# chzchzchz/raftsql

Hardware: AMD Instinct MI355X
Metric: quorum decisions/sec (commit+vote) across G groups (higher is better)
Workload: dtype u64

## Files before the change

go/raftq/engine_more.go:

```go
package raftq

import "C"

import "unsafe"

func ABIVersion() int { return int(C.raftq_abi_version()) }

func Quorum(peers uint32) uint32 { return uint32(C.raftq_quorum(C.uint32_t(peers))) }

func (e *Engine) NGroups() uint64 { return uint64(C.raftq_groups(e.h)) }
func (e *Engine) NPeers() uint32  { return uint32(C.raftq_peers(e.h)) }

func (e *Engine) SelfMax() (int, error) {
	var slot C.int32_t
	if err := e.err(C.raftq_self_max(e.h, &slot)); err != nil {
		return -1, err
	}
	return int(slot), nil
}

func (e *Engine) Narrow() (bool, error) {
	var valid C.int32_t
	if err := e.err(C.raftq_narrow(e.h, &valid)); err != nil {
		return false, err
	}
	return valid != 0, nil
}

func (e *Engine) NarrowRebuild() error { return e.err(C.raftq_narrow_rebuild(e.h)) }

func (e *Engine) SetStream(stream unsafe.Pointer) error { return e.err(C.raftq_set_stream(e.h, stream)) }
func (e *Engine) Stream() unsafe.Pointer                { return C.raftq_get_stream(e.h) }

type TermDelta struct{ Group, CurTerm, FirstIdxCurTerm uint64 }

func (e *Engine) ApplyTermDeltas(d []TermDelta) error {
	if len(d) == 0 {
		return nil
	}
	return e.err(C.raftq_apply_term_deltas(e.h, (*C.raftq_term_delta_t)(unsafe.Pointer(&d[0])), C.uint64_t(len(d))))
}

func (e *Engine) CommitAdvance(gated bool, committedOut []uint64) (changed uint64, err error) {
	var p *C.uint64_t
	if committedOut != nil {
		p = (*C.uint64_t)(unsafe.Pointer(&committedOut[0]))
	}
	g := C.int(0)
	if gated {
		g = 1
	}
	var n C.uint64_t
	err = e.err(C.raftq_commit_advance(e.h, g, p, &n))
	return uint64(n), err
}

func (e *Engine) VoteTally(outcomeOut []uint8) (Counts, error) {
	var p *C.uint8_t
	if outcomeOut != nil {
		p = (*C.uint8_t)(unsafe.Pointer(&outcomeOut[0]))
	}
	var c C.raftq_counts_t
	if err := e.err(C.raftq_vote_tally(e.h, p, &c)); err != nil {
		return Counts{}, err
	}
	return Counts{uint64(c.n_changed), uint64(c.n_won), uint64(c.n_lost)}, nil
}

func (e *Engine) ReadVotes(out []uint8) error {
	return e.err(C.raftq_read_votes(e.h, (*C.uint8_t)(unsafe.Pointer(&out[0]))))
}

func (e *Engine) SetTimers(electionTick, heartbeatTick uint32, seed uint64) error {
	return e.err(C.raftq_set_timers(e.h, C.uint32_t(electionTick), C.uint32_t(heartbeatTick), C.uint64_t(seed)))
}

type TickCounts struct{ Hup, Beat uint64 }

func (e *Engine) Tick(wantCounts bool) (TickCounts, error) {
	var c C.raftq_tick_counts_t
	if !wantCounts {
		return TickCounts{}, e.err(C.raftq_tick(e.h, nil))
	}
	err := e.err(C.raftq_tick(e.h, &c))
	return TickCounts{uint64(c.n_hup), uint64(c.n_beat)}, err
}

func (e *Engine) CollectHups(out []uint64) (uint64, error) {
	var n C.uint64_t
	var p *C.uint64_t
	if len(out) > 0 {
		p = (*C.uint64_t)(unsafe.Pointer(&out[0]))
	}
	rc := C.raftq_collect_hups(e.h, p, C.uint64_t(len(out)), &n)
	return uint64(n), e.err(rc)
}

func (e *Engine) TickCollect(hups, beats []uint64) (nHup, nBeat uint64, err error) {
	var hp, bp *C.uint64_t
	if len(hups) > 0 {
		hp = (*C.uint64_t)(unsafe.Pointer(&hups[0]))
	}
	if len(beats) > 0 {
		bp = (*C.uint64_t)(unsafe.Pointer(&beats[0]))
	}
	var nh, nb C.uint64_t
	err = e.err(C.raftq_tick_collect(e.h, hp, C.uint64_t(len(hups)), &nh, bp, C.uint64_t(len(beats)), &nb))
	return uint64(nh), uint64(nb), err
}

const TickBeatBitmap = uint(C.RAFTQ_TICK_BEAT_BITMAP)

// ... 218 lines not shown
```

include/raftq.h:

```cpp
#ifndef RAFTQ_H
#define RAFTQ_H

#include <stddef.h>
#include <stdint.h>

#ifdef __cplusplus
extern "C" {
#endif

#define RAFTQ_ABI_VERSION 1
#define RAFTQ_MAX_PEERS 9

#define RAFTQ_OK 0
#define RAFTQ_EINVAL (-1)
#define RAFTQ_ENOMEM (-2)
#define RAFTQ_EHIP (-3)
#define RAFTQ_ESTATE (-4)
#define RAFTQ_ENODEV (-5)

#define RAFTQ_SWEEP_COMMIT 0x01u
#define RAFTQ_SWEEP_GATED 0x02u
#define RAFTQ_SWEEP_VOTES 0x04u
#define RAFTQ_SWEEP_NO_ADOPT 0x08u
#define RAFTQ_SWEEP_LDS 0x10u
// ... 16 lines not shown
  uint64_t match;
  uint32_t peer;
  uint32_t _pad;
} raftq_delta_t;

typedef struct raftq_vote_delta {
  uint64_t group;
  uint32_t peer;
  uint8_t vote;
  uint8_t _pad[3];
} raftq_vote_delta_t;

typedef struct raftq_term_delta {
  uint64_t group;
  uint64_t cur_term;
  uint64_t first_idx_cur_term;
} raftq_term_delta_t;

typedef struct raftq_advance {
  uint64_t group;
  uint64_t old_commit;
  uint64_t new_commit;
} raftq_advance_t;

typedef struct raftq_delta16 {
  uint64_t match;
  uint32_t group;
  uint32_t peer;
} raftq_delta16_t;
typedef struct raftq_advance16 {
  uint64_t new_commit;
  uint32_t group;
  uint32_t advanced_by;
} raftq_advance16_t;

int raftq_abi_version(void);
int raftq_device_count(int* n);
uint32_t raftq_quorum(uint32_t n_peers);

#define RAFTQ_MAX_GROUPS (1ull << 30)
int raftq_create(int device, uint64_t n_groups, uint32_t n_peers, raftq_t** out);
void raftq_destroy(raftq_t* h);
uint64_t raftq_groups(const raftq_t* h);
uint32_t raftq_peers(const raftq_t* h);
const char* raftq_last_error(const raftq_t* h);

int raftq_set_stream(raftq_t* h, void* stream);
void* raftq_get_stream(const raftq_t* h);

int raftq_load_match(raftq_t* h, const uint64_t* match ,
                     const uint64_t* committed );
int raftq_load_terms(raftq_t* h, const uint64_t* cur_term ,
                     const uint64_t* first_idx_cur_term );
int raftq_load_votes(raftq_t* h, const uint8_t* votes );

int raftq_apply_deltas(raftq_t* h, const raftq_delta_t* d, uint64_t n);
int raftq_apply_vote_deltas(raftq_t* h, const raftq_vote_delta_t* d, uint64_t n);
int raftq_apply_term_deltas(raftq_t* h, const raftq_term_delta_t* d, uint64_t n);

typedef struct raftq_voter_delta {
  uint64_t group;
  uint16_t voters;
  uint16_t reset;
  uint32_t _pad;
} raftq_voter_delta_t;
int raftq_load_voters(raftq_t* h, const uint16_t* voters);
int raftq_apply_voter_deltas(raftq_t* h, const raftq_voter_delta_t* d, uint64_t n);
int raftq_read_voters(raftq_t* h, uint16_t* voters_out);

int raftq_step_async(raftq_t* h, unsigned flags);
int raftq_wait(raftq_t* h, raftq_counts_t* counts);

int raftq_commit_advance(raftq_t* h, int gated, uint64_t* committed_out ,
                         uint64_t* n_changed );
int raftq_vote_tally(raftq_t* h, uint8_t* outcome_out ,
                     raftq_counts_t* counts );

int raftq_read_committed(raftq_t* h, uint64_t* committed_out );
int raftq_read_outcome(raftq_t* h, uint8_t* outcome_out );
int raftq_read_match(raftq_t* h, uint64_t* match_out );
int raftq_self_max(raftq_t* h, int32_t* slot_out);
int raftq_narrow(raftq_t* h, int32_t* valid_out);
int raftq_narrow_rebuild(raftq_t* h);
int raftq_read_votes(raftq_t* h, uint8_t* votes_out );
int raftq_collect_changed(raftq_t* h, raftq_advance_t* out, uint64_t cap, uint64_t* n);

#define RAFTQ_ROLE_FOLLOWER 0
#define RAFTQ_ROLE_CANDIDATE 1
#define RAFTQ_ROLE_LEADER 2
#define RAFTQ_ROLE_PRE_CANDIDATE 3
typedef struct raftq_tick_counts {
  uint64_t n_hup;
  uint64_t n_beat;
} raftq_tick_counts_t;
int raftq_set_timers(raftq_t* h, uint32_t election_tick, uint32_t heartbeat_tick, uint64_t seed);
int raftq_load_roles(raftq_t* h, const uint8_t* role , const uint32_t* elapsed );
int raftq_tick_set_voters(raftq_t* h, int on);
int raftq_tick(raftq_t* h, raftq_tick_counts_t* counts);
int raftq_read_tick(raftq_t* h, uint8_t* action , uint32_t* elapsed , uint8_t* role );
int raftq_collect_hups(raftq_t* h, uint64_t* groups, uint64_t cap, uint64_t* n);
int raftq_collect_beats(raftq_t* h, uint64_t* groups, uint64_t cap, uint64_t* n);
int raftq_tick_collect(raftq_t* h, uint64_t* hups, uint64_t hup_cap, uint64_t* n_hup, uint64_t* beats, uint64_t beat_cap,
                       uint64_t* n_beat);

#define RAFTQ_TICK_BEAT_BITMAP 1u
int raftq_tick_collect_lists(raftq_t* h, unsigned flags, uint64_t hup_cap, uint64_t beat_cap, uint64_t* n_hup, uint64_t* n_beat);
int raftq_last_tick_lists(raftq_t* h, const uint32_t** hups, uint64_t* n_hups, const uint32_t** beats, uint64_t* n_beats,
                          const uint64_t** beat_bitmap, uint64_t* bitmap_words);
int raftq_set_check_quorum(raftq_t* h, int on);
int raftq_tick_set_checks(raftq_t* h, uint64_t chk_cap);
int raftq_last_tick_checks(raftq_t* h, const uint32_t** checks, uint64_t* n_listed, uint64_t* n_total);
int raftq_load_activity(raftq_t* h, const uint16_t* active , const uint32_t* lead_elapsed );
int raftq_read_activity(raftq_t* h, uint16_t* active , uint32_t* lead_elapsed );
int raftq_collect_checks(raftq_t* h, uint64_t* groups, uint64_t cap, uint64_t* n);

int raftq_set_pre_vote(raftq_t* h, int on);

int raftq_set_lead_transfer(raftq_t* h, int on);
int raftq_load_transfer(raftq_t* h, const uint8_t* transferee );
int raftq_read_transfer(raftq_t* h, uint8_t* transferee );

#define RAFTQ_READ_SAFE 1
#define RAFTQ_READ_LEASE 2
int raftq_set_read_index(raftq_t* h, int mode);
int raftq_load_reads(raftq_t* h, const uint32_t* seq , const uint32_t* acked );
int raftq_read_reads(raftq_t* h, uint32_t* seq, uint32_t* acked, uint32_t* confirmed );

int raftq_campaign(raftq_t* h, const uint64_t* groups, uint64_t n, uint32_t self_peer);

int raftq_cycle(raftq_t* h, const raftq_delta_t* deltas, uint64_t n_deltas,
                const raftq_vote_delta_t* vote_deltas, uint64_t n_vote_deltas, unsigned flags,
                raftq_advance_t* advances_out, uint64_t cap, uint64_t* n_advanced,
                raftq_counts_t* counts);

int raftq_stage(raftq_t* h, uint64_t n_deltas, uint64_t n_vote_deltas, raftq_delta_t** deltas,
                raftq_vote_delta_t** vote_deltas);
int raftq_last_advances(raftq_t* h, const raftq_advance_t** list, uint64_t* n_listed);

int raftq_cycle_packed(raftq_t* h, const raftq_delta16_t* deltas, uint64_t n_deltas,
                       const raftq_vote_delta_t* vote_deltas, uint64_t n_vote_deltas, unsigned flags,
                       raftq_advance16_t* advances_out, uint64_t cap, uint64_t* n_advanced,
                       raftq_counts_t* counts);
int raftq_stage_packed(raftq_t* h, uint64_t n_deltas, uint64_t n_vote_deltas, raftq_delta16_t** deltas,
                       raftq_vote_delta_t** vote_deltas);
int raftq_last_advances_packed(raftq_t* h, const raftq_advance16_t** list, uint64_t* n_listed);

#define RAFTQ_CYCLE_SEGMENTED 0x200u
int raftq_last_advance_segments(raftq_t* h, const raftq_advance16_t** recs, const uint32_t** counts, uint32_t* n_segments,
                                uint64_t* stride);

typedef struct raftq_set raftq_set_t;
#define RAFTQ_SET_GRID 0
#define RAFTQ_SET_PERSISTENT 1
int raftq_set_create(raftq_t* const* handles, uint32_t n, raftq_set_t** out);
int raftq_set_create_voters(raftq_t* const* handles, uint32_t n, raftq_set_t** out);
void raftq_set_destroy(raftq_set_t* s);
uint32_t raftq_set_size(const raftq_set_t* s);
const char* raftq_set_last_error(const raftq_set_t* s);
void* raftq_set_get_stream(const raftq_set_t* s);
int raftq_set_mode(raftq_set_t* s, int mode, uint32_t persist_workgroups);
int raftq_set_sweep_async(raftq_set_t* s, unsigned flags);
int raftq_set_tick(raftq_set_t* s);
int raftq_set_wait(raftq_set_t* s, raftq_counts_t* per_member, raftq_counts_t* total);
int raftq_set_timer_begin(raftq_set_t* s);
int raftq_set_timer_end(raftq_set_t* s, float* elapsed_ms);
int raftq_sweep_many_async(raftq_t* const* handles, uint32_t n, unsigned flags);
// ... 13 lines not shown
```

raftsql_amd/_lib.py:

```python
from __future__ import annotations

import ctypes as C
import os

_HERE = os.path.dirname(os.path.abspath(__file__))
LIB_PATH = os.environ.get("RAFTQ_LIB") or os.path.join(_HERE, "libraftq.so")

RAFTQ_OK = 0
RAFTQ_EINVAL, RAFTQ_ENOMEM, RAFTQ_EHIP, RAFTQ_ESTATE, RAFTQ_ENODEV = -1, -2, -3, -4, -5

SWEEP_COMMIT = 0x01
SWEEP_GATED = 0x02
SWEEP_VOTES = 0x04
SWEEP_NO_ADOPT = 0x08
SWEEP_LDS = 0x10
SWEEP_CHANGED = 0x20
SWEEP_STREAM = 0x40
SWEEP_CACHED = 0x80
CYCLE_TRUSTED = 0x100
TICK_BEAT_BITMAP = 1
CYCLE_SEGMENTED = 0x200
SET_GRID, SET_PERSISTENT = 0, 1

MAX_PEERS = 9
READ_SAFE, READ_LEASE = 1, 2


class Counts(C.Structure):
    _fields_ = [("n_changed", C.c_uint64), ("n_won", C.c_uint64), ("n_lost", C.c_uint64)]


class TickCounts(C.Structure):
    _fields_ = [("n_hup", C.c_uint64), ("n_beat", C.c_uint64)]


class Delta(C.Structure):
    _fields_ = [("group", C.c_uint64), ("match", C.c_uint64), ("peer", C.c_uint32), ("_pad", C.c_uint32)]


class VoteDelta(C.Structure):
    _fields_ = [("group", C.c_uint64), ("peer", C.c_uint32), ("vote", C.c_uint8), ("_pad", C.c_uint8 * 3)]


class VoterDelta(C.Structure):
    _fields_ = [("group", C.c_uint64), ("voters", C.c_uint16), ("reset", C.c_uint16), ("_pad", C.c_uint32)]


class Advance(C.Structure):
    _fields_ = [("group", C.c_uint64), ("old_commit", C.c_uint64), ("new_commit", C.c_uint64)]


_H = C.c_void_p
_SIGS = [
    ("raftq_abi_version", C.c_int, []),
    ("raftq_device_count", C.c_int, [C.POINTER(C.c_int)]),
    ("raftq_quorum", C.c_uint32, [C.c_uint32]),
    ("raftq_create", C.c_int, [C.c_int, C.c_uint64, C.c_uint32, C.POINTER(_H)]),
    ("raftq_destroy", None, [_H]),
    ("raftq_groups", C.c_uint64, [_H]),
    ("raftq_peers", C.c_uint32, [_H]),
    ("raftq_last_error", C.c_char_p, [_H]),
    ("raftq_set_stream", C.c_int, [_H, C.c_void_p]),
    ("raftq_get_stream", C.c_void_p, [_H]),
    ("raftq_load_match", C.c_int, [_H, C.c_void_p, C.c_void_p]),
    ("raftq_load_terms", C.c_int, [_H, C.c_void_p, C.c_void_p]),
    ("raftq_load_votes", C.c_int, [_H, C.c_void_p]),
    ("raftq_apply_deltas", C.c_int, [_H, C.c_void_p, C.c_uint64]),
    ("raftq_apply_vote_deltas", C.c_int, [_H, C.c_void_p, C.c_uint64]),
    ("raftq_apply_term_deltas", C.c_int, [_H, C.c_void_p, C.c_uint64]),
    ("raftq_load_voters", C.c_int, [_H, C.c_void_p]),
    ("raftq_apply_voter_deltas", C.c_int, [_H, C.c_void_p, C.c_uint64]),
    ("raftq_read_voters", C.c_int, [_H, C.c_void_p]),
    ("raftq_step_async", C.c_int, [_H, C.c_uint]),
    ("raftq_wait", C.c_int, [_H, C.POINTER(Counts)]),
    ("raftq_commit_advance", C.c_int, [_H, C.c_int, C.c_void_p, C.POINTER(C.c_uint64)]),
    ("raftq_vote_tally", C.c_int, [_H, C.c_void_p, C.POINTER(Counts)]),
    ("raftq_read_committed", C.c_int, [_H, C.c_void_p]),
    ("raftq_read_outcome", C.c_int, [_H, C.c_void_p]),
    ("raftq_read_match", C.c_int, [_H, C.c_void_p]),
    ("raftq_self_max", C.c_int, [_H, C.POINTER(C.c_int32)]),
    ("raftq_narrow", C.c_int, [_H, C.POINTER(C.c_int32)]),
    ("raftq_narrow_rebuild", C.c_int, [_H]),
    ("raftq_read_votes", C.c_int, [_H, C.c_void_p]),
    ("raftq_collect_changed", C.c_int, [_H, C.c_void_p, C.c_uint64, C.POINTER(C.c_uint64)]),
    ("raftq_set_timers", C.c_int, [_H, C.c_uint32, C.c_uint32, C.c_uint64]),
    ("raftq_load_roles", C.c_int, [_H, C.c_void_p, C.c_void_p]),
    ("raftq_tick_set_voters", C.c_int, [_H, C.c_int]),
    ("raftq_tick_set_checks", C.c_int, [_H, C.c_uint64]),
    ("raftq_last_tick_checks", C.c_int, [_H, C.POINTER(C.c_void_p), C.POINTER(C.c_uint64), C.POINTER(C.c_uint64)]),
    ("raftq_tick", C.c_int, [_H, C.POINTER(TickCounts)]),
    ("raftq_read_tick", C.c_int, [_H, C.c_void_p, C.c_void_p, C.c_void_p]),
    ("raftq_collect_hups", C.c_int, [_H, C.c_void_p, C.c_uint64, C.POINTER(C.c_uint64)]),
    ("raftq_collect_beats", C.c_int, [_H, C.c_void_p, C.c_uint64, C.POINTER(C.c_uint64)]),
    ("raftq_tick_collect", C.c_int, [_H, C.c_void_p, C.c_uint64, C.POINTER(C.c_uint64), C.c_void_p, C.c_uint64, C.POINTER(C.c_uint64)]),
    ("raftq_tick_collect_lists", C.c_int, [_H, C.c_uint, C.c_uint64, C.c_uint64, C.POINTER(C.c_uint64), C.POINTER(C.c_uint64)]),
    ("raftq_last_tick_lists", C.c_int, [_H, C.POINTER(C.c_void_p), C.POINTER(C.c_uint64), C.POINTER(C.c_void_p), C.POINTER(C.c_uint64),
                                        C.POINTER(C.c_void_p), C.POINTER(C.c_uint64)]),
    ("raftq_set_check_quorum", C.c_int, [_H, C.c_int]),
    ("raftq_set_pre_vote", C.c_int, [_H, C.c_int]),
    ("raftq_set_lead_transfer", C.c_int, [_H, C.c_int]),
    ("raftq_load_transfer", C.c_int, [_H, C.c_void_p]),
    ("raftq_read_transfer", C.c_int, [_H, C.c_void_p]),
    ("raftq_set_read_index", C.c_int, [_H, C.c_int]),
    ("raftq_load_reads", C.c_int, [_H, C.c_void_p, C.c_void_p]),
    ("raftq_read_reads", C.c_int, [_H, C.c_void_p, C.c_void_p, C.c_void_p]),
    ("raftq_load_activity", C.c_int, [_H, C.c_void_p, C.c_void_p]),
    ("raftq_read_activity", C.c_int, [_H, C.c_void_p, C.c_void_p]),
    ("raftq_collect_checks", C.c_int, [_H, C.c_void_p, C.c_uint64, C.POINTER(C.c_uint64)]),
    ("raftq_campaign", C.c_int, [_H, C.c_void_p, C.c_uint64, C.c_uint32]),
    ("raftq_cycle", C.c_int, [_H, C.c_void_p, C.c_uint64, C.c_void_p, C.c_uint64, C.c_uint, C.c_void_p, C.c_uint64,
                              C.POINTER(C.c_uint64), C.POINTER(Counts)]),
    ("raftq_stage", C.c_int, [_H, C.c_uint64, C.c_uint64, C.POINTER(C.c_void_p), C.POINTER(C.c_void_p)]),
    ("raftq_last_advances", C.c_int, [_H, C.POINTER(C.c_void_p), C.POINTER(C.c_uint64)]),
    ("raftq_cycle_packed", C.c_int, [_H, C.c_void_p, C.c_uint64, C.c_void_p, C.c_uint64, C.c_uint, C.c_void_p, C.c_uint64,
                                     C.POINTER(C.c_uint64), C.POINTER(Counts)]),
    ("raftq_stage_packed", C.c_int, [_H, C.c_uint64, C.c_uint64, C.POINTER(C.c_void_p), C.POINTER(C.c_void_p)]),
    ("raftq_last_advances_packed", C.c_int, [_H, C.POINTER(C.c_void_p), C.POINTER(C.c_uint64)]),
    ("raftq_last_advance_segments", C.c_int, [_H, C.POINTER(C.c_void_p), C.POINTER(C.c_void_p), C.POINTER(C.c_uint32), C.POINTER(C.c_uint64)]),
    ("raftq_set_create", C.c_int, [C.POINTER(_H), C.c_uint32, C.POINTER(_H)]),
    ("raftq_set_create_voters", C.c_int, [C.POINTER(_H), C.c_uint32, C.POINTER(_H)]),
    ("raftq_set_destroy", None, [_H]),
    ("raftq_set_size", C.c_uint32, [_H]),
    ("raftq_set_last_error", C.c_char_p, [_H]),
    ("raftq_set_get_stream", C.c_void_p, [_H]),
    ("raftq_set_mode", C.c_int, [_H, C.c_int, C.c_uint32]),
    ("raftq_set_sweep_async", C.c_int, [_H, C.c_uint]),
    ("raftq_set_wait", C.c_int, [_H, C.c_void_p, C.POINTER(Counts)]),
    ("raftq_set_tick", C.c_int, [_H]),
    ("raftq_set_timer_begin", C.c_int, [_H]),
    ("raftq_set_timer_end", C.c_int, [_H, C.POINTER(C.c_float)]),
    ("raftq_sweep_many_async", C.c_int, [C.POINTER(_H), C.c_uint32, C.c_uint]),
    ("raftq_clone_state", C.c_int, [_H, _H]),
    ("raftq_timer_begin", C.c_int, [_H]),
    ("raftq_timer_end", C.c_int, [_H, C.POINTER(C.c_float)]),
    ("raftq_host_alloc", C.c_int, [C.POINTER(C.c_void_p), C.c_uint64]),
    ("raftq_host_free", None, [C.c_void_p]),
]
EXPORTS = [s[0] for s in _SIGS]


class StepCounts(C.Structure):
    _fields_ = [("n_msgs", C.c_uint64), ("n_groups_touched", C.c_uint64)]


_STEP_SIGS = [
    ("raftq_set_self", C.c_int, [_H, C.c_uint32]),
    ("raftq_load_node", C.c_int, [_H, C.c_void_p, C.c_void_p, C.c_void_p, C.c_void_p, C.c_void_p]),
    ("raftq_read_node", C.c_int, [_H, C.c_void_p, C.c_void_p, C.c_void_p, C.c_void_p, C.c_void_p, C.c_void_p]),
    ("raftq_step_batch", C.c_int, [_H, C.c_void_p, C.c_uint64, C.c_void_p, C.POINTER(StepCounts)]),
    ("raftq_apply_log_deltas", C.c_int, [_H, C.c_void_p, C.c_uint64, C.c_void_p]),
    ("raftq_apply_log_deltas_nowait", C.c_int, [_H, C.c_void_p, C.c_uint64]),
    ("raftq_step_submit", C.c_int, [_H, C.c_void_p, C.c_uint64]),
    ("raftq_step_collect", C.c_int, [_H, C.c_void_p, C.POINTER(StepCounts)]),
    ("raftq_step_stage", C.c_int, [_H, C.c_uint64, C.POINTER(C.c_void_p)]),
    ("raftq_step_stage_packed", C.c_int, [_H, C.c_uint64, C.POINTER(C.c_void_p)]),
    ("raftq_step_submit_packed", C.c_int, [_H, C.c_void_p, C.c_uint64]),
    ("raftq_step_results", C.c_int, [_H, C.POINTER(C.c_void_p), C.POINTER(C.c_uint64)]),
    ("raftq_step_set_compact", C.c_int, [_H, C.c_int]),
    ("raftq_step_set_msg_flags", C.c_int, [_H, C.c_int]),
    ("raftq_step_set_voters", C.c_int, [_H, C.c_int]),
    ("raftq_step_set_props", C.c_int, [_H, C.c_int]),
    ("raftq_step_results_c", C.c_int, [_H, C.POINTER(C.c_void_p), C.POINTER(C.c_uint64)]),
    ("raftq_step_results_s", C.c_int, [_H, C.POINTER(C.c_void_p), C.POINTER(C.c_uint64)]),
]
STEP_EXPORTS = [s[0] for s in _STEP_SIGS]
# ... 86 lines not shown
```

raftsql_amd/csrc/raftq_capi.hip:

```cpp
#include "raftq.h"

#include <hip/hip_runtime.h>

#include <algorithm>
#include <atomic>
#include <mutex>
#include <chrono>
#include <cstdlib>
#include <cstdio>
#include <cstring>
#include <new>
#include <string>
#include <type_traits>
#include <unordered_set>
#include <vector>

#include "raftq_internal.hpp"

#ifndef RAFTQ_GPL
#define RAFTQ_GPL 4
#endif
#ifndef RAFTQ_AUTO_STREAM_BYTES
#define RAFTQ_AUTO_STREAM_BYTES (128ull << 20)
#endif
// ... 147 lines not shown
        const dim3 grid((unsigned)(gpad / ((uint64_t)kBlock * G))), block(kBlock);
        hipLaunchKernelGGL((sweep_voters_kernel<NP, G, Form::commit, Form::gated, Form::votes, decltype(pol)::value>), grid, block, 0, s, a);
        return hipGetLastError();
      });
    });
  });
}

struct VoterSetLaunch {
  const VoterSweepArgs* tab;
  uint32_t members, want_bits;
  uint64_t gpad;
};

hipError_t launch_set_voters(uint32_t N, const VoterSetLaunch& L, unsigned flags, int nt, hipStream_t s) {
  return with_peers(N, [&](auto n) {
    return with_flag_form(flags, [&](auto form) {
      return with_policy(nt, [&](auto pol) {
        using Form = decltype(form);
        constexpr int NP = decltype(n)::value, G = voters_gpl(NP);
        const dim3 grid((unsigned)(L.gpad / ((uint64_t)kBlock * G)), L.members), block(kBlock);
        hipLaunchKernelGGL((sweep_set_voters_kernel<NP, G, Form::commit, Form::gated, Form::votes, decltype(pol)::value>), grid, block, 0, s,
                           L.tab, L.want_bits);
        return hipGetLastError();
      });
    });
  });
}

}
int raftq_detail::ensure_staging(raftq_t* h, size_t bytes) {
  HIPCHK(h, h->stage.grow(bytes, std::max({bytes, h->stage.cap * 2, (size_t)1 << 20}), &h->stream));
  return RAFTQ_OK;
}

int raftq_detail::ensure_ingest(raftq_t* h, size_t bytes) {
  HIPCHK(h, h->ingest.grow(bytes, std::max({bytes, h->ingest.cap * 2, (size_t)1 << 20}), &h->stream, h->bar));
  return RAFTQ_OK;
}

namespace {
int ensure_adv(raftq_t* h, uint64_t entries) {
  const uint64_t have = h->adv.cap / sizeof(Advance);
  const uint64_t want = std::min<uint64_t>(std::max<uint64_t>({entries, have * 2, 4096}), h->gpad);
  HIPCHK(h, h->adv.grow(entries * sizeof(Advance), want * sizeof(Advance), &h->stream));
  return RAFTQ_OK;
}

}
int raftq_detail::self_max_check(raftq_t* h) {
  if (int rc = use_device(h)) return rc;
  if (h->step_collected != h->step_submitted) {
    HIPCHK(h, hipMemsetAsync(h->self_max, 0, sizeof(uint32_t), h->stream));
    return RAFTQ_OK;
  }
  HIPCHK(h, hipMemsetD32Async((hipDeviceptr_t)h->self_max, (int)(kSelfMaxValid | h->self_peer), 1, h->stream));
  const uint64_t blocks = std::min<uint64_t>((h->G + kBlock - 1) / kBlock, 4096);
  hipLaunchKernelGGL(self_max_check_kernel, dim3((unsigned)std::max<uint64_t>(blocks, 1)), dim3(kBlock), 0, h->stream,
                     (const uint64_t*)h->match, h->ld, h->G, h->N, h->self_peer, h->self_max);
  HIPCHK(h, hipGetLastError());
  return RAFTQ_OK;
}
int raftq_detail::narrow_build(raftq_t* h) {
  if (int rc = use_device(h)) return rc;
  if (h->narrow_off) return RAFTQ_OK;
  if (h->step_collected != h->step_submitted) {
    HIPCHK(h, hipMemsetAsync(h->narrow_word(), 0, sizeof(uint32_t), h->stream));
    return RAFTQ_OK;
  }
  if (!h->anchor) {
    const hipError_t e = raftq_buf::alloc_group({{(void**)&h->anchor, h->ld * sizeof(uint64_t)},
                                                 {(void**)&h->moff, (size_t)h->N * h->ld * sizeof(uint32_t)}},
                                                h->stream);
    if (e != hipSuccess) {
      (void)hipGetLastError();
      return RAFTQ_OK;
    }
    if (h->in_set) h->in_set->tab_stale = true;
  }
  HIPCHK(h, hipMemsetD32Async((hipDeviceptr_t)h->narrow_word(), (int)kNarrowValid, 1, h->stream));
  const uint64_t blocks = std::min<uint64_t>((h->G + kBlock - 1) / kBlock, 4096);
  hipLaunchKernelGGL(narrow_build_kernel, dim3((unsigned)std::max<uint64_t>(blocks, 1)), dim3(kBlock), 0, h->stream,
                     (const uint64_t*)h->match, h->ld, h->G, h->N, h->anchor, h->moff, h->narrow_word());
  HIPCHK(h, hipGetLastError());
  return RAFTQ_OK;
}
int raftq_detail::use_device(raftq_t* h) {
  if (!h) return fail(nullptr, RAFTQ_EINVAL, "null handle");
  HIPCHK(h, hipSetDevice(h->device));
  return RAFTQ_OK;
}
int raftq_detail::use_device_idle(raftq_t* h, const char* who) {
  if (int rc = use_device(h)) return rc;
  if (h->step_collected != h->step_submitted)
    return fail(h, RAFTQ_ESTATE, std::string(who) + ": Step batches are in flight; collect them first");
  return RAFTQ_OK;
}
using raftq_detail::ensure_staging;
using raftq_detail::ensure_ingest;
using raftq_detail::use_device;
using raftq_detail::use_device_idle;
using raftq_detail::ensure_tick_state;
using raftq_detail::dense_changed;

template <typename W>
static void pack_votes(const uint8_t* votes, uint64_t G, uint32_t N, W* out) {
  for (uint64_t g = 0; g < G; ++g) out[g] = 0;
  for (uint32_t p = 0; p < N; ++p) {
    const uint8_t* row = votes + (size_t)p * G;
    for (uint64_t g = 0; g < G; ++g) {
      const uint8_t v = row[g];
      out[g] = (W)(out[g] | (W)((v == 1 ? 1u : v == 2 ? 2u : 0u) << (2 * p)));
    }
  }
}
template <typename W>
static void unpack_votes(const W* in, uint64_t G, uint32_t N, uint8_t* votes) {
  for (uint32_t p = 0; p < N; ++p) {
    uint8_t* row = votes + (size_t)p * G;
    for (uint64_t g = 0; g < G; ++g) {
      const uint32_t f = ((uint32_t)in[g] >> (2 * p)) & 3u;
      row[g] = f == 3u ? 0 : (uint8_t)f;
    }
  }
}

extern "C" {

int raftq_abi_version(void) { return RAFTQ_ABI_VERSION; }

uint32_t raftq_quorum(uint32_t n_peers) { return n_peers / 2 + 1; }

int raftq_device_count(int* n) {
  if (!n) return fail(nullptr, RAFTQ_EINVAL, "raftq_device_count: null out");
  int c = 0;
  hipError_t e = hipGetDeviceCount(&c);
  if (e != hipSuccess) {
    *n = 0;
    return fail(nullptr, RAFTQ_ENODEV, std::string("hipGetDeviceCount: ") + hipGetErrorString(e));
  }
  *n = c;
  return RAFTQ_OK;
}

const char* raftq_last_error(const raftq_t* h) { return h ? h->err.c_str() : g_err.c_str(); }

uint64_t raftq_groups(const raftq_t* h) { return h ? h->G : 0; }
uint32_t raftq_peers(const raftq_t* h) { return h ? h->N : 0; }

int raftq_create(int device, uint64_t n_groups, uint32_t n_peers, raftq_t** out) {
  if (!out) return fail(nullptr, RAFTQ_EINVAL, "raftq_create: null out");
  *out = nullptr;
  if (n_groups == 0 || n_groups > RAFTQ_MAX_GROUPS)
    return fail(nullptr, RAFTQ_EINVAL, "raftq_create: n_groups out of range (1 .. RAFTQ_MAX_GROUPS = 2^30 per handle)");
  if (n_peers < 1 || n_peers > RAFTQ_MAX_PEERS) return fail(nullptr, RAFTQ_EINVAL, "raftq_create: n_peers must be 1..9");
  int ndev = 0;
  if (hipGetDeviceCount(&ndev) != hipSuccess || ndev <= 0)
    return fail(nullptr, RAFTQ_ENODEV, "raftq_create: no HIP device (this library has no CPU path)");
  if (device < 0 || device >= ndev) return fail(nullptr, RAFTQ_ENODEV, "raftq_create: device index out of range");
  raftq_t* h = new (std::nothrow) raftq();
  if (!h) return fail(nullptr, RAFTQ_ENOMEM, "raftq_create: host allocation failed");
  h->device = device;
  h->G = n_groups;
  h->N = n_peers;
  h->last_gpl = kGPL;
  h->gpad = (n_groups + kTileMax - 1) / kTileMax * kTileMax;
  h->ld = h->gpad + kRowStagger;
  const uint64_t ld = h->ld;
  h->max_partials = h->gpad / (kBlock * 2) * kWaves;
  int rc = RAFTQ_OK;
  do {
    if ((rc = use_device(h))) break;
    hipError_t e = hipStreamCreateWithFlags(&h->stream, hipStreamNonBlocking);
    if (e != hipSuccess) { rc = fail(h, RAFTQ_EHIP, std::string("hipStreamCreate: ") + hipGetErrorString(e)); break; }
    h->own_stream = true;
    {
      int large_bar = 0;
      (void)hipDeviceGetAttribute(&large_bar, hipDeviceAttributeIsLargeBar, device);
      const char* st = std::getenv("RAFTQ_STAGE");
      h->bar.staging = large_bar == 1 && !(st && std::strcmp(st, "host") == 0);
    }
    e = raftq_buf::alloc_group({{(void**)&h->match, (size_t)n_peers * ld * 8},
                                {(void**)&h->committed[0], ld * 8},
                                {(void**)&h->committed[1], ld * 8},
                                {(void**)&h->first_idx, ld * 8},
                                {(void**)&h->votes, (size_t)vote_word_bytes((int)n_peers) * ld},
                                {(void**)&h->outcome, ld / 4 + 64},
                                {(void**)&h->changed_bits, h->gpad / 8},
                                {(void**)&h->partials, h->max_partials * sizeof(uint4)},
                                {(void**)&h->offsets, (h->max_partials + 1) * 8},
                                {(void**)&h->self_max, 64}},
                               h->stream);
    if (e != hipSuccess) {
      rc = fail(h, e == hipErrorOutOfMemory ? RAFTQ_ENOMEM : RAFTQ_EHIP, std::string("device arrays: ") + hipGetErrorString(e));
      break;
    }
    {
      const char* nr = std::getenv("RAFTQ_NARROW");
      h->narrow_off = nr && std::strcmp(nr, "0") == 0;
    }
    e = hipMemsetD32Async((hipDeviceptr_t)h->self_max, (int)(kSelfMaxValid | 0u), 1, h->stream);
    if (e != hipSuccess) { rc = fail(h, RAFTQ_EHIP, std::string("hipMemsetD32Async: ") + hipGetErrorString(e)); break; }
    e = raftq_buf::alloc_group({{(void**)&h->h_partials, h->max_partials * sizeof(uint4), raftq_buf::Kind::pinned},
                                {(void**)&h->h_total, 64, raftq_buf::Kind::mapped_coherent, (void**)&h->d_total}},
                               h->stream);
    if (e != hipSuccess) { rc = fail(h, RAFTQ_ENOMEM, std::string("page-locked memory: ") + hipGetErrorString(e)); break; }
    e = hipEventCreate(&h->ev0);
    if (e == hipSuccess) e = hipEventCreate(&h->ev1);
    if (e != hipSuccess) { rc = fail(h, RAFTQ_EHIP, std::string("hipEventCreate: ") + hipGetErrorString(e)); break; }
    e = hipStreamSynchronize(h->stream);
    if (e != hipSuccess) { rc = fail(h, RAFTQ_EHIP, std::string("hipStreamSynchronize: ") + hipGetErrorString(e)); break; }
  } while (0);
  if (rc != RAFTQ_OK) {
    std::string keep = h->err;
    raftq_destroy(h);
    g_err = keep;
    return rc;
  }
  *out = h;
  return RAFTQ_OK;
}

void raftq_destroy(raftq_t* h) {
  if (!h) return;
  if (h->in_set) {
    raftq_set_t* s = h->in_set;
    s->broken = true;
    s->members.erase(std::remove(s->members.begin(), s->members.end(), h), s->members.end());
    (void)hipSetDevice(h->device);
    (void)hipStreamSynchronize(s->stream);
    h->stream = nullptr;
    h->own_stream = false;
  }
  if (h->prof_n && std::getenv("RAFTQ_PROFILE"))
    std::fprintf(stderr,
                 "[raftq] cycle phases, avg us over %llu calls: stage/validate %.1f | enqueue scatter %.1f | enqueue sweep "
                 "%.1f | enqueue collect %.1f | sync %.1f | copy-out %.1f | turns that ended in the blocking wait instead of the "
                 "polled flag: %llu\n",
                 (unsigned long long)h->prof_n, h->prof[0] / h->prof_n, h->prof[1] / h->prof_n, h->prof[2] / h->prof_n,
                 h->prof[3] / h->prof_n, h->prof[4] / h->prof_n, h->prof[5] / h->prof_n, (unsigned long long)h->flag_fallbacks);
  (void)hipSetDevice(h->device);
  if (h->stream) (void)hipStreamSynchronize(h->stream);
  if (h->many_aux) (void)hipStreamSynchronize(h->many_aux);
  raftq_detail::free_node_state(h);
  raftq_detail::free_wire_state(h);
  raftq_buf::free_device(h->match, h->committed[0], h->committed[1], h->first_idx, h->votes, h->voters, h->outcome, h->changed_bits,
                         h->partials, h->offsets, h->self_max, h->anchor, h->moff, h->claim, h->delta_bad, h->role, h->elapsed, h->action, h->hup_bits,
                         h->beat_bits, h->tick_partials, h->tick_offsets2, h->tick_offsets3, h->cq, h->chk_bits, h->reads);
  raftq_buf::free_host(h->h_partials, h->h_total);
  if (h->ev0) (void)hipEventDestroy(h->ev0);
  if (h->ev1) (void)hipEventDestroy(h->ev1);
  if (h->many_aux) {
    (void)hipEventDestroy(h->many_fork);
    (void)hipEventDestroy(h->many_join);
  }
  const hipStream_t streams[4] = {h->many_aux, h->step_s_in, h->step_s_out, h->own_stream ? h->stream : nullptr};
  delete h;
  for (hipStream_t st : streams)
    if (st) (void)hipStreamDestroy(st);
}

int raftq_set_stream(raftq_t* h, void* stream) {
  if (int rc = use_device_idle(h, "raftq_set_stream")) return rc;
  if (h->in_set) return fail(h, RAFTQ_ESTATE, "raftq_set_stream: the handle is a member of a sweep set, which owns its stream");
  HIPCHK(h, hipStreamSynchronize(h->stream));
  if (h->own_stream) HIPCHK(h, hipStreamDestroy(h->stream));
  h->stream = (hipStream_t)stream;
  h->own_stream = false;
  return RAFTQ_OK;
}

void* raftq_get_stream(const raftq_t* h) { return h ? (void*)h->stream : nullptr; }

int raftq_load_match(raftq_t* h, const uint64_t* match, const uint64_t* committed) {
  if (int rc = use_device_idle(h, "raftq_load_match")) return rc;
  if (!match && !committed) return fail(h, RAFTQ_EINVAL, "raftq_load_match: nothing to load");
  if (match) {
    for (uint32_t p = 0; p < h->N; ++p)
      HIPCHK(h, hipMemcpyAsync(h->match + (size_t)p * h->ld, match + (size_t)p * h->G, h->G * 8, hipMemcpyHostToDevice, h->stream));
    if (int rc = raftq_detail::self_max_check(h)) return rc;
    if (int rc = raftq_detail::narrow_build(h)) return rc;
  }
  dense_changed(h);
  if (committed)
    HIPCHK(h, hipMemcpyAsync(h->committed[h->cur], committed, h->G * 8, hipMemcpyHostToDevice, h->stream));
  HIPCHK(h, hipStreamSynchronize(h->stream));
  return RAFTQ_OK;
}

int raftq_load_terms(raftq_t* h, const uint64_t* cur_term, const uint64_t* first_idx_cur_term) {
  if (int rc = use_device_idle(h, "raftq_load_terms")) return rc;
  if (!cur_term || !first_idx_cur_term) return fail(h, RAFTQ_EINVAL, "raftq_load_terms: null argument");
  std::vector<uint64_t> f;
  try {
    f.assign(first_idx_cur_term, first_idx_cur_term + h->G);
  } catch (...) {
    return fail(h, RAFTQ_ENOMEM, "raftq_load_terms: host allocation failed");
  }
  for (uint64_t g = 0; g < h->G; ++g)
    if (cur_term[g] == 0) f[g] = 0;
  HIPCHK(h, hipMemcpyAsync(h->first_idx, f.data(), h->G * 8, hipMemcpyHostToDevice, h->stream));
  dense_changed(h);
  HIPCHK(h, hipStreamSynchronize(h->stream));
  h->have_terms = true;
  return RAFTQ_OK;
}

int raftq_load_votes(raftq_t* h, const uint8_t* votes) {
  if (int rc = use_device_idle(h, "raftq_load_votes")) return rc;
  if (!votes) return fail(h, RAFTQ_EINVAL, "raftq_load_votes: null argument");
  const size_t wb = (size_t)vote_word_bytes((int)h->N);
  std::vector<uint8_t> packed;
  try {
    packed.resize(h->G * wb);
  } catch (...) {
    return fail(h, RAFTQ_ENOMEM, "raftq_load_votes: host allocation failed");
  }
  if (wb == 2) pack_votes(votes, h->G, h->N, reinterpret_cast<uint16_t*>(packed.data()));
  else pack_votes(votes, h->G, h->N, reinterpret_cast<uint32_t*>(packed.data()));
  HIPCHK(h, hipMemcpyAsync(h->votes, packed.data(), packed.size(), hipMemcpyHostToDevice, h->stream));
  HIPCHK(h, hipStreamSynchronize(h->stream));
  return RAFTQ_OK;
}

static int ensure_delta_dev(raftq_t* h, size_t bytes) {
  if (!h->delta_bad) HIPCHK(h, raftq_buf::alloc_zeroed((void**)&h->delta_bad, 64, h->stream));
  HIPCHK(h, h->delta_dev.grow(bytes, std::max(bytes * 2, (size_t)1 << 20), &h->stream));
  return RAFTQ_OK;
}

static int check_deltas(raftq_t* h, bool trusted = false) {
  int rc = RAFTQ_OK;
  const char* what = trusted ? "; that record was dropped, every other record of the turn was applied (RAFTQ_CYCLE_TRUSTED)"
                             : "; nothing applied";
  if (h->delta_check[0] && h->h_total[1] == h->delta_check[0])
    rc = fail(h, RAFTQ_EINVAL, std::string("a match delta is out of range (group >= G or peer >= N)") + what);
  if (h->delta_check[1] && h->h_total[2] == h->delta_check[1])
    rc = fail(h, RAFTQ_EINVAL, std::string("a vote delta is invalid (group/peer out of range or vote not 1/2)") + what);
  h->delta_check[0] = h->delta_check[1] = 0;
  return rc;
}

}

template <typename Rec, typename AbiRec>
static int enqueue_ingest(raftq_t* h, const AbiRec* d, uint64_t n, const raftq_vote_delta_t* vd, uint64_t nv, size_t off_votes,
                          bool trusted = false) {
  static_assert(sizeof(Rec) == sizeof(AbiRec), "ABI struct mismatch");
  static_assert(sizeof(VoteDeltaRec) == sizeof(raftq_vote_delta_t), "ABI struct mismatch");
  if (nv > 0xfffffffeull) return fail(h, RAFTQ_EINVAL, "vote delta batch too large");
  auto inside = [&](const void* q) {
    return (const uint8_t*)q >= (const uint8_t*)h->ingest.h && (const uint8_t*)q < (const uint8_t*)h->ingest.h + h->ingest.cap;
  };
  if (n) {
    AbiRec* dst = (AbiRec*)h->ingest.h;
    if ((const void*)d != (const void*)dst) {
      if (inside(d)) return fail(h, RAFTQ_EINVAL, "match deltas staged with other counts / another record layout than this call's");
      std::memcpy(dst, d, (size_t)n * sizeof(AbiRec));
    }
  }
  if (nv) {
    raftq_vote_delta_t* dst = (raftq_vote_delta_t*)((uint8_t*)h->ingest.h + off_votes);
    if ((const void*)vd != (const void*)dst) {
      if (inside(vd)) return fail(h, RAFTQ_EINVAL, "vote deltas staged with other counts / another record layout than this call's");
      std::memcpy(dst, vd, (size_t)nv * sizeof(raftq_vote_delta_t));
    }
    if (!h->claim) {
      HIPCHK(h, raftq_buf::alloc_filled((void**)&h->claim, (size_t)h->N * h->ld * sizeof(uint32_t), 0xff, h->stream));
    }
  }
  h->ingest.publish();
  if (int rc = ensure_delta_dev(h, h->ingest.cap)) return rc;
  const unsigned long long em = n ? ++h->delta_epoch : kNoEpoch, ev = nv ? ++h->delta_epoch : kNoEpoch;
  h->delta_check[0] = n ? em : 0;
  h->delta_check[1] = nv ? ev : 0;
  Rec* dev_m = (Rec*)h->delta_dev.d;
  VoteDeltaRec* dev_v = (VoteDeltaRec*)((uint8_t*)h->delta_dev.d + off_votes);
  const unsigned long long* bad = h->delta_bad;
  const dim3 gm((unsigned)((n + kBlock - 1) / kBlock)), gv((unsigned)((nv + kBlock - 1) / kBlock));
  if (n) dense_changed(h);
  if (n && trusted)
    hipLaunchKernelGGL((deltas_in_apply_kernel<Rec>), gm, dim3(kBlock), 0, h->stream, (const Rec*)h->ingest.d, n, h->match, h->ld,
                       h->G, h->N, h->delta_bad, h->d_total + 1, em, h->self_max, h->narrow_mirror());
  else if (n)
    hipLaunchKernelGGL((deltas_in_kernel<Rec>), gm, dim3(kBlock), 0, h->stream, (const Rec*)h->ingest.d, dev_m, n, h->G, h->N,
                       h->delta_bad, h->d_total + 1, em);
  if (nv)
    hipLaunchKernelGGL(vote_deltas_in_kernel, gv, dim3(kBlock), 0, h->stream,
                       (const VoteDeltaRec*)((uint8_t*)h->ingest.d + off_votes), dev_v, nv, h->G, h->N, h->delta_bad + 1,
                       h->d_total + 2, ev);
  if (n && !trusted)
    hipLaunchKernelGGL((apply_deltas_kernel<Rec>), gm, dim3(kBlock), 0, h->stream, h->match, h->ld, (const Rec*)dev_m, n, bad, em,
                       ev, h->self_max, h->narrow_mirror());
  if (nv) {
    const unsigned long long em_gate = trusted ? kNoEpoch : em;
    hipLaunchKernelGGL(vote_claim_kernel, gv, dim3(kBlock), 0, h->stream, h->claim, h->ld, (const VoteDeltaRec*)dev_v, nv, bad,
                       em_gate, ev, h->G, h->N, trusted ? 1 : 0);
    hipLaunchKernelGGL(vote_apply_kernel, gv, dim3(kBlock), 0, h->stream, h->votes, h->N > 8 ? 1 : 0, h->claim, h->ld,
                       (const VoteDeltaRec*)dev_v, nv, bad, em_gate, ev, h->G, h->N, trusted ? 1 : 0);
  }
  HIPCHK(h, hipGetLastError());
  return RAFTQ_OK;
}

extern "C" {

int raftq_apply_deltas(raftq_t* h, const raftq_delta_t* d, uint64_t n) {
  if (int rc = use_device_idle(h, "raftq_apply_deltas")) return rc;
  if (n == 0) return RAFTQ_OK;
  if (!d) return fail(h, RAFTQ_EINVAL, "raftq_apply_deltas: null argument");
  if (int rc = ensure_ingest(h, (size_t)n * sizeof(raftq_delta_t))) return rc;
  if (int rc = enqueue_ingest<DeltaRec>(h, d, n, nullptr, 0, 0)) return rc;
  HIPCHK(h, hipStreamSynchronize(h->stream));
  return check_deltas(h);
}

int raftq_apply_term_deltas(raftq_t* h, const raftq_term_delta_t* d, uint64_t n) {
  static_assert(sizeof(TermDeltaRec) == sizeof(raftq_term_delta_t), "ABI struct mismatch");
  if (int rc = use_device_idle(h, "raftq_apply_term_deltas")) return rc;
  if (n == 0) return RAFTQ_OK;
  if (!d) return fail(h, RAFTQ_EINVAL, "raftq_apply_term_deltas: null argument");
  for (uint64_t i = 0; i < n; ++i)
    if (d[i].group >= h->G) return fail(h, RAFTQ_EINVAL, "a term delta is out of range; nothing applied");
  if (int rc = ensure_staging(h, (size_t)n * sizeof(raftq_term_delta_t))) return rc;
  raftq_term_delta_t* dst = (raftq_term_delta_t*)h->stage.h;
  uint64_t m = 0;
  {
    std::unordered_set<uint64_t> seen;
    seen.reserve((size_t)n * 2);
    std::vector<uint64_t> keep;
    keep.reserve(n);
    for (uint64_t i = n; i-- > 0;)
      if (seen.insert(d[i].group).second) keep.push_back(i);
    for (auto it = keep.rbegin(); it != keep.rend(); ++it) dst[m++] = d[*it];
  }
  const dim3 grid((unsigned)((m + kBlock - 1) / kBlock));
  dense_changed(h);
  hipLaunchKernelGGL(apply_term_deltas_kernel, grid, dim3(kBlock), 0, h->stream, h->first_idx,
                     (const TermDeltaRec*)h->stage.d, m);
  HIPCHK(h, hipGetLastError());
  HIPCHK(h, hipStreamSynchronize(h->stream));
  h->have_terms = true;
  return RAFTQ_OK;
}

int raftq_apply_vote_deltas(raftq_t* h, const raftq_vote_delta_t* d, uint64_t n) {
  if (int rc = use_device_idle(h, "raftq_apply_vote_deltas")) return rc;
  if (n == 0) return RAFTQ_OK;
  if (!d) return fail(h, RAFTQ_EINVAL, "raftq_apply_vote_deltas: null argument");
  if (int rc = ensure_ingest(h, (size_t)n * sizeof(raftq_vote_delta_t))) return rc;
  if (int rc = enqueue_ingest<DeltaRec>(h, (const raftq_delta_t*)nullptr, 0, d, n, 0)) return rc;
  HIPCHK(h, hipStreamSynchronize(h->stream));
  return check_deltas(h);
}

}

static int ensure_voters(raftq_t* h) {
  if (h->voters) return RAFTQ_OK;
  HIPCHK(h, raftq_buf::alloc_zeroed((void**)&h->voters, h->ld * sizeof(uint16_t), h->stream));
  if (h->in_set) h->in_set->tab_stale = true;
  return RAFTQ_OK;
}
static int drop_voters(raftq_t* h) {
  if (!h->voters) return RAFTQ_OK;
  HIPCHK(h, hipStreamSynchronize(h->stream));
  raftq_buf::free_device(h->voters);
  if (h->in_set) h->in_set->tab_stale = true;
  return RAFTQ_OK;
}
static int voters_not_in_set(raftq_t* h, const char* who) {
  if (!h->in_set || h->in_set->allow_voters) return RAFTQ_OK;
  return fail(h, RAFTQ_ESTATE, std::string(who) + ": the handle is a member of a sweep set, whose dispatches count every slot "
                                                  "(voter masks on set members are out of scope)");
}
int raftq_detail::refuse_voters(raftq_t* h, const char* who, bool step_family, bool tick_rounds, bool bcast) {
  if (!h || !h->voters) return RAFTQ_OK;
  if (tick_rounds && h->tick_voters) return RAFTQ_OK;
  if (bcast) {
    if (h->bcast_voters) return RAFTQ_OK;
    return fail(h, RAFTQ_ESTATE, std::string(who) + ": the handle has voter masks loaded and did not opt in with raftq_bcast_set_voters; its broadcast "
                                                    "would go to N - 1 slots, not to a group's membership (whatever raftq_step_set_voters and "
                                                    "raftq_tick_set_voters say)");
  }
  if (h->step_voters) {
    if (step_family) return RAFTQ_OK;
    return fail(h, RAFTQ_ESTATE, std::string(who) + ": the handle has voter masks loaded; the broadcasts built on the device go to N - 1 slots, "
                                                    "not to a group's membership (out of scope, whatever raftq_step_set_voters says)");
  }
  return fail(h, RAFTQ_ESTATE, std::string(who) + ": the handle has voter masks loaded; Step's maybeCommit / poll on the device "
                                                  "count every slot (out of scope: raftq_load_voters(h, NULL) first)");
}

extern "C" {

int raftq_load_voters(raftq_t* h, const uint16_t* voters) {
  if (int rc = use_device_idle(h, "raftq_load_voters")) return rc;
  if (int rc = voters_not_in_set(h, "raftq_load_voters")) return rc;
  if (!voters) return drop_voters(h);
  const uint32_t beyond = 0xffffu & ~((1u << h->N) - 1u);
  for (uint64_t g = 0; g < h->G; ++g)
    if (voters[g] & beyond) return fail(h, RAFTQ_EINVAL, "raftq_load_voters: a mask names a peer slot >= N; nothing loaded");
  if (int rc = ensure_voters(h)) return rc;
  HIPCHK(h, hipMemcpyAsync(h->voters, voters, h->G * sizeof(uint16_t), hipMemcpyHostToDevice, h->stream));
  HIPCHK(h, hipStreamSynchronize(h->stream));
  return RAFTQ_OK;
}

int raftq_read_voters(raftq_t* h, uint16_t* voters_out) {
  if (int rc = use_device_idle(h, "raftq_read_voters")) return rc;
  if (!voters_out) return fail(h, RAFTQ_EINVAL, "raftq_read_voters: null argument");
  if (!h->voters) {
    std::fill(voters_out, voters_out + h->G, (uint16_t)((1u << h->N) - 1u));
    return RAFTQ_OK;
  }
  HIPCHK(h, hipMemcpyAsync(voters_out, h->voters, h->G * sizeof(uint16_t), hipMemcpyDeviceToHost, h->stream));
  HIPCHK(h, hipStreamSynchronize(h->stream));
  return RAFTQ_OK;
}

int raftq_apply_voter_deltas(raftq_t* h, const raftq_voter_delta_t* d, uint64_t n) {
  static_assert(sizeof(VoterDeltaRec) == sizeof(raftq_voter_delta_t), "ABI struct mismatch");
  if (int rc = use_device_idle(h, "raftq_apply_voter_deltas")) return rc;
  if (int rc = voters_not_in_set(h, "raftq_apply_voter_deltas")) return rc;
  if (n == 0) return RAFTQ_OK;
  if (!d) return fail(h, RAFTQ_EINVAL, "raftq_apply_voter_deltas: null argument");
  const uint32_t beyond = 0xffffu & ~((1u << h->N) - 1u);
  for (uint64_t i = 0; i < n; ++i)
    if (d[i].group >= h->G || ((d[i].voters | d[i].reset) & beyond))
      return fail(h, RAFTQ_EINVAL, "a voter delta is out of range (group >= G or a bit >= N); nothing applied");
  if (int rc = ensure_staging(h, (size_t)n * sizeof(raftq_voter_delta_t))) return rc;
  raftq_voter_delta_t* dst = (raftq_voter_delta_t*)h->stage.h;
  uint64_t m = 0;
  try {
    std::unordered_set<uint64_t> seen;
    seen.reserve((size_t)n * 2);
    std::vector<uint64_t> keep;
    keep.reserve(n);
    for (uint64_t i = n; i-- > 0;)
      if (seen.insert(d[i].group).second) keep.push_back(i);
    for (auto it = keep.rbegin(); it != keep.rend(); ++it) dst[m++] = d[*it];
  } catch (...) {
    return fail(h, RAFTQ_ENOMEM, "raftq_apply_voter_deltas: host allocation failed");
  }
  if (!h->voters) {
    if (int rc = ensure_voters(h)) return rc;
    hipLaunchKernelGGL(fill_voters_kernel, dim3((unsigned)((h->G + kBlock - 1) / kBlock)), dim3(kBlock), 0, h->stream, h->voters, h->G,
                       (uint16_t)((1u << h->N) - 1u));
    HIPCHK(h, hipGetLastError());
  }
  dense_changed(h);
  hipLaunchKernelGGL(apply_voter_deltas_kernel, dim3((unsigned)((m + kBlock - 1) / kBlock)), dim3(kBlock), 0, h->stream, h->voters, h->match,
                     h->ld, h->votes, h->N > 8 ? 1 : 0, h->N, (const VoterDeltaRec*)h->stage.d, m, h->self_max, h->narrow_word());
  HIPCHK(h, hipGetLastError());
  HIPCHK(h, hipStreamSynchronize(h->stream));
  return RAFTQ_OK;
}

static int sweep_check(raftq_t* h, unsigned flags, const char* who) {
  const unsigned known = RAFTQ_SWEEP_COMMIT | RAFTQ_SWEEP_GATED | RAFTQ_SWEEP_VOTES | RAFTQ_SWEEP_NO_ADOPT |
                         RAFTQ_SWEEP_LDS | RAFTQ_SWEEP_CHANGED | RAFTQ_SWEEP_STREAM | RAFTQ_SWEEP_CACHED;
  const std::string w(who);
  if (flags & ~known) return fail(h, RAFTQ_EINVAL, w + ": unknown flag");
  const bool commit = flags & (RAFTQ_SWEEP_COMMIT | RAFTQ_SWEEP_GATED);
  const bool votes = flags & RAFTQ_SWEEP_VOTES;
  if (!commit && !votes) return fail(h, RAFTQ_EINVAL, w + ": nothing to sweep");
  if ((flags & RAFTQ_SWEEP_GATED) && !h->have_terms)
    return fail(h, RAFTQ_ESTATE, w + ": gated sweep before raftq_load_terms");
  if ((flags & RAFTQ_SWEEP_STREAM) && (flags & RAFTQ_SWEEP_CACHED))
    return fail(h, RAFTQ_EINVAL, w + ": RAFTQ_SWEEP_STREAM and RAFTQ_SWEEP_CACHED are exclusive");
  if ((flags & RAFTQ_SWEEP_CHANGED) && !commit)
    return fail(h, RAFTQ_EINVAL, w + ": RAFTQ_SWEEP_CHANGED needs a commit sweep");
  if ((flags & RAFTQ_SWEEP_LDS) && h->voters)
    return fail(h, RAFTQ_EINVAL, w + ": RAFTQ_SWEEP_LDS has no form for a handle with voter masks loaded (the A/B variant counts every slot)");
  return RAFTQ_OK;
}

static SweepArgs sweep_args(const raftq_t* h, int cur, bool want_bits) {
  SweepArgs a;
  a.match = h->match;
  a.committed = h->committed[cur];
  a.committed_out = h->committed[cur ^ 1];
  a.first_idx = h->first_idx;
  a.votes = h->votes;
  a.outcome = h->outcome;
  a.changed_bits = want_bits ? h->changed_bits : nullptr;
  a.partials = h->partials;
  a.ld = h->ld;
  a.self_max = h->self_max;
  a.narrow = h->anchor ? h->narrow_word() : nullptr;
  a.anchor = h->anchor;
  a.moff = h->moff;
  return a;
}

static uint64_t sweep_footprint(const raftq_t* h) { return h->ld * (8ull * h->N + 24 + vote_word_bytes((int)h->N) + 1 + (h->voters ? 2 : 0)); }

static int sweep_policy(unsigned flags, uint64_t footprint) {
  const bool stream = (flags & RAFTQ_SWEEP_STREAM) ? true
                      : (flags & RAFTQ_SWEEP_CACHED) ? false
                                                     : footprint >= RAFTQ_AUTO_STREAM_BYTES;
  return !stream ? 0 : footprint >= RAFTQ_AUTO_STREAM_BYTES ? 3 : 1;
}

static void sweep_done(raftq_t* h, unsigned flags, int gpl) {
  const bool commit = flags & (RAFTQ_SWEEP_COMMIT | RAFTQ_SWEEP_GATED);
  h->n_partials = h->gpad / ((uint64_t)kBlock * gpl) * kWaves;
  h->last_flags = flags;
  h->last_gpl = gpl;
  if (commit) {
    h->last_old = h->committed[h->cur];
    h->last_new = h->committed[h->cur ^ 1];
    if (!(flags & RAFTQ_SWEEP_NO_ADOPT)) {
      h->cur ^= 1;
      dense_changed(h);
    }
  }
}

static int sweep_on(raftq_t* h, unsigned flags, hipStream_t s, const char* who) {
  if (int rc = use_device_idle(h, who)) return rc;
  if (int rc = sweep_check(h, flags, who)) return rc;
  const bool commit = flags & (RAFTQ_SWEEP_COMMIT | RAFTQ_SWEEP_GATED);
  const SweepArgs a = sweep_args(h, h->cur, flags & RAFTQ_SWEEP_CHANGED);
  if (h->voters) {
    VoterSweepArgs va;
    va.s = a;
    va.voters = h->voters;
    HIPCHK(h, launch_voters(h->N, va, h->gpad, flags, sweep_policy(flags, sweep_footprint(h)), s));
    sweep_done(h, flags, voters_gpl((int)h->N));
    return RAFTQ_OK;
  }
  const bool lds = (flags & RAFTQ_SWEEP_LDS) && commit;
  SweepLaunch L;
  L.one = &a;
  L.gpad = h->gpad;
  HIPCHK(h, launch_sweep(h->N, L, flags, sweep_policy(flags, sweep_footprint(h)), s));
  sweep_done(h, flags, lds ? kLdsGPL : kGPL);
  return RAFTQ_OK;
}

int raftq_step_async(raftq_t* h, unsigned flags) {
  if (!h) return fail(nullptr, RAFTQ_EINVAL, "null handle");
  return sweep_on(h, flags, h->stream, "raftq_step_async");
}


int raftq_sweep_many_async(raftq_t* const* handles, uint32_t n, unsigned flags) {
  if (!handles && n) return fail(nullptr, RAFTQ_EINVAL, "raftq_sweep_many_async: null handle array");
  bool alternate = n >= 2;
  for (uint32_t i = 0; alternate && i < n; ++i) {
    if (!handles[i] || handles[i]->stream != handles[0]->stream || handles[i]->device != handles[0]->device) alternate = false;
    for (uint32_t j = 0; alternate && j < i; ++j)
      if (handles[j] == handles[i]) alternate = false;
  }
  if (!alternate) {
    for (uint32_t i = 0; i < n; ++i)
      if (int rc = raftq_step_async(handles[i], flags)) return rc;
    return RAFTQ_OK;
  }
  raftq_t* h0 = handles[0];
  if (int rc = use_device(h0)) return rc;
  if (!h0->many_aux) {
    HIPCHK(h0, hipStreamCreateWithFlags(&h0->many_aux, hipStreamNonBlocking));
    HIPCHK(h0, hipEventCreateWithFlags(&h0->many_fork, hipEventDisableTiming));
    HIPCHK(h0, hipEventCreateWithFlags(&h0->many_join, hipEventDisableTiming));
  }
  HIPCHK(h0, hipEventRecord(h0->many_fork, h0->stream));
  HIPCHK(h0, hipStreamWaitEvent(h0->many_aux, h0->many_fork, 0));
  int rc = RAFTQ_OK;
  for (uint32_t i = 0; i < n && rc == RAFTQ_OK; ++i)
    rc = sweep_on(handles[i], flags, (i & 1) ? h0->many_aux : h0->stream, "raftq_sweep_many_async");
  HIPCHK(h0, hipEventRecord(h0->many_join, h0->many_aux));
  HIPCHK(h0, hipStreamWaitEvent(h0->stream, h0->many_join, 0));
  return rc;
}

int raftq_wait(raftq_t* h, raftq_counts_t* counts) {
  if (int rc = use_device_idle(h, "raftq_wait")) return rc;
  if (counts) {
    if (h->n_partials == 0) return fail(h, RAFTQ_ESTATE, "raftq_wait: no sweep to report on");
    HIPCHK(h, hipMemcpyAsync(h->h_partials, h->partials, h->n_partials * sizeof(uint4), hipMemcpyDeviceToHost, h->stream));
  }
  HIPCHK(h, hipStreamSynchronize(h->stream));
  if (counts) {
    uint64_t c = 0, w = 0, l = 0;
    for (uint64_t i = 0; i < h->n_partials; ++i) {
      c += h->h_partials[i].x;
      w += h->h_partials[i].y;
      l += h->h_partials[i].z;
    }
    const bool commit = h->last_flags & (RAFTQ_SWEEP_COMMIT | RAFTQ_SWEEP_GATED);
    const bool votes = h->last_flags & RAFTQ_SWEEP_VOTES;
    counts->n_changed = commit ? c : 0;
    counts->n_won = votes ? w : 0;
    counts->n_lost = votes ? l : 0;
  }
  return RAFTQ_OK;
}

int raftq_read_committed(raftq_t* h, uint64_t* out) {
  if (int rc = use_device_idle(h, "raftq_read_committed")) return rc;
  if (!out) return fail(h, RAFTQ_EINVAL, "raftq_read_committed: null argument");
  const uint64_t* src = (h->last_flags & RAFTQ_SWEEP_NO_ADOPT) && h->last_new ? h->last_new : h->committed[h->cur];
  HIPCHK(h, hipMemcpyAsync(out, src, h->G * 8, hipMemcpyDeviceToHost, h->stream));
  HIPCHK(h, hipStreamSynchronize(h->stream));
  return RAFTQ_OK;
}

int raftq_read_outcome(raftq_t* h, uint8_t* out) {
  if (int rc = use_device_idle(h, "raftq_read_outcome")) return rc;
  if (!out) return fail(h, RAFTQ_EINVAL, "raftq_read_outcome: null argument");
  std::vector<uint8_t> packed;
  try {
    packed.resize((h->G + 3) / 4);
  } catch (...) {
    return fail(h, RAFTQ_ENOMEM, "raftq_read_outcome: host allocation failed");
  }
  HIPCHK(h, hipMemcpyAsync(packed.data(), h->outcome, packed.size(), hipMemcpyDeviceToHost, h->stream));
  HIPCHK(h, hipStreamSynchronize(h->stream));
  for (uint64_t g = 0; g < h->G; ++g) out[g] = (uint8_t)((packed[g >> 2] >> (2 * (g & 3))) & 3u);
  return RAFTQ_OK;
}

int raftq_self_max(raftq_t* h, int32_t* slot) {
  if (int rc = use_device_idle(h, "raftq_self_max")) return rc;
  if (!slot) return fail(h, RAFTQ_EINVAL, "raftq_self_max: null argument");
  uint32_t w = 0;
  HIPCHK(h, hipMemcpyAsync(&w, h->self_max, sizeof w, hipMemcpyDeviceToHost, h->stream));
  HIPCHK(h, hipStreamSynchronize(h->stream));
  *slot = (w & kSelfMaxValid) ? (int32_t)(w & 0xffu) : -1;
  return RAFTQ_OK;
}

int raftq_narrow(raftq_t* h, int32_t* valid) {
  if (int rc = use_device_idle(h, "raftq_narrow")) return rc;
  if (!valid) return fail(h, RAFTQ_EINVAL, "raftq_narrow: null argument");
  uint32_t w = 0;
  HIPCHK(h, hipMemcpyAsync(&w, h->narrow_word(), sizeof w, hipMemcpyDeviceToHost, h->stream));
  HIPCHK(h, hipStreamSynchronize(h->stream));
  *valid = w == kNarrowValid ? 1 : 0;
  return RAFTQ_OK;
}

int raftq_narrow_rebuild(raftq_t* h) {
  if (int rc = use_device_idle(h, "raftq_narrow_rebuild")) return rc;
  if (int rc = raftq_detail::narrow_build(h)) return rc;
  HIPCHK(h, hipStreamSynchronize(h->stream));
  return RAFTQ_OK;
}

int raftq_read_match(raftq_t* h, uint64_t* out) {
  if (int rc = use_device_idle(h, "raftq_read_match")) return rc;
  if (!out) return fail(h, RAFTQ_EINVAL, "raftq_read_match: null argument");
  for (uint32_t p = 0; p < h->N; ++p)
    HIPCHK(h, hipMemcpyAsync(out + (size_t)p * h->G, h->match + (size_t)p * h->ld, h->G * 8, hipMemcpyDeviceToHost, h->stream));
  HIPCHK(h, hipStreamSynchronize(h->stream));
  return RAFTQ_OK;
}

int raftq_read_votes(raftq_t* h, uint8_t* out) {
  if (int rc = use_device_idle(h, "raftq_read_votes")) return rc;
  if (!out) return fail(h, RAFTQ_EINVAL, "raftq_read_votes: null argument");
  const size_t wb = (size_t)vote_word_bytes((int)h->N);
  std::vector<uint8_t> packed;
  try {
    packed.resize(h->G * wb);
  } catch (...) {
    return fail(h, RAFTQ_ENOMEM, "raftq_read_votes: host allocation failed");
  }
  HIPCHK(h, hipMemcpyAsync(packed.data(), h->votes, packed.size(), hipMemcpyDeviceToHost, h->stream));
  HIPCHK(h, hipStreamSynchronize(h->stream));
  if (wb == 2) unpack_votes(reinterpret_cast<const uint16_t*>(packed.data()), h->G, h->N, out);
  else unpack_votes(reinterpret_cast<const uint32_t*>(packed.data()), h->G, h->N, out);
  return RAFTQ_OK;
}

int raftq_commit_advance(raftq_t* h, int gated, uint64_t* committed_out, uint64_t* n_changed) {
  if (int rc = raftq_step_async(h, gated ? (RAFTQ_SWEEP_COMMIT | RAFTQ_SWEEP_GATED) : RAFTQ_SWEEP_COMMIT)) return rc;
  raftq_counts_t c;
  if (int rc = raftq_wait(h, &c)) return rc;
  if (n_changed) *n_changed = c.n_changed;
  if (committed_out) return raftq_read_committed(h, committed_out);
  return RAFTQ_OK;
}

int raftq_vote_tally(raftq_t* h, uint8_t* outcome_out, raftq_counts_t* counts) {
  if (int rc = raftq_step_async(h, RAFTQ_SWEEP_VOTES)) return rc;
  raftq_counts_t c;
  if (int rc = raftq_wait(h, &c)) return rc;
  if (counts) *counts = c;
  if (outcome_out) return raftq_read_outcome(h, outcome_out);
  return RAFTQ_OK;
}

}

static hipError_t wait_turn(raftq_t* h, uint64_t flag_epoch, int kind = 0) {
  constexpr uint32_t kMisses = 8, kRetry = 1024;
  const bool try_flag = flag_epoch && (h->flag_misses[kind] < kMisses || (++h->flag_rested[kind] % kRetry) == 0);
  if (try_flag) {
    volatile uint64_t* flag = h->h_total + 3;
    const auto t0 = std::chrono::steady_clock::now();
    for (int i = 0;; ++i) {
      if ((*flag & h->flag_mask) == flag_epoch) {
        std::atomic_thread_fence(std::memory_order_acquire);
        h->flag_misses[kind] = 0;
        if (hipPeekAtLastError() == hipSuccess) return hipSuccess;
        (void)hipGetLastError();
        return hipStreamSynchronize(h->stream);
      }
      if ((i & 255) == 255 && std::chrono::steady_clock::now() - t0 > std::chrono::microseconds(2000)) break;
    }
    ++h->flag_misses[kind];
  }
  if (flag_epoch) ++h->flag_fallbacks;
  return hipStreamSynchronize(h->stream);
}

hipError_t raftq_detail::wait_call(raftq_t* h) {
  hipError_t e;
  if (!h->d_total) {
    e = hipStreamSynchronize(h->stream);
  } else {
    const uint64_t epoch = ++h->compact_epoch;
    h->flag_mask = ~0ull;
    hipLaunchKernelGGL(raise_flag_kernel, dim3(1), dim3(64), 0, h->stream, h->d_total + 3, epoch);
    e = hipGetLastError() != hipSuccess ? hipStreamSynchronize(h->stream) : wait_turn(h, epoch, 1);
  }
  if (e == hipSuccess && h->wal_pending && !h->wal_pending_done) h->wal_pending_waited = true;
// ... 564 lines not shown
  if (beats) *beats = bitmap ? nullptr : h->tl.h + h->tl_beat_at;
  if (n_beats) *n_beats = bitmap ? 0 : std::min(h->tl_n_beat, h->tl_beat_cap);
  if (beat_bitmap) *beat_bitmap = bitmap ? (const uint64_t*)((const uint8_t*)h->tl.h + h->tl_map_off) : nullptr;
  if (bitmap_words) *bitmap_words = bitmap ? (h->G + 63) / 64 : 0;
  return RAFTQ_OK;
}

int raftq_last_tick_checks(raftq_t* h, const uint32_t** checks, uint64_t* n_listed, uint64_t* n_total) {
  if (!h) return fail(nullptr, RAFTQ_EINVAL, "null handle");
  if (!h->tl_valid || !h->tl_chk_valid)
    return fail(h, RAFTQ_ESTATE, "raftq_last_tick_checks: no raftq_tick_collect_lists / raftq_tick_frames / raftq_tick_elect_frames under "
                                 "raftq_tick_set_checks (with raftq_set_check_quorum on) before it");
  if (checks) *checks = (const uint32_t*)((const uint8_t*)h->tl.h + h->tl_chk_off);
  if (n_listed) *n_listed = std::min(h->tl_n_chk, h->tl_chk_cap);
  if (n_total) *n_total = h->tl_n_chk;
  return RAFTQ_OK;
}

int raftq_read_tick(raftq_t* h, uint8_t* action, uint32_t* elapsed, uint8_t* role) {
  if (int rc = use_device_idle(h, "raftq_read_tick")) return rc;
  if (!h->role) return fail(h, RAFTQ_ESTATE, "raftq_read_tick: no tick state (raftq_load_roles / raftq_tick first)");
  if (action) HIPCHK(h, hipMemcpyAsync(action, h->action, h->G, hipMemcpyDeviceToHost, h->stream));
  if (elapsed) HIPCHK(h, hipMemcpyAsync(elapsed, h->elapsed, h->G * 4, hipMemcpyDeviceToHost, h->stream));
  if (role) HIPCHK(h, hipMemcpyAsync(role, h->role, h->G, hipMemcpyDeviceToHost, h->stream));
  HIPCHK(h, hipStreamSynchronize(h->stream));
  return RAFTQ_OK;
}

static int collect_tick_list(raftq_t* h, const char* who, int field, uint64_t* groups, uint64_t cap, uint64_t* n) {
  if (int rc = use_device_idle(h, who)) return rc;
  if (!n) return fail(h, RAFTQ_EINVAL, std::string(who) + ": null count");
  if (!h->ticked) return fail(h, RAFTQ_ESTATE, std::string(who) + ": no raftq_tick yet");
  if (cap && !groups) return fail(h, RAFTQ_EINVAL, std::string(who) + ": null out with cap > 0");
  const uint64_t take_cap = std::min<uint64_t>(cap, h->G);
  if (take_cap)
    if (int rc = ensure_adv(h, (take_cap + 2) / 3 + 1)) return rc;
  const uint64_t nw = h->gpad / 256;
  hipLaunchKernelGGL(scan_partials_kernel, dim3(1), dim3(1024), 0, h->stream, h->tick_partials, nw, h->offsets,
                     h->d_total, field);
  if (take_cap)
    hipLaunchKernelGGL(compact_hups_kernel, dim3((unsigned)(h->gpad / 1024)), dim3(kBlock), 0, h->stream,
                       field == 2 ? h->chk_bits : field ? h->beat_bits : h->hup_bits, h->offsets, (uint64_t*)h->adv.d, take_cap);
  HIPCHK(h, hipGetLastError());
  HIPCHK(h, hipStreamSynchronize(h->stream));
  const uint64_t total = *h->h_total;
  *n = total;
  const uint64_t take = std::min(total, take_cap);
  if (take) std::memcpy(groups, h->adv.h, take * 8);
  h->adv_listed = 0;
  return RAFTQ_OK;
}

int raftq_collect_hups(raftq_t* h, uint64_t* groups, uint64_t cap, uint64_t* n) {
  return collect_tick_list(h, "raftq_collect_hups", 0, groups, cap, n);
}

int raftq_collect_beats(raftq_t* h, uint64_t* groups, uint64_t cap, uint64_t* n) {
  return collect_tick_list(h, "raftq_collect_beats", 1, groups, cap, n);
}

int raftq_collect_checks(raftq_t* h, uint64_t* groups, uint64_t cap, uint64_t* n) {
  if (h && !h->cq) {
    if (int rc = use_device_idle(h, "raftq_collect_checks")) return rc;
    if (!n) return fail(h, RAFTQ_EINVAL, "raftq_collect_checks: null count");
    if (cap && !groups) return fail(h, RAFTQ_EINVAL, "raftq_collect_checks: null out with cap > 0");
    *n = 0;
    return RAFTQ_OK;
  }
  return collect_tick_list(h, "raftq_collect_checks", 2, groups, cap, n);
}

int raftq_campaign(raftq_t* h, const uint64_t* groups, uint64_t n, uint32_t self_peer) {
  if (int rc = use_device_idle(h, "raftq_campaign")) return rc;
  if (n == 0) return RAFTQ_OK;
  if (!groups) return fail(h, RAFTQ_EINVAL, "raftq_campaign: null argument");
  if (self_peer >= h->N) return fail(h, RAFTQ_EINVAL, "raftq_campaign: self_peer out of range");
  uint64_t bad = 0;
  for (uint64_t i = 0; i < n; ++i) bad |= (uint64_t)(groups[i] >= h->G);
  if (bad) return fail(h, RAFTQ_EINVAL, "raftq_campaign: a group is out of range; nothing applied");
  if (int rc = ensure_tick_state(h)) return rc;
  if (int rc = ensure_staging(h, (size_t)n * 8)) return rc;
  std::memcpy(h->stage.h, groups, n * 8);
  hipLaunchKernelGGL(campaign_kernel, dim3((unsigned)((n + kBlock - 1) / kBlock)), dim3(kBlock), 0, h->stream,
                     h->role, h->elapsed, h->votes, h->N, self_peer, (const uint64_t*)h->stage.d, n);
  dense_changed(h);
  HIPCHK(h, hipGetLastError());
  HIPCHK(h, hipStreamSynchronize(h->stream));
  return RAFTQ_OK;
}

}


template <typename Adv>
static int enqueue_collect(raftq_t* h, uint64_t take_cap, bool want_flag) {
  static_assert(sizeof(Advance) == sizeof(raftq_advance_t) && sizeof(Advance16) == sizeof(raftq_advance16_t), "ABI struct mismatch");
  const int gpl = h->last_gpl;
  const dim3 grid((unsigned)(h->gpad / ((uint64_t)kBlock * gpl)));
  Adv* out = (Adv*)h->adv.d;
  const uint64_t* wave_offsets = nullptr;
  if (h->n_partials > (1u << 14)) {
    hipLaunchKernelGGL(scan_partials_kernel, dim3(1), dim3(1024), 0, h->stream, h->partials, h->n_partials, h->offsets,
                       h->d_total, 0);
    wave_offsets = h->offsets;
  }
  switch (gpl) {
    case 2:
      hipLaunchKernelGGL((compact_changed_kernel<2, Adv>), grid, dim3(kBlock), 0, h->stream, h->changed_bits, h->partials,
                         h->last_old, h->last_new, out, take_cap, h->d_total, wave_offsets);
      break;
    case 8:
      hipLaunchKernelGGL((compact_changed_kernel<8, Adv>), grid, dim3(kBlock), 0, h->stream, h->changed_bits, h->partials,
                         h->last_old, h->last_new, out, take_cap, h->d_total, wave_offsets);
      break;
    default:
      static_assert((kGPL == 4 || kGPL == 8) && kLdsGPL == 4, "compaction instantiations cover GPL 2, 4, 8");
      hipLaunchKernelGGL((compact_changed_kernel<4, Adv>), grid, dim3(kBlock), 0, h->stream, h->changed_bits, h->partials,
                         h->last_old, h->last_new, out, take_cap, h->d_total, wave_offsets);
  }
  HIPCHK(h, hipGetLastError());
  h->compact_epoch_armed = 0;
  if (want_flag) {
    const uint64_t epoch = ++h->compact_epoch;
    hipLaunchKernelGGL(raise_flag_kernel, dim3(1), dim3(64), 0, h->stream, h->d_total + 3, epoch);
    HIPCHK(h, hipGetLastError());
    h->compact_epoch_armed = epoch;
  }
  return RAFTQ_OK;
}

constexpr uint64_t kSegmentsMaxGroups = 1ull << 22;
static bool segments_ok(const raftq_t* h, unsigned flags) {
  if (const char* e = std::getenv("RAFTQ_CYCLE_SEGMENTS"))
    if (e[0] == '0') return false;
  const unsigned allowed = RAFTQ_SWEEP_COMMIT | RAFTQ_SWEEP_GATED | RAFTQ_SWEEP_CHANGED | RAFTQ_SWEEP_NO_ADOPT | RAFTQ_SWEEP_STREAM | RAFTQ_SWEEP_CACHED;
  if (h->voters) return false;
  return (flags & (RAFTQ_SWEEP_COMMIT | RAFTQ_SWEEP_GATED)) && !(flags & ~allowed) && h->gpad <= kSegmentsMaxGroups;
}
static int enqueue_sweep_segments(raftq_t* h, unsigned flags) {
  const uint32_t n_tiles = (uint32_t)(h->gpad / kTile);
  if (int rc = ensure_adv(h, (h->gpad * sizeof(Advance16) + sizeof(Advance) - 1) / sizeof(Advance))) return rc;
  HIPCHK(h, h->seg_h.grow((size_t)n_tiles * 4, (size_t)n_tiles * 4, &h->stream));
  HIPCHK(h, h->seg_d.grow((size_t)n_tiles * 4, (size_t)n_tiles * 4, &h->stream));
  const SweepArgs a = sweep_args(h, h->cur, true);
  uint64_t epoch = ++h->compact_epoch;
  if ((uint32_t)epoch == 0) epoch = ++h->compact_epoch;
  HIPCHK(h, launch_segments(h->N, a, n_tiles, (flags & RAFTQ_SWEEP_GATED) != 0, sweep_policy(flags, sweep_footprint(h)), (Advance16*)h->adv.d, h->seg_h.d,
                            h->seg_d.d, h->stream));
  sweep_done(h, flags, kGPL);
  hipLaunchKernelGGL(raise_flag_segments_kernel, dim3(1), dim3(kBlock), 0, h->stream, h->d_total + 3, (uint32_t)epoch, h->seg_d.d, n_tiles);
  HIPCHK(h, hipGetLastError());
  h->compact_epoch_armed = (uint64_t)(uint32_t)epoch << 32;
  h->flag_mask = 0xffffffff00000000ull;
  h->seg_tiles = n_tiles;
  h->seg_stride = kTile;
  return RAFTQ_OK;
}

extern "C" {

int raftq_collect_changed(raftq_t* h, raftq_advance_t* out, uint64_t cap, uint64_t* n) {
  if (int rc = use_device_idle(h, "raftq_collect_changed")) return rc;
  if (!n) return fail(h, RAFTQ_EINVAL, "raftq_collect_changed: null count");
  if (!(h->last_flags & RAFTQ_SWEEP_CHANGED) || !h->last_old)
    return fail(h, RAFTQ_ESTATE, "raftq_collect_changed: last sweep did not set RAFTQ_SWEEP_CHANGED");
  if (cap && !out) return fail(h, RAFTQ_EINVAL, "raftq_collect_changed: null out with cap > 0");
  const uint64_t take_cap = std::min<uint64_t>(cap, h->G);
// ... 559 lines not shown
  if (want) {
    if (!s->swept) return sfail(s, RAFTQ_ESTATE, "raftq_set_wait: no set sweep to report on");
    set_fill_table(s, -1, s->tab_host);
    SETCHK(s, hipMemcpyAsync(s->tab[2].d, s->tab_host.data(), n * sizeof(SweepArgs), hipMemcpyHostToDevice, s->stream));
    s->np_host.resize(n);
    for (size_t i = 0; i < n; ++i) s->np_host[i] = s->members[i]->n_partials;
    SETCHK(s, hipMemcpyAsync(s->np.d, s->np_host.data(), n * 8, hipMemcpyHostToDevice, s->stream));
    hipLaunchKernelGGL(set_counts_kernel, dim3((unsigned)n), dim3(kBlock), 0, s->stream, (const SweepArgs*)s->tab[2].d,
                       (const uint64_t*)s->np.d, s->counts.d);
    SETCHK(s, hipGetLastError());
    SETCHK(s, hipMemcpyAsync(s->counts_h.h, s->counts.d, n * 32, hipMemcpyDeviceToHost, s->stream));
  }
  SETCHK(s, hipStreamSynchronize(s->stream));
  if (want) {
    raftq_counts_t t{0, 0, 0};
    for (size_t i = 0; i < n; ++i) {
      const unsigned f = s->members[i]->last_flags;
      const bool commit = f & (RAFTQ_SWEEP_COMMIT | RAFTQ_SWEEP_GATED);
      const bool votes = f & RAFTQ_SWEEP_VOTES;
      raftq_counts_t c{commit ? s->counts_h.h[4 * i] : 0, votes ? s->counts_h.h[4 * i + 1] : 0, votes ? s->counts_h.h[4 * i + 2] : 0};
      if (per_member) per_member[i] = c;
      t.n_changed += c.n_changed;
      t.n_won += c.n_won;
      t.n_lost += c.n_lost;
    }
    if (total) *total = t;
  }
  return RAFTQ_OK;
}

int raftq_set_timer_begin(raftq_set_t* s) {
  if (int rc = set_ready(s, "raftq_set_timer_begin")) return rc;
  SETCHK(s, hipEventRecord(s->ev0, s->stream));
  return RAFTQ_OK;
}

int raftq_set_timer_end(raftq_set_t* s, float* elapsed_ms) {
  if (int rc = set_ready(s, "raftq_set_timer_end")) return rc;
  if (!elapsed_ms) return sfail(s, RAFTQ_EINVAL, "raftq_set_timer_end: null argument");
  SETCHK(s, hipEventRecord(s->ev1, s->stream));
  SETCHK(s, hipEventSynchronize(s->ev1));
  SETCHK(s, hipEventElapsedTime(elapsed_ms, s->ev0, s->ev1));
  return RAFTQ_OK;
}

int raftq_clone_state(raftq_t* dst, raftq_t* src) {
  if (int rc = use_device_idle(dst, "raftq_clone_state")) return rc;
  if (!src) return fail(dst, RAFTQ_EINVAL, "raftq_clone_state: null source");
  if (src == dst) return RAFTQ_OK;
  if (src->device != dst->device || src->N != dst->N || src->G != dst->G)
    return fail(dst, RAFTQ_EINVAL, "raftq_clone_state: source and destination must have the same device, groups and peers");
  if (src->step_collected != src->step_submitted)
    return fail(dst, RAFTQ_ESTATE, "raftq_clone_state: the source has Step batches in flight");
  if (src->voters && dst->in_set && !dst->in_set->allow_voters)
    return fail(dst, RAFTQ_ESTATE, "raftq_clone_state: the source has voter masks loaded and the destination is a member of a sweep "
                                   "set, whose dispatches count every slot (out of scope)");
  if (src->voters) {
    if (int rc = ensure_voters(dst)) return rc;
  } else if (int rc = drop_voters(dst)) {
    return rc;
  }
  HIPCHK(dst, hipStreamSynchronize(src->stream));
  const uint64_t ld = dst->ld;
  HIPCHK(dst, hipMemcpyAsync(dst->match, src->match, (size_t)dst->N * ld * 8, hipMemcpyDeviceToDevice, dst->stream));
  HIPCHK(dst, hipMemcpyAsync(dst->committed[dst->cur], src->committed[src->cur], ld * 8, hipMemcpyDeviceToDevice, dst->stream));
  HIPCHK(dst, hipMemcpyAsync(dst->first_idx, src->first_idx, ld * 8, hipMemcpyDeviceToDevice, dst->stream));
  HIPCHK(dst, hipMemcpyAsync(dst->votes, src->votes, (size_t)vote_word_bytes((int)dst->N) * ld, hipMemcpyDeviceToDevice,
                             dst->stream));
  HIPCHK(dst, hipMemcpyAsync(dst->self_max, src->self_max, sizeof(uint32_t), hipMemcpyDeviceToDevice, dst->stream));
  if (src->anchor && !dst->narrow_off && !dst->anchor) {
    if (raftq_buf::alloc_group({{(void**)&dst->anchor, ld * sizeof(uint64_t), raftq_buf::Kind::device, nullptr, false},
                                {(void**)&dst->moff, (size_t)dst->N * ld * sizeof(uint32_t), raftq_buf::Kind::device, nullptr, false}},
                               dst->stream) != hipSuccess)
      (void)hipGetLastError();
    else if (dst->in_set) dst->in_set->tab_stale = true;
  }
  if (src->anchor && dst->anchor && !dst->narrow_off) {
    HIPCHK(dst, hipMemcpyAsync(dst->anchor, src->anchor, ld * sizeof(uint64_t), hipMemcpyDeviceToDevice, dst->stream));
    HIPCHK(dst, hipMemcpyAsync(dst->moff, src->moff, (size_t)dst->N * ld * sizeof(uint32_t), hipMemcpyDeviceToDevice, dst->stream));
    HIPCHK(dst, hipMemcpyAsync(dst->narrow_word(), src->narrow_word(), sizeof(uint32_t), hipMemcpyDeviceToDevice, dst->stream));
  } else {
    HIPCHK(dst, hipMemsetAsync(dst->narrow_word(), 0, sizeof(uint32_t), dst->stream));
  }
  if (src->voters) HIPCHK(dst, hipMemcpyAsync(dst->voters, src->voters, ld * sizeof(uint16_t), hipMemcpyDeviceToDevice, dst->stream));
  if (src->cq && dst->cq) HIPCHK(dst, hipMemcpyAsync(dst->cq, src->cq, ld * sizeof(uint32_t), hipMemcpyDeviceToDevice, dst->stream));
  if (src->reads && dst->reads) HIPCHK(dst, hipMemcpyAsync(dst->reads, src->reads, ld * sizeof(raftqk::ReadRec), hipMemcpyDeviceToDevice, dst->stream));
  HIPCHK(dst, hipStreamSynchronize(dst->stream));
  dst->have_terms = src->have_terms;
  dense_changed(dst);
  return RAFTQ_OK;
}

}
```

raftsql_amd/csrc/raftq_internal.hpp:

```cpp
#pragma once
#include <hip/hip_runtime.h>

#include <string>
#include <vector>

#include "raftq.h"
#include "raftq_wire.h"
#include "raftq_kernels.hpp"
#include "raftq_buffers.hpp"

struct raftq {
  int device = 0;
  uint64_t G = 0, gpad = 0, ld = 0;
  uint32_t N = 0;
  hipStream_t stream = nullptr;
  bool own_stream = false;
  struct raftq_set* in_set = nullptr;
  uint64_t* match = nullptr;
  uint64_t* committed[2] = {nullptr, nullptr};
  int cur = 0;
  uint64_t* first_idx = nullptr;
  uint8_t* votes = nullptr;
  uint16_t* voters = nullptr;
  uint8_t* outcome = nullptr;
  uint64_t* changed_bits = nullptr;
  uint4* partials = nullptr;
  uint4* h_partials = nullptr;
  uint64_t n_partials = 0;
  uint64_t max_partials = 0;
  uint64_t* offsets = nullptr;
  uint64_t* h_total = nullptr;
  raftq_buf::Buffer<> stage{raftq_buf::Kind::mapped};
  raftq_buf::HostWritable ingest;
  raftq_buf::BarRule bar;
  std::vector<uint64_t> ld_mark, ld_start;
  struct LdNowait {
    raftq_buf::Buffer<> buf{raftq_buf::Kind::mapped};
    hipEvent_t ev = nullptr;
  };
  LdNowait ld_nowait[2];
  uint32_t ld_nowait_next = 0;
  std::vector<uint32_t> ld_round, ld_pos;
  uint32_t ld_epoch = 0;
  raftq_buf::Buffer<raftqk::Advance> adv{raftq_buf::Kind::mapped_coherent};
  uint64_t adv_listed = 0;
  bool adv_packed = false;
  bool adv_segmented = false;
  raftq_buf::Buffer<uint32_t> seg_h{raftq_buf::Kind::mapped_coherent};
  raftq_buf::Buffer<unsigned int> seg_d{raftq_buf::Kind::device};
  uint32_t seg_tiles = 0, seg_stride = 0, seg_one = 0;
  uint64_t flag_mask = ~0ull;
  uint32_t* self_max = nullptr;
  uint64_t* anchor = nullptr;
  uint32_t* moff = nullptr;
  bool narrow_off = false;
  uint32_t* narrow_word() const { return self_max + 1; }
  raftqk::NarrowMirror narrow_mirror() const { return raftqk::NarrowMirror{self_max + 1, anchor, moff}; }
  uint64_t compact_epoch = 0;
  uint64_t compact_epoch_armed = 0;
  uint32_t flag_misses[2] = {0, 0}, flag_rested[2] = {0, 0};
  uint64_t flag_fallbacks = 0;
  uint32_t* claim = nullptr;
  raftq_buf::Buffer<> delta_dev{raftq_buf::Kind::device};
  unsigned long long* delta_bad = nullptr;
  unsigned long long delta_epoch = 0;
  unsigned long long delta_check[2] = {0, 0};
  uint8_t* role = nullptr;
  uint32_t* elapsed = nullptr;
  uint8_t* action = nullptr;
  uint64_t* hup_bits = nullptr;
  uint64_t* beat_bits = nullptr;
  uint4* tick_partials = nullptr;
  raftq_buf::Buffer<uint32_t> tl{raftq_buf::Kind::mapped_coherent};
  uint64_t tl_hup_cap = 0, tl_beat_cap = 0, tl_beat_at = 0, tl_map_off = 0;
  uint64_t tl_n_hup = 0, tl_n_beat = 0;
  unsigned tl_flags = 0;
  bool tl_valid = false;
  uint64_t* tick_offsets2 = nullptr;
  uint32_t election_tick = 10, heartbeat_tick = 1;
  uint64_t tick_seed = 0x1000, tick_no = 0;
  bool ticked = false;
  uint32_t* cq = nullptr;
  uint64_t* chk_bits = nullptr;
  bool pre_vote = false;
  bool lead_transfer = false;
  uint8_t read_index = 0;
  void* reads = nullptr;
  uint64_t tick_chk_cap = 0;
  uint64_t tl_chk_cap = 0, tl_chk_off = 0, tl_n_chk = 0;
  bool tl_chk_valid = false;
  uint64_t* tick_offsets3 = nullptr;
  uint64_t* d_total = nullptr;
  bool have_terms = false;
  unsigned last_flags = 0;
  int last_gpl = 0;
  const uint64_t* last_old = nullptr;
  const uint64_t* last_new = nullptr;
  uint32_t self_peer = 0;
  bool self_set = false;
  bool node_mirror_fresh = false;
  uint64_t node_mirror_refreshes = 0;
  void* node_rec = nullptr;
  unsigned int* step_stall = nullptr;
  uint8_t step_compact = 0;
  bool step_msg_flags = false;
  bool step_voters = false;
  bool step_props = false;
  bool tick_voters = false;
  bool bcast_voters = false;
  bool resp_lead = false;
  bool resp_props = false;
  bool prop_forward = false;
  int step_walk_mode = 1;
  uint32_t step_stalls_in_a_row = 0, step_sorted_left = 0;
  uint64_t step_replays = 0;
  static constexpr int kStepSlots = 3;
  struct StepSlot {
    raftq_buf::Buffer<> in_h{raftq_buf::Kind::pinned};
    raftq_buf::HostWritable in_bar;
    raftq_buf::Buffer<> dev{raftq_buf::Kind::device};
    raftq_buf::Buffer<> out{raftq_buf::Kind::mapped};
    uint64_t n = 0;
    hipEvent_t ev_in = nullptr, ev_out = nullptr;
    bool busy = false;
    bool lists = false;
    bool replayed = false;
    bool copy_pending = false;
    const void* w_off_in_place = nullptr;
    const void* w_stream_in_place = nullptr;
    size_t w_stage_stream_off = 0;
    const void* msgs_in_place = nullptr;
    const void* outs_d = nullptr;
    uint64_t out_quads = 0;
    int end_bit = 0;
    uint32_t rec = 64;
    bool tail_zeroed = false;
    uint64_t tail_n = 0;
    uint32_t tail_rec = 0;
    const void* tail_dev = nullptr;
    uint64_t w_nbytes = 0;
// ... 24 lines not shown
  unsigned long long* wire_flags = nullptr;
  raftq_buf::Buffer<unsigned long long> wire_lb{raftq_buf::Kind::device};
  uint64_t wire_lb_tiles = 0;
  uint32_t wire_ticket_base = 0, wire_epoch = 0;
  uint32_t wire_chunk_base = 0, wire_chunk_pending = 0;
  bool wire_chunk_unknown = false;
  unsigned int prop_stamp = 0;
  raftq_buf::Buffer<uint8_t> prop_what{raftq_buf::Kind::mapped};
  uint64_t prop_what_n = 0;
  raftq_buf::Buffer<> resp_dev{raftq_buf::Kind::device};
  bool resp_on = false;
  uint32_t resp_stamp = 0;
  const uint64_t* resp_at_tail_d = nullptr;
  uint32_t resp_ent_base = 0;
  bool wal_pending = false, wal_pending_done = false;
  bool wal_pending_waited = false;
  uint64_t wal_pending_n = 0, wal_pending_cap = 0;
  uint32_t wal_pending_prev = 0;
  int wal_pending_rc = 0;
  raftq_wal_counts_t wal_pending_counts{};
  std::string wal_pending_err;
  std::string err;
  double prof[6] = {0, 0, 0, 0, 0, 0};
  uint64_t prof_n = 0;
};


struct raftq_set {
  template <class T>
  struct Dev : raftq_buf::Buffer<T> {
    Dev() : raftq_buf::Buffer<T>(raftq_buf::Kind::device) {}
  };
  int device = 0;
  uint32_t N = 0;
  uint64_t gpad = 0;
  std::vector<raftq_t*> members;
  hipStream_t stream = nullptr;
  Dev<raftqk::SweepArgs> tab[3];
  std::vector<raftqk::SweepArgs> tab_host;
  Dev<uint64_t> counts;
  Dev<uint64_t> np;
  std::vector<uint64_t> np_host;
  raftq_buf::Buffer<uint64_t> counts_h{raftq_buf::Kind::pinned};
  bool swept = false;
  bool broken = false;
  bool tab_stale = false;
  bool allow_voters = false;
  Dev<raftqk::VoterSweepArgs> vtab[3];
  std::vector<raftqk::VoterSweepArgs> vtab_host;
  unsigned last_flags = 0;
  int mode = 0;
  uint32_t persist_wgs = 0;
  hipEvent_t ev0 = nullptr, ev1 = nullptr;
  Dev<raftqk::TickArgs> tick_tab;
  std::vector<raftqk::TickArgs> tick_host;
  uint64_t tick_since = 0;
  Dev<raftqk::TickVotersArgs> tick_vtab;
  std::vector<raftqk::TickVotersArgs> tick_vhost;
  uint64_t tick_vsince = 0;
  std::string err;
};


struct raftq_wire_counts;
namespace raftqk {
struct NodeArrays;
}
namespace raftq_detail {
int node_arrays_of(raftq_t* h, raftqk::NodeArrays* out);
int fail(raftq_t* h, int code, const std::string& msg);
int use_device(raftq_t* h);
int use_device_idle(raftq_t* h, const char* who);
int refuse_voters(raftq_t* h, const char* who, bool step_family = false, bool tick_rounds = false, bool bcast = false);
inline void dense_changed(raftq_t* h) { h->node_mirror_fresh = false; }
inline bool masked_tick(const raftq_t* h) { return h->voters != nullptr && h->tick_voters; }
inline bool masked_bcast(const raftq_t* h) { return h->voters != nullptr && h->bcast_voters; }
int refuse_check_quorum(raftq_t* h, const char* who, bool fused = false);
int refuse_pre_vote(raftq_t* h, const char* who, bool fused = false);
int refuse_lead_transfer(raftq_t* h, const char* who);
int refuse_read_index(raftq_t* h, const char* who);
inline bool tick_checks(const raftq_t* h) { return h->cq != nullptr && h->tick_chk_cap != 0; }
int self_max_check(raftq_t* h);
int narrow_build(raftq_t* h);
int ensure_staging(raftq_t* h, size_t bytes);
int ensure_ingest(raftq_t* h, size_t bytes);
int ensure_tick_state(raftq_t* h);
void free_node_state(raftq_t* h);
void free_wire_state(raftq_t* h);
struct PackedDst {
  int form;
  uint32_t head_types;
  void* wide;
  uint64_t wide_cap;
};
int wire_frames_enqueue(raftq_t* h, const void* stream, uint64_t nbytes, const uint64_t* frame_off, uint64_t n, void* msgs, void* ents,
                        uint64_t ents_cap, void* msgs_d, int tail_appends, void* zero2 ,
                        const PackedDst* packed = nullptr);
uint64_t wire_frames_n_wide(raftq_t* h);
int wire_frames_finish(raftq_t* h, const uint64_t* frame_off, uint64_t n, bool have_ents, uint64_t ents_cap, ::raftq_wire_counts* counts);
struct RespPlan {
  uint64_t n = 0, n_max = 0, cap = 0;
  void* v_out = nullptr;
  uint64_t* v_resp_off = nullptr;
  uint64_t* peer_off = nullptr;
  bool lead = false;
  bool props = false;
  uint64_t ent_base = 0, nbytes = 0;
  const void* v_ents = nullptr;
  const void* v_stream = nullptr;
  size_t keep = 0, pool_off = 0;
};
int respond_prepare(raftq_t* h, const void* stream, uint64_t nbytes, const uint64_t* frame_off, const void* msgs, const void* ents,
                    uint64_t ents_cap, const uint64_t* at_tail, void* out, uint64_t cap, uint64_t* resp_off, uint64_t* peer_off, uint64_t n,
                    RespPlan* p);
int respond_enqueue(raftq_t* h, const RespPlan& p);
int respond_finish(raftq_t* h, const RespPlan& p, ::raftq_wire_counts* resp_counts);
struct TickLists {
  unsigned flags;
  uint64_t cap_h, cap_b, beat_at, map_off;
  const uint64_t* off_beat;
  const uint64_t* off_h = nullptr;
  uint64_t cap_c = 0, chk_off = 0;
};
int tick_lists_prepare(raftq_t* h, const char* who, unsigned flags, uint64_t hup_cap, uint64_t beat_cap, TickLists* tl);
int tick_lists_enqueue(raftq_t* h, TickLists* tl);
int tick_lists_finish(raftq_t* h, const char* who, const TickLists& tl, uint64_t* n_hup, uint64_t* n_beat);
int node_records_of(raftq_t* h, const char* who, raftqk::NodeArrays* out, bool tick_rounds = false, bool bcast = false);
int respond_pass_ok(raftq_t* h);
hipError_t wait_call(raftq_t* h);
}

#define HIPCHK(h, expr)                                                                        \
  do {                                                                                         \
    hipError_t _e = (expr);                                                                    \
    if (_e != hipSuccess) {                                                                    \
      return raftq_detail::fail((h), _e == hipErrorOutOfMemory ? RAFTQ_ENOMEM : RAFTQ_EHIP,    \
                                std::string(#expr) + ": " + hipGetErrorString(_e));            \
    }                                                                                          \
  } while (0)
```

raftsql_amd/csrc/raftq_kernels.hpp:

```cpp
#pragma once
#include <hip/hip_runtime.h>
#include <stdint.h>

#include <utility>

namespace raftqk {

typedef unsigned long long u64x2 __attribute__((ext_vector_type(2)));

constexpr int kBlock = 256;
constexpr int kWaves = kBlock / 64;
constexpr int kMaxPeers = 9;
constexpr int kTileMax = 2048;

struct __attribute__((aligned(64))) ReadRec {
  uint32_t seq;
  uint32_t acked[kMaxPeers];
  uint32_t pad[15 - kMaxPeers];
};
static_assert(sizeof(ReadRec) == 64, "one record per group, half a line");

struct SweepArgs {
  const uint64_t* match;
  const uint64_t* committed;
  uint64_t* committed_out;
  const uint64_t* first_idx;
  const uint8_t* votes;
  uint8_t* outcome;
  uint64_t* changed_bits;
  uint4* partials;
  uint64_t ld;
  const uint32_t* self_max = nullptr;
  const uint32_t* narrow = nullptr;
  const uint64_t* anchor = nullptr;
  const uint32_t* moff = nullptr;
};

constexpr uint32_t kSelfMaxValid = 0x80000000u;

constexpr uint32_t kNarrowValid = 1u;

template <typename T>
__device__ __forceinline__ void ce_desc(T& a, T& b) {
  const bool gt = a > b;
  const T hi = gt ? a : b;
  const T lo = gt ? b : a;
  a = hi;
  b = lo;
}

template <int N, typename T = uint64_t>
__device__ __forceinline__ T select_quorum_network(T (&v)[N]) {
#define CE(i, j) ce_desc(v[i], v[j])
  if constexpr (N == 2) { CE(0, 1); }
  if constexpr (N == 3) { CE(0, 2); CE(0, 1); CE(1, 2); }
  if constexpr (N == 4) { CE(0, 2); CE(1, 3); CE(0, 1); CE(2, 3); CE(1, 2); }
  if constexpr (N == 5) {
    CE(0, 3); CE(1, 4); CE(0, 2); CE(1, 3); CE(0, 1); CE(2, 4); CE(1, 2); CE(3, 4); CE(2, 3);
  }
  if constexpr (N == 6) {
    CE(0, 5); CE(1, 3); CE(2, 4); CE(1, 2); CE(3, 4); CE(0, 3);
    CE(2, 5); CE(0, 1); CE(2, 3); CE(4, 5); CE(1, 2); CE(3, 4);
  }
  if constexpr (N == 7) {
    CE(0, 6); CE(2, 3); CE(4, 5); CE(0, 2); CE(1, 4); CE(3, 6); CE(0, 1); CE(2, 5);
    CE(3, 4); CE(1, 2); CE(4, 6); CE(2, 3); CE(4, 5); CE(1, 2); CE(3, 4); CE(5, 6);
  }
  if constexpr (N == 8) {
    CE(0, 2); CE(1, 3); CE(4, 6); CE(5, 7); CE(0, 4); CE(1, 5); CE(2, 6); CE(3, 7); CE(0, 1); CE(2, 3);
    CE(4, 5); CE(6, 7); CE(2, 4); CE(3, 5); CE(1, 4); CE(3, 6); CE(1, 2); CE(3, 4); CE(5, 6);
  }
  if constexpr (N == 9) {
    CE(0, 3); CE(1, 7); CE(2, 5); CE(4, 8); CE(0, 7); CE(2, 4); CE(3, 8); CE(5, 6); CE(0, 2);
    CE(1, 3); CE(4, 5); CE(7, 8); CE(1, 4); CE(3, 6); CE(5, 7); CE(0, 1); CE(2, 4); CE(3, 5);
    CE(6, 8); CE(2, 3); CE(4, 5); CE(6, 7); CE(1, 2); CE(3, 4); CE(5, 6);
  }
#undef CE
  return v[N / 2];
}

template <int N>
__device__ __forceinline__ uint64_t select_other_network(uint64_t (&v)[N]) {
#define CE(i, j) ce_desc(v[i], v[j])
  if constexpr (N == 3) { CE(0, 1); }
  if constexpr (N == 4) { CE(0, 2); CE(0, 1); CE(1, 2); }
  if constexpr (N == 5) { CE(0, 2); CE(1, 3); CE(0, 1); CE(2, 3); CE(1, 2); }
  if constexpr (N == 6) {
    CE(0, 3); CE(1, 4); CE(0, 2); CE(1, 3); CE(0, 1); CE(2, 4); CE(1, 2); CE(3, 4); CE(2, 3);
  }
  if constexpr (N == 7) {
    CE(0, 5); CE(1, 3); CE(2, 4); CE(1, 2); CE(3, 4); CE(0, 3); CE(2, 5); CE(0, 1); CE(2, 3); CE(1, 2);
  }
  if constexpr (N == 8) {
    CE(0, 6); CE(2, 3); CE(4, 5); CE(0, 2); CE(1, 4); CE(3, 6); CE(0, 1);
    CE(2, 5); CE(3, 4); CE(1, 2); CE(4, 6); CE(2, 3); CE(4, 5); CE(3, 4);
  }
  if constexpr (N == 9) {
    CE(0, 2); CE(1, 3); CE(4, 6); CE(5, 7); CE(0, 4); CE(1, 5); CE(2, 6); CE(3, 7); CE(0, 1);
    CE(2, 3); CE(4, 5); CE(6, 7); CE(2, 4); CE(3, 5); CE(1, 4); CE(3, 6); CE(3, 4);
  }
#undef CE
  return v[N / 2 - 1];
}

template <int N>
__device__ __forceinline__ uint64_t select_quorum_oddeven(uint64_t (&v)[N]) {
#pragma unroll
  for (int r = 0; r < N; ++r) {
#pragma unroll
    for (int i = (r & 1); i + 1 < N; i += 2) ce_desc(v[i], v[i + 1]);
  }
  return v[N / 2];
}

template <bool GATED>
__device__ __forceinline__ uint64_t maybe_commit(uint64_t mci, uint64_t committed, uint64_t first_idx) {
  bool adv = mci > committed;
  if constexpr (GATED) adv = adv && (first_idx != 0) && (mci >= first_idx);
  return adv ? mci : committed;
}

__device__ __forceinline__ uint64_t bytes_equal(uint64_t v, uint64_t pattern) {
  const uint64_t k7f = 0x7f7f7f7f7f7f7f7full;
  const uint64_t x = v ^ pattern;
  uint64_t y = (x & k7f) + k7f;
  y = ~(y | x | k7f);
  return y >> 7;
}

__host__ __device__ constexpr int vote_word_bytes(int n_peers) { return n_peers <= 8 ? 2 : 4; }
typedef unsigned int u32x4p __attribute__((ext_vector_type(4)));

template <int N>
__device__ __forceinline__ uint32_t poll_word(uint32_t w) {
  constexpr uint32_t kLow = 0x55555555u & ((N >= 16) ? 0xffffffffu : ((1u << (2 * N)) - 1u));
  constexpr uint32_t q = N / 2 + 1;
  const uint32_t granted = __popc(w & ~(w >> 1) & kLow);
  const uint32_t rejected = __popc((w >> 1) & ~w & kLow);
  const uint32_t won = granted >= q ? 1u : 0u;
  const uint32_t lost = (won == 0u && rejected >= q) ? 2u : 0u;
  return won | lost;
}

template <typename T>
__device__ __forceinline__ T ld_stream(const T* p) {
  return __builtin_nontemporal_load(p);
}
template <typename T>
__device__ __forceinline__ void st_stream(T* p, T v) {
  __builtin_nontemporal_store(v, p);
}

#define RAFTQ_GLOBAL __attribute__((address_space(1)))
template <bool NT, typename T>
__device__ __forceinline__ T ldg(const T* p) {
  const RAFTQ_GLOBAL T* g = (const RAFTQ_GLOBAL T*)p;
  if constexpr (NT) return __builtin_nontemporal_load(g);
  else return *g;
}
template <bool NT, typename T>
__device__ __forceinline__ void stg(T* p, T v) {
  RAFTQ_GLOBAL T* g = (RAFTQ_GLOBAL T*)p;
  if constexpr (NT) __builtin_nontemporal_store(v, g);
  else *g = v;
}
typedef unsigned int u32x4 __attribute__((ext_vector_type(4)));
__device__ __forceinline__ void stg_u4(uint4* p, uint4 v) {
  u32x4 t;
  t.x = v.x; t.y = v.y; t.z = v.z; t.w = v.w;
  *(RAFTQ_GLOBAL u32x4*)p = t;
}

__device__ __forceinline__ uint32_t wave_sum_u32(uint32_t x) {
#pragma unroll
  for (int o = 32; o > 0; o >>= 1) x += __shfl_xor(x, o, 64);
  return x;
}

constexpr int kLdNT = 1, kStNT = 2, kNoStore = 4;
constexpr int kNoCompute = 8;

template <int N, int GPL, bool COMMIT, bool GATED, bool VOTES>
struct TileRegs {
  static constexpr int kRounds = GPL / 2;
  u64x2 m[COMMIT ? kRounds : 1][N];
  u64x2 c[COMMIT ? kRounds : 1];
  u64x2 f[COMMIT && GATED ? kRounds : 1];
  u32x4p vw[VOTES ? (N <= 8 ? 1 : 2) : 1];
  uint32_t skip = 0;
};

constexpr int kBodyAll = 0, kBodySkip = 1, kBodyNarrow = 2;
constexpr uint32_t kSkipNarrow = 0x100u;

template <int N, bool COMMIT>
__device__ __forceinline__ uint32_t self_max_skip(const SweepArgs& a) {
  if constexpr (!COMMIT || N < 2) {
    return 0;
  } else {
    if (a.self_max == nullptr) return 0;
    const uint32_t w = __builtin_amdgcn_readfirstlane(ldg<false>(a.self_max));
    return (w & kSelfMaxValid) != 0 ? (w & 0xffu) + 1 : 0;
  }
}

template <int N, bool COMMIT>
__device__ __forceinline__ uint32_t tile_body(const SweepArgs& a) {
  const uint32_t skip = self_max_skip<N, COMMIT>(a);
  if constexpr (!COMMIT || N < 3) {
    return skip;
  } else {
    if (N < 5 && skip != 0) return skip;
    if (a.narrow == nullptr) return skip;
    const uint32_t w = __builtin_amdgcn_readfirstlane(ldg<false>(a.narrow));
    return w == kNarrowValid ? kSkipNarrow : skip;
  }
}

template <int N, int GPL, bool COMMIT, bool GATED, bool VOTES, int POLICY, int BLOCK = kBlock, int BODY = kBodyAll>
__device__ __forceinline__ void tile_load(TileRegs<N, GPL, COMMIT, GATED, VOTES>& r, const SweepArgs& a,
                                          const uint32_t tile) {
  constexpr bool NT = (POLICY & kLdNT) != 0;
  constexpr int kTile = BLOCK * GPL;
  constexpr int kRounds = GPL / 2;
  constexpr bool SKIP = BODY == kBodySkip;
  constexpr int kRows = SKIP && N >= 2 ? N - 1 : N;
  static_assert(BODY != kBodyNarrow || N >= 3, "the narrow body is chosen from N = 3 (tile_body)");
  const uint32_t tid = threadIdx.x;
  const uint64_t tile0 = (uint64_t)tile * kTile;
  constexpr int kVoteLanes = kTile / 8;
  if constexpr (VOTES) {
    if (tid < kVoteLanes) {
      const uint8_t* src = a.votes + (tile0 + 8ull * tid) * vote_word_bytes(N);
      r.vw[0] = ldg<NT>(reinterpret_cast<const u32x4p*>(src));
      if constexpr (N > 8) r.vw[1] = ldg<NT>(reinterpret_cast<const u32x4p*>(src + 16));
    }
  }
  if constexpr (COMMIT) {
    const uint64_t* row[kRows];
#pragma unroll
    for (int p = 0; p < kRows; ++p) {
      const uint32_t slot = SKIP ? (uint32_t)p + ((uint32_t)p + 1 >= r.skip ? 1u : 0u) : (uint32_t)p;
      row[p] = a.match + (uint64_t)slot * a.ld;
    }
#pragma unroll
    for (int j = 0; j < kRounds; ++j) {
      const uint64_t g = tile0 + (uint64_t)(tid >> 6) * (64 * GPL) + (uint64_t)j * 128 + 2 * (tid & 63);
      if constexpr (BODY == kBodyNarrow) {
#pragma unroll
        for (int p = 0; p < N; ++p) {
          const uint64_t w = ldg<NT>(reinterpret_cast<const uint64_t*>(a.moff + (uint64_t)p * a.ld + g));
          if (p & 1) r.m[j][p >> 1].y = w;
          else r.m[j][p >> 1].x = w;
        }
        r.m[j][N - 1] = ldg<NT>(reinterpret_cast<const u64x2*>(a.anchor + g));
      } else {
#pragma unroll
        for (int p = 0; p < kRows; ++p) {
          r.m[j][p] = ldg<NT>(reinterpret_cast<const u64x2*>(row[p] + g));
        }
      }
      r.c[j] = ldg<NT>(reinterpret_cast<const u64x2*>(a.committed + g));
      if constexpr (GATED) r.f[j] = ldg<NT>(reinterpret_cast<const u64x2*>(a.first_idx + g));
    }
  }
}

template <int N, bool SKIP>
__device__ __forceinline__ uint64_t quorum_select(uint64_t (&v)[N]) {
  if constexpr (N == 1) return v[0];
  else if constexpr (SKIP) return select_other_network<N>(v);
  else return select_quorum_network<N>(v);
}

template <int N, int BODY, bool XOR, typename Regs>
__device__ __forceinline__ void tile_mci(const Regs& r, const int j, uint64_t& mci0, uint64_t& mci1) {
  if constexpr (BODY == kBodyNarrow) {
    uint32_t v0[N], v1[N];
#pragma unroll
    for (int p = 0; p < N; ++p) {
      const uint64_t w = (p & 1) ? r.m[j][p >> 1].y : r.m[j][p >> 1].x;
      v0[p] = (uint32_t)w;
      v1[p] = (uint32_t)(w >> 32);
    }
    uint32_t s0, s1;
    if constexpr (XOR) {
      s0 = v0[0];
      s1 = v1[0];
#pragma unroll
      for (int p = 1; p < N; ++p) {
        s0 ^= v0[p];
        s1 ^= v1[p];
      }
    } else {
      s0 = select_quorum_network<N, uint32_t>(v0);
      s1 = select_quorum_network<N, uint32_t>(v1);
    }
    mci0 = r.m[j][N - 1].x + s0;
    mci1 = r.m[j][N - 1].y + s1;
  } else {
    constexpr bool SKIP = BODY == kBodySkip;
    constexpr int kRows = SKIP && N >= 2 ? N - 1 : N;
    uint64_t v0[N], v1[N];
#pragma unroll
    for (int p = 0; p < kRows; ++p) {
      v0[p] = r.m[j][p].x;
      v1[p] = r.m[j][p].y;
    }
    if constexpr (XOR) {
      mci0 = v0[0];
      mci1 = v1[0];
#pragma unroll
      for (int p = 1; p < kRows; ++p) {
        mci0 ^= v0[p];
        mci1 ^= v1[p];
      }
    } else {
      mci0 = quorum_select<N, SKIP>(v0);
      mci1 = quorum_select<N, SKIP>(v1);
    }
  }
}

template <int N, int GPL, bool COMMIT, bool GATED, bool VOTES, int POLICY, bool BITS, int BLOCK = kBlock, int BODY = kBodyAll>
__device__ __forceinline__ void tile_finish(const TileRegs<N, GPL, COMMIT, GATED, VOTES>& r, const SweepArgs& a,
                                            const uint32_t tile) {
  constexpr bool STNT = (POLICY & kStNT) != 0;
  constexpr bool NOSTORE = (POLICY & kNoStore) != 0;
  constexpr int kTile = BLOCK * GPL;
  constexpr int kWavesB = BLOCK / 64;
  constexpr int kRounds = GPL / 2;
  const uint32_t tid = threadIdx.x;
  const uint64_t tile0 = (uint64_t)tile * kTile;
  uint32_t n_changed = 0;
  uint32_t won_lost = 0;
  constexpr int kVoteLanes = kTile / 8;
  const bool vote_lane = VOTES && tid < kVoteLanes;

  if constexpr (COMMIT) {
#pragma unroll
    for (int j = 0; j < kRounds; ++j) {
      const uint64_t g = tile0 + (uint64_t)(tid >> 6) * (64 * GPL) + (uint64_t)j * 128 + 2 * (tid & 63);
      uint64_t mci0, mci1;
      tile_mci<N, BODY, (POLICY & kNoCompute) != 0>(r, j, mci0, mci1);
      u64x2 o;
      if constexpr ((POLICY & kNoCompute) != 0) {
        o.x = mci0 ^ r.c[j].x;
        o.y = mci1 ^ r.c[j].y;
      } else {
        o.x = maybe_commit<GATED>(mci0, r.c[j].x, GATED ? r.f[j].x : 0);
        o.y = maybe_commit<GATED>(mci1, r.c[j].y, GATED ? r.f[j].y : 0);
      }
      const bool ch0 = o.x != r.c[j].x;
      const bool ch1 = o.y != r.c[j].y;
      const uint64_t b0 = __ballot(ch0);
      const uint64_t b1 = __ballot(ch1);
      n_changed += __popcll(b0) + __popcll(b1);
      if constexpr (BITS) {
        if (a.changed_bits != nullptr && (tid & 63) == 0) {
          u64x2 w;
          w.x = b0;
          w.y = b1;
          stg<false>(reinterpret_cast<u64x2*>(a.changed_bits + (g >> 6)), w);
        }
      }
      if constexpr (NOSTORE) {
        asm volatile("" ::"v"(o.x), "v"(o.y));
      } else {
        stg<STNT>(reinterpret_cast<u64x2*>(a.committed_out + g), o);
      }
    }
  }

  if constexpr (VOTES) {
    if (vote_lane) {
      const uint64_t g = tile0 + 8ull * tid;
      uint32_t out = 0, n_won = 0, n_lost = 0;
#pragma unroll
      for (int k = 0; k < 8; ++k) {
        uint32_t w;
        if constexpr (N <= 8) {
          const uint32_t pair = k < 2 ? r.vw[0].x : k < 4 ? r.vw[0].y : k < 6 ? r.vw[0].z : r.vw[0].w;
          w = (k & 1) ? pair >> 16 : pair & 0xffffu;
        } else {
          w = k == 0 ? r.vw[0].x : k == 1 ? r.vw[0].y : k == 2 ? r.vw[0].z : k == 3 ? r.vw[0].w
            : k == 4 ? r.vw[1].x : k == 5 ? r.vw[1].y : k == 6 ? r.vw[1].z : r.vw[1].w;
        }
        const uint32_t oc = poll_word<N>(w);
        out |= oc << (2 * k);
        n_won += oc & 1u;
        n_lost += oc >> 1;
      }
      uint16_t* dst = reinterpret_cast<uint16_t*>(a.outcome + (g >> 2));
      if constexpr (NOSTORE) {
        asm volatile("" ::"v"(out));
      } else {
        stg<STNT>(dst, (uint16_t)out);
      }
      won_lost = n_won | (n_lost << 16);
    }
  }

  const uint32_t wl = VOTES ? wave_sum_u32(won_lost) : 0u;
  if ((tid & 63) == 0) {
    uint4 t;
    t.x = n_changed;
    t.y = wl & 0xffffu;
    t.z = wl >> 16;
    t.w = 0;
    stg_u4(a.partials + ((uint64_t)tile * kWavesB + (tid >> 6)), t);
  }
}

template <int N, int GPL, bool COMMIT, bool GATED, bool VOTES, int POLICY, bool BITS, int BLOCK = kBlock>
__device__ __forceinline__ void sweep_tile(const SweepArgs& a, const uint32_t tile) {
  TileRegs<N, GPL, COMMIT, GATED, VOTES> r;
  r.skip = tile_body<N, COMMIT>(a);
  if constexpr (COMMIT && N >= 3) {
    if (r.skip == kSkipNarrow) {
      tile_load<N, GPL, COMMIT, GATED, VOTES, POLICY, BLOCK, kBodyNarrow>(r, a, tile);
      tile_finish<N, GPL, COMMIT, GATED, VOTES, POLICY, BITS, BLOCK, kBodyNarrow>(r, a, tile);
      return;
    }
  }
  if (r.skip != 0) {
    tile_load<N, GPL, COMMIT, GATED, VOTES, POLICY, BLOCK, kBodySkip>(r, a, tile);
    tile_finish<N, GPL, COMMIT, GATED, VOTES, POLICY, BITS, BLOCK, kBodySkip>(r, a, tile);
  } else {
    tile_load<N, GPL, COMMIT, GATED, VOTES, POLICY, BLOCK>(r, a, tile);
    tile_finish<N, GPL, COMMIT, GATED, VOTES, POLICY, BITS, BLOCK>(r, a, tile);
  }
}

template <int N, int GPL, bool COMMIT, bool GATED, bool VOTES, int POLICY, bool BITS, int BLOCK = kBlock>
static __global__ __launch_bounds__(BLOCK) void sweep_kernel(SweepArgs a) {
  sweep_tile<N, GPL, COMMIT, GATED, VOTES, POLICY, BITS, BLOCK>(a, blockIdx.x);
}

template <int N, int GPL, bool COMMIT, bool GATED, bool VOTES, int POLICY, bool BITS, int BLOCK = kBlock>
static __global__ __launch_bounds__(BLOCK) void sweep_set_kernel(const SweepArgs* __restrict__ tab, uint32_t want_bits) {
  SweepArgs a = tab[blockIdx.y];
  if (!want_bits) a.changed_bits = nullptr;
  sweep_tile<N, GPL, COMMIT, GATED, VOTES, POLICY, BITS, BLOCK>(a, blockIdx.x);
}

template <int N, int GPL, bool COMMIT, bool GATED, bool VOTES, int POLICY, bool BITS, int MINW = 1>
static __global__ __launch_bounds__(kBlock, MINW) void sweep_persist_kernel(const SweepArgs* __restrict__ tab,
                                                                      uint32_t tiles_per_member, uint32_t total_tiles,
                                                                      uint32_t want_bits) {
  using Regs = TileRegs<N, GPL, COMMIT, GATED, VOTES>;
  const uint32_t stride = gridDim.x;
  uint32_t t = blockIdx.x;
  if (t >= total_tiles) return;
  auto locate = [&](uint32_t lin, SweepArgs& a, uint32_t& tile) {
    const uint32_t m = lin / tiles_per_member;
    tile = lin - m * tiles_per_member;
    a = tab[m];
    if (!want_bits) a.changed_bits = nullptr;
  };
  auto load = [&](Regs& r, const SweepArgs& a, uint32_t tile) {
    r.skip = tile_body<N, COMMIT>(a);
    if constexpr (COMMIT && N >= 3) {
      if (r.skip == kSkipNarrow) {
        tile_load<N, GPL, COMMIT, GATED, VOTES, POLICY, kBlock, kBodyNarrow>(r, a, tile);
        return;
      }
    }
    if (r.skip != 0) tile_load<N, GPL, COMMIT, GATED, VOTES, POLICY, kBlock, kBodySkip>(r, a, tile);
    else tile_load<N, GPL, COMMIT, GATED, VOTES, POLICY>(r, a, tile);
  };
  auto finish = [&](const Regs& r, const SweepArgs& a, uint32_t tile) {
    if constexpr (COMMIT && N >= 3) {
      if (r.skip == kSkipNarrow) {
        tile_finish<N, GPL, COMMIT, GATED, VOTES, POLICY, BITS, kBlock, kBodyNarrow>(r, a, tile);
        return;
      }
    }
    if (r.skip != 0) tile_finish<N, GPL, COMMIT, GATED, VOTES, POLICY, BITS, kBlock, kBodySkip>(r, a, tile);
    else tile_finish<N, GPL, COMMIT, GATED, VOTES, POLICY, BITS>(r, a, tile);
  };
  Regs A, B;
  SweepArgs aA, aB;
  uint32_t tileA, tileB;
  locate(t, aA, tileA);
  load(A, aA, tileA);
  while (true) {
    t += stride;
    if (t >= total_tiles) {
      finish(A, aA, tileA);
      break;
    }
    locate(t, aB, tileB);
    load(B, aB, tileB);
    finish(A, aA, tileA);
    t += stride;
    if (t >= total_tiles) {
      finish(B, aB, tileB);
      break;
    }
    locate(t, aA, tileA);
    load(A, aA, tileA);
    finish(B, aB, tileB);
  }
}

static __global__ __launch_bounds__(kBlock) void set_counts_kernel(const SweepArgs* __restrict__ tab,
                                                                    const uint64_t* __restrict__ n_partials_of,
                                                                    uint64_t* __restrict__ out) {
  __shared__ uint64_t red[3][kWaves];
  const uint4* p = tab[blockIdx.x].partials;
  const uint64_t n_partials = n_partials_of[blockIdx.x];
  uint64_t c = 0, w = 0, l = 0;
  for (uint64_t i = threadIdx.x; i < n_partials; i += kBlock) {
    const uint4 v = p[i];
    c += v.x;
    w += v.y;
    l += v.z;
  }
#pragma unroll
  for (int o = 32; o > 0; o >>= 1) {
    c += __shfl_xor(c, o, 64);
    w += __shfl_xor(w, o, 64);
    l += __shfl_xor(l, o, 64);
  }
  if ((threadIdx.x & 63) == 0) {
    red[0][threadIdx.x >> 6] = c;
    red[1][threadIdx.x >> 6] = w;
    red[2][threadIdx.x >> 6] = l;
  }
  __syncthreads();
  if (threadIdx.x < 3) {
    uint64_t t = 0;
    for (int k = 0; k < kWaves; ++k) t += red[threadIdx.x][k];
    out[(uint64_t)blockIdx.x * 4 + threadIdx.x] = t;
  }
  if (threadIdx.x == 3) out[(uint64_t)blockIdx.x * 4 + 3] = 0;
}

typedef __attribute__((address_space(3))) void lds_void_t;
typedef const __attribute__((address_space(1))) void global_cvoid_t;

template <int N, int GPL, bool GATED, bool VOTES, bool BITS>
static __global__ __launch_bounds__(kBlock) void sweep_lds_kernel(SweepArgs a) {
  constexpr int kTile = kBlock * GPL;
// ... 99 lines not shown
  }
}

struct DeltaRec {
  uint64_t group, match;
  uint32_t peer, pad;
};
struct Delta16Rec {
  uint64_t match;
  uint32_t group, peer;
};
struct VoteDeltaRec {
  uint64_t group;
  uint32_t peer;
  uint8_t vote, pad[3];
};

constexpr unsigned long long kNoEpoch = ~0ull;
__device__ __forceinline__ bool batch_is_bad(const unsigned long long* bad, unsigned long long epoch_match,
                                             unsigned long long epoch_votes) {
  return bad[0] == epoch_match || bad[1] == epoch_votes;
}

static __global__ __launch_bounds__(kBlock) void self_max_check_kernel(const uint64_t* __restrict__ match, uint64_t ld,
                                                                       uint64_t n_groups, uint32_t n_peers, uint32_t slot,
                                                                       uint32_t* word) {
  bool broken = false;
  for (uint64_t g = (uint64_t)blockIdx.x * kBlock + threadIdx.x; g < n_groups; g += (uint64_t)gridDim.x * kBlock) {
    const uint64_t own = match[(uint64_t)slot * ld + g];
    for (uint32_t p = 0; p < n_peers; ++p) broken |= match[(uint64_t)p * ld + g] > own;
  }
  if (__ballot(broken) != 0 && (threadIdx.x & 63) == 0) *word = 0u;
}

__device__ __forceinline__ bool breaks_self_max(uint32_t w, const uint64_t* match, uint64_t ld, uint64_t group, uint32_t peer,
                                                uint64_t value) {
  if ((w & kSelfMaxValid) == 0) return false;
  const uint32_t slot = w & 0xffu;
  return peer != slot && value > match[(uint64_t)slot * ld + group];
}
__device__ __forceinline__ void clear_self_max_if(bool broken, uint32_t* word) {
  const uint64_t b = __ballot(broken);
  if (b != 0 && (threadIdx.x & 63) == (uint32_t)(__ffsll((unsigned long long)b) - 1)) *word = 0u;
}

static __global__ __launch_bounds__(kBlock) void narrow_build_kernel(const uint64_t* __restrict__ match, uint64_t ld,
                                                                     uint64_t n_groups, uint32_t n_peers,
                                                                     uint64_t* __restrict__ anchor, uint32_t* __restrict__ moff,
                                                                     uint32_t* word) {
  bool broken = false;
  for (uint64_t g = (uint64_t)blockIdx.x * kBlock + threadIdx.x; g < n_groups; g += (uint64_t)gridDim.x * kBlock) {
    uint64_t lo = match[g], hi = lo;
    for (uint32_t p = 1; p < n_peers; ++p) {
      const uint64_t v = match[(uint64_t)p * ld + g];
      lo = v < lo ? v : lo;
      hi = v > hi ? v : hi;
    }
    anchor[g] = lo;
    if (hi - lo > 0xffffffffull) {
      broken = true;
    } else {
      for (uint32_t p = 0; p < n_peers; ++p) moff[(uint64_t)p * ld + g] = (uint32_t)(match[(uint64_t)p * ld + g] - lo);
    }
  }
  if (__ballot(broken) != 0 && (threadIdx.x & 63) == 0) *word = 0u;
}

struct NarrowMirror {
  uint32_t* word;
  const uint64_t* anchor;
  uint32_t* moff;
};
__device__ __forceinline__ bool narrow_follow(uint32_t w, const NarrowMirror& m, uint64_t ld, uint64_t group, uint32_t peer,
                                              uint64_t value) {
  if (w != kNarrowValid) return false;
  const uint64_t base = m.anchor[group];
  if (value < base) return false;
  if (value - base > 0xffffffffull) return true;
  atomicMax(m.moff + (uint64_t)peer * ld + group, (uint32_t)(value - base));
  return false;
}
__device__ __forceinline__ void clear_narrow_if(bool broken, uint32_t* word) { clear_self_max_if(broken, word); }

template <typename Rec>
static __global__ __launch_bounds__(kBlock) void deltas_in_kernel(const Rec* __restrict__ src, Rec* __restrict__ dst,
                                                                  uint64_t n, uint64_t n_groups, uint32_t n_peers,
                                                                  unsigned long long* bad_epoch, uint64_t* bad_host,
                                                                  unsigned long long epoch) {
  const uint64_t i = (uint64_t)blockIdx.x * kBlock + threadIdx.x;
  bool bad = false;
  if (i < n) {
    const Rec r = src[i];
    dst[i] = r;
    bad = r.group >= n_groups || r.peer >= n_peers;
  }
  if (__ballot(bad) != 0 && (threadIdx.x & 63) == 0) {
    atomicMax(bad_epoch, epoch);
    *bad_host = epoch;
  }
}

template <typename Rec>
static __global__ __launch_bounds__(kBlock) void deltas_in_apply_kernel(const Rec* __restrict__ src, uint64_t n, uint64_t* match,
                                                                        uint64_t ld, uint64_t n_groups, uint32_t n_peers,
                                                                        unsigned long long* bad_epoch, uint64_t* bad_host,
                                                                        unsigned long long epoch, uint32_t* self_max,
                                                                        NarrowMirror mirror) {
  const uint64_t i = (uint64_t)blockIdx.x * kBlock + threadIdx.x;
  const uint32_t w = *self_max;
  const uint32_t nw = *mirror.word;
  bool bad = false, broken = false, wide = false;
  if (i < n) {
    const Rec r = src[i];
    bad = r.group >= n_groups || r.peer >= n_peers;
    if (!bad) {
      broken = breaks_self_max(w, match, ld, r.group, r.peer, r.match);
      wide = narrow_follow(nw, mirror, ld, r.group, r.peer, r.match);
      atomicMax(reinterpret_cast<unsigned long long*>(match + (uint64_t)r.peer * ld + r.group), (unsigned long long)r.match);
    }
  }
  clear_self_max_if(broken, self_max);
  clear_narrow_if(wide, mirror.word);
  if (__ballot(bad) != 0 && (threadIdx.x & 63) == 0) {
    atomicMax(bad_epoch, epoch);
    *bad_host = epoch;
  }
}

template <typename Rec>
static __global__ __launch_bounds__(kBlock) void apply_deltas_kernel(uint64_t* match, uint64_t ld,
                                                              const Rec* __restrict__ d, uint64_t n,
                                                              const unsigned long long* bad,
                                                              unsigned long long epoch_match, unsigned long long epoch_votes,
                                                              uint32_t* self_max, NarrowMirror mirror) {
  if (batch_is_bad(bad, epoch_match, epoch_votes)) return;
  const uint64_t i = (uint64_t)blockIdx.x * kBlock + threadIdx.x;
  const uint32_t w = *self_max;
  const uint32_t nw = *mirror.word;
  bool broken = false, wide = false;
  if (i < n) {
    const Rec r = d[i];
    broken = breaks_self_max(w, match, ld, r.group, r.peer, r.match);
    wide = narrow_follow(nw, mirror, ld, r.group, r.peer, r.match);
    atomicMax(reinterpret_cast<unsigned long long*>(match + (uint64_t)r.peer * ld + r.group),
              (unsigned long long)r.match);
  }
  clear_self_max_if(broken, self_max);
  clear_narrow_if(wide, mirror.word);
}

struct TermDeltaRec {
  uint64_t group, cur_term, first_idx_cur_term;
};
static __global__ __launch_bounds__(kBlock) void apply_term_deltas_kernel(uint64_t* first_idx,
                                                                   const TermDeltaRec* __restrict__ d, uint64_t n) {
  const uint64_t i = (uint64_t)blockIdx.x * kBlock + threadIdx.x;
  if (i >= n) return;
  const TermDeltaRec r = d[i];
  first_idx[r.group] = r.cur_term == 0 ? 0ull : r.first_idx_cur_term;
}

static __global__ __launch_bounds__(kBlock) void vote_deltas_in_kernel(const VoteDeltaRec* __restrict__ src,
                                                                       VoteDeltaRec* __restrict__ dst, uint64_t n,
                                                                       uint64_t n_groups, uint32_t n_peers,
                                                                       unsigned long long* bad_epoch, uint64_t* bad_host,
                                                                       unsigned long long epoch) {
  const uint64_t i = (uint64_t)blockIdx.x * kBlock + threadIdx.x;
  bool bad = false;
  if (i < n) {
    const VoteDeltaRec r = src[i];
    dst[i] = r;
    bad = r.group >= n_groups || r.peer >= n_peers || (unsigned)(r.vote - 1) > 1u;
  }
  if (__ballot(bad) != 0 && (threadIdx.x & 63) == 0) {
    atomicMax(bad_epoch, epoch);
    *bad_host = epoch;
  }
}

__device__ __forceinline__ bool vote_rec_ok(const VoteDeltaRec& r, uint64_t n_groups, uint32_t n_peers) {
  return r.group < n_groups && r.peer < n_peers && (unsigned)(r.vote - 1) <= 1u;
}

static __global__ __launch_bounds__(kBlock) void vote_claim_kernel(uint32_t* claim, uint64_t ld,
                                                            const VoteDeltaRec* __restrict__ d, uint64_t n,
                                                            const unsigned long long* bad, unsigned long long epoch_match,
                                                            unsigned long long epoch_votes, uint64_t n_groups,
                                                            uint32_t n_peers, int each) {
  if (!each && batch_is_bad(bad, epoch_match, epoch_votes)) return;
  const uint64_t i = (uint64_t)blockIdx.x * kBlock + threadIdx.x;
  if (i >= n) return;
  const VoteDeltaRec r = d[i];
  if (each && !vote_rec_ok(r, n_groups, n_peers)) return;
  atomicMin(claim + (uint64_t)r.peer * ld + r.group, (uint32_t)i);
}

static __global__ __launch_bounds__(kBlock) void vote_apply_kernel(uint8_t* votes, int wide, uint32_t* claim, uint64_t ld,
                                                            const VoteDeltaRec* __restrict__ d, uint64_t n,
                                                            const unsigned long long* bad, unsigned long long epoch_match,
                                                            unsigned long long epoch_votes, uint64_t n_groups,
                                                            uint32_t n_peers, int each) {
  if (!each && batch_is_bad(bad, epoch_match, epoch_votes)) return;
  const uint64_t i = (uint64_t)blockIdx.x * kBlock + threadIdx.x;
  if (i >= n) return;
  const VoteDeltaRec r = d[i];
  if (each && !vote_rec_ok(r, n_groups, n_peers)) return;
  const uint64_t slot = (uint64_t)r.peer * ld + r.group;
  if (claim[slot] != (uint32_t)i) return;
  unsigned int* word = reinterpret_cast<unsigned int*>(votes) + (wide ? r.group : r.group >> 1);
  const unsigned sh = (wide ? 0u : (unsigned)(r.group & 1ull) * 16u) + 2u * r.peer;
  const unsigned nv = (unsigned)r.vote << sh;
  unsigned old = *word;
  while (true) {
    const unsigned cur = (old >> sh) & 3u;
    if (cur == 1u || cur == 2u) break;
    const unsigned seen = atomicCAS(word, old, (old & ~(3u << sh)) | nv);
    if (seen == old) break;
    old = seen;
  }
  claim[slot] = 0xffffffffu;
}

struct Advance {
  uint64_t group, old_commit, new_commit;
};
struct Advance16 {
  uint64_t new_commit;
  uint32_t group, advanced_by;
};
__device__ __forceinline__ Advance make_advance(Advance*, uint64_t g, uint64_t o, uint64_t n) { return Advance{g, o, n}; }
__device__ __forceinline__ Advance16 make_advance(Advance16*, uint64_t g, uint64_t o, uint64_t n) {
  const uint64_t by = n - o;
  return Advance16{n, (uint32_t)g, by > 0xfffffffeull ? 0xffffffffu : (uint32_t)by};
}

static __global__ __launch_bounds__(1024) void scan_partials_kernel(const uint4* __restrict__ partials, uint64_t n_waves,
                                                             uint64_t* __restrict__ offsets, uint64_t* total, int field) {
  __shared__ uint64_t wave_tot[16];
  const uint32_t tid = threadIdx.x, lane = tid & 63, w = tid >> 6;
  const uint64_t per = (n_waves + 1023) / 1024;
  const uint64_t lo = (uint64_t)tid * per, hi = lo + per < n_waves ? lo + per : n_waves;
  const uint32_t* p32 = reinterpret_cast<const uint32_t*>(partials) + field;
  constexpr int kKeep = 8;
  uint32_t keep[kKeep];
  uint64_t sum = 0;
  if (per <= kKeep) {
#pragma unroll
    for (int k = 0; k < kKeep; ++k) keep[k] = (uint64_t)k < per && lo + k < hi ? p32[(lo + k) * 4] : 0u;
#pragma unroll
    for (int k = 0; k < kKeep; ++k) sum += keep[k];
  } else {
    for (uint64_t i = lo; i < hi; ++i) sum += p32[i * 4];
  }
  uint64_t incl = sum;
#pragma unroll
  for (int o = 1; o < 64; o <<= 1) {
    const uint64_t y = __shfl_up(incl, o, 64);
    if (lane >= (uint32_t)o) incl += y;
  }
  if (lane == 63) wave_tot[w] = incl;
  __syncthreads();
  uint64_t pre = 0;
  for (uint32_t k = 0; k < w; ++k) pre += wave_tot[k];
  uint64_t run = pre + incl - sum;
  if (per <= kKeep) {
#pragma unroll
    for (int k = 0; k < kKeep; ++k)
      if ((uint64_t)k < per && lo + k < hi) {
        offsets[lo + k] = run;
        run += keep[k];
      }
  } else {
    for (uint64_t i = lo; i < hi; ++i) {
      offsets[i] = run;
      run += p32[i * 4];
    }
  }
  if (tid == 1023) *total = pre + incl;
}

template <int GPL, typename Adv>
static __global__ __launch_bounds__(kBlock) void compact_changed_kernel(const uint64_t* changed_bits,
                                                                 const uint4* __restrict__ partials,
                                                                 const uint64_t* old_commit,
                                                                 const uint64_t* new_commit,
                                                                 Adv* out, uint64_t cap, uint64_t* total,
                                                                 const uint64_t* __restrict__ wave_offsets) {
  constexpr int kTile = kBlock * GPL;
  constexpr int kRounds = GPL / 2;
  __shared__ uint64_t red[kWaves];
  __shared__ uint32_t mine[kWaves];
  const uint32_t tid = threadIdx.x, lane = tid & 63, wave = tid >> 6;
  const uint64_t first_wave = (uint64_t)blockIdx.x * kWaves;
  const uint32_t* cnt = reinterpret_cast<const uint32_t*>(partials);
  uint64_t acc = 0;
  if (wave_offsets == nullptr) {
    uint32_t a0 = 0, a1 = 0, a2 = 0, a3 = 0;
    uint64_t i = tid;
    for (; i + 3 * kBlock < first_wave; i += 4 * kBlock) {
      a0 += cnt[4 * i];
      a1 += cnt[4 * (i + kBlock)];
      a2 += cnt[4 * (i + 2 * kBlock)];
      a3 += cnt[4 * (i + 3 * kBlock)];
    }
    for (; i < first_wave; i += kBlock) a0 += cnt[4 * i];
    acc = (uint64_t)a0 + a1 + a2 + a3;
#pragma unroll
    for (int o = 32; o > 0; o >>= 1) acc += __shfl_xor(acc, o, 64);
  } else if (lane == 0 && wave == 0) {
    acc = wave_offsets[first_wave];
  }
  if (lane == 0) red[wave] = acc;
  if (tid < kWaves) mine[tid] = cnt[4 * (first_wave + tid)];
  __syncthreads();
  uint64_t pos = 0;
#pragma unroll
  for (int k = 0; k < kWaves; ++k) pos += red[k];
  if (blockIdx.x == gridDim.x - 1 && tid == 0) {
    uint64_t t = pos;
    for (int k = 0; k < kWaves; ++k) t += mine[k];
    *total = t;
  }
  for (uint32_t k = 0; k < wave; ++k) pos += mine[k];
  const uint64_t below = lane == 0 ? 0ull : (~0ull >> (64 - lane));
#pragma unroll
  for (int j = 0; j < kRounds; ++j) {
    const uint64_t g0 = (uint64_t)blockIdx.x * kTile + (uint64_t)wave * (64 * GPL) + (uint64_t)j * 128;
    const uint64_t b0 = changed_bits[(g0 >> 6)];
    const uint64_t b1 = changed_bits[(g0 >> 6) + 1];
    const bool e = (b0 >> lane) & 1, o = (b1 >> lane) & 1;
    const uint64_t rank = __popcll(b0 & below) + __popcll(b1 & below);
    if (e) {
      const uint64_t g = g0 + 2 * lane, s = pos + rank;
      if (s < cap) out[s] = make_advance((Adv*)nullptr, g, old_commit[g], new_commit[g]);
    }
    if (o) {
      const uint64_t g = g0 + 2 * lane + 1, s = pos + rank + (e ? 1 : 0);
      if (s < cap) out[s] = make_advance((Adv*)nullptr, g, old_commit[g], new_commit[g]);
    }
    pos += __popcll(b0) + __popcll(b1);
  }
}

static __global__ void raise_flag_kernel(uint64_t* flag, uint64_t epoch) {
  if (threadIdx.x == 0 && blockIdx.x == 0) __hip_atomic_store(flag, epoch, __ATOMIC_RELAXED, __HIP_MEMORY_SCOPE_SYSTEM);
}

template <int N, int GPL, bool GATED, int POLICY>
static __global__ __launch_bounds__(kBlock) void sweep_segments_kernel(SweepArgs a, Advance16* list, unsigned int* counts_host, unsigned int* counts_dev) {
  constexpr bool STNT = (POLICY & kStNT) != 0;
  constexpr int kTile = kBlock * GPL;
  constexpr int kRounds = GPL / 2;
  __shared__ uint32_t wave_cnt[kWaves];
  const uint32_t tid = threadIdx.x, lane = tid & 63, wave = tid >> 6, tile = blockIdx.x;
  TileRegs<N, GPL, true, GATED, false> r;
  r.skip = tile_body<N, true>(a);
  const bool narrow = N >= 3 && r.skip == kSkipNarrow;
  if (narrow) {
    if constexpr (N >= 3) tile_load<N, GPL, true, GATED, false, POLICY, kBlock, kBodyNarrow>(r, a, tile);
  } else if (r.skip != 0) {
    tile_load<N, GPL, true, GATED, false, POLICY, kBlock, kBodySkip>(r, a, tile);
  } else {
    tile_load<N, GPL, true, GATED, false, POLICY>(r, a, tile);
  }
  const uint64_t tile0 = (uint64_t)tile * kTile;
  u64x2 nw[kRounds];
  uint64_t even[kRounds], odd[kRounds];
  uint32_t n_changed = 0;
#pragma unroll
  for (int j = 0; j < kRounds; ++j) {
    const uint64_t g = tile0 + (uint64_t)wave * (64 * GPL) + (uint64_t)j * 128 + 2 * lane;
    uint64_t mci0 = 0, mci1 = 0;
    if (narrow) {
      if constexpr (N >= 3) tile_mci<N, kBodyNarrow, false>(r, j, mci0, mci1);
    } else if (r.skip != 0) {
      tile_mci<N, kBodySkip, false>(r, j, mci0, mci1);
    } else {
      tile_mci<N, kBodyAll, false>(r, j, mci0, mci1);
    }
    u64x2 o;
    o.x = maybe_commit<GATED>(mci0, r.c[j].x, GATED ? r.f[j].x : 0);
    o.y = maybe_commit<GATED>(mci1, r.c[j].y, GATED ? r.f[j].y : 0);
    even[j] = __ballot(o.x != r.c[j].x);
    odd[j] = __ballot(o.y != r.c[j].y);
    n_changed += __popcll(even[j]) + __popcll(odd[j]);
    nw[j] = o;
    if (a.changed_bits != nullptr && lane == 0) {
      u64x2 w;
      w.x = even[j];
      w.y = odd[j];
      stg<false>(reinterpret_cast<u64x2*>(a.changed_bits + (g >> 6)), w);
    }
    stg<STNT>(reinterpret_cast<u64x2*>(a.committed_out + g), o);
  }
  if (lane == 0) {
    uint4 t;
    t.x = n_changed;
    t.y = t.z = t.w = 0;
    stg_u4(a.partials + ((uint64_t)tile * kWaves + wave), t);
    wave_cnt[wave] = n_changed;
  }
  __syncthreads();
  uint64_t pos = tile0;
  for (uint32_t k = 0; k < wave; ++k) pos += wave_cnt[k];
  if (tid == 0) {
    uint32_t tile_cnt = 0;
#pragma unroll
    for (int k = 0; k < kWaves; ++k) tile_cnt += wave_cnt[k];
    counts_host[tile] = tile_cnt;
    counts_dev[tile] = tile_cnt;
  }
  const uint64_t below = lane == 0 ? 0ull : (~0ull >> (64 - lane));
#pragma unroll
  for (int j = 0; j < kRounds; ++j) {
    const uint64_t g0 = tile0 + (uint64_t)wave * (64 * GPL) + (uint64_t)j * 128;
    const bool e = (even[j] >> lane) & 1, o = (odd[j] >> lane) & 1;
    const uint64_t rank = __popcll(even[j] & below) + __popcll(odd[j] & below);
    if (e) list[pos + rank] = make_advance((Advance16*)nullptr, g0 + 2 * lane, r.c[j].x, nw[j].x);
    if (o) list[pos + rank + (e ? 1 : 0)] = make_advance((Advance16*)nullptr, g0 + 2 * lane + 1, r.c[j].y, nw[j].y);
    pos += __popcll(even[j]) + __popcll(odd[j]);
  }
}

static __global__ __launch_bounds__(kBlock) void raise_flag_segments_kernel(uint64_t* flag, uint32_t epoch, const unsigned int* counts_dev, uint32_t n_tiles) {
  __shared__ uint32_t red[kWaves];
  uint32_t acc = 0;
  for (uint32_t i = threadIdx.x; i < n_tiles; i += kBlock) acc += counts_dev[i];
#pragma unroll
  for (int o = 32; o > 0; o >>= 1) acc += __shfl_xor(acc, o, 64);
  if ((threadIdx.x & 63) == 0) red[threadIdx.x >> 6] = acc;
  __syncthreads();
  if (threadIdx.x == 0) {
    uint32_t total = 0;
#pragma unroll
    for (int k = 0; k < kWaves; ++k) total += red[k];
    __hip_atomic_store(flag, ((uint64_t)epoch << 32) | total, __ATOMIC_RELAXED, __HIP_MEMORY_SCOPE_SYSTEM);
  }
}

// ... 29 lines not shown
  return (m | (m << 1)) & 0x55555555u;
}

__device__ __forceinline__ uint32_t poll_word_voters(uint32_t w, uint32_t mask) {
  const uint32_t low = spread_even(mask);
  const uint32_t q = ((uint32_t)__popc(mask) >> 1) + 1u;
  const uint32_t granted = __popc(w & ~(w >> 1) & low);
  const uint32_t rejected = __popc((w >> 1) & ~w & low);
  const uint32_t won = granted >= q ? 1u : 0u;
  const uint32_t lost = (won == 0u && rejected >= q) ? 2u : 0u;
  return won | lost;
}

template <int N, int GPL, bool COMMIT, bool GATED, bool VOTES, int POLICY>
static __global__ __launch_bounds__(kBlock) void sweep_voters_kernel(VoterSweepArgs va) {
#define RAFTQ_VT_PROLOGUE      \
  const SweepArgs& a = va.s; \
  const uint32_t tid = threadIdx.x, tile = blockIdx.x;
#define RAFTQ_VT_VMASK(at) ldg<NT>(reinterpret_cast<const u32x4p*>(va.voters + at))
#define RAFTQ_VT_CMASK(j, at) ldg<NT>(reinterpret_cast<const uint32_t*>(va.voters + at))
#include "raftq_sweep_voters_tile.inc"
#undef RAFTQ_VT_PROLOGUE
#undef RAFTQ_VT_VMASK
#undef RAFTQ_VT_CMASK
}

template <int GPL, bool COMMIT>
struct TileMasks {
  u32x4p v;
  uint32_t c[COMMIT ? GPL / 2 : 1];
};
template <int N, int GPL, bool COMMIT, bool VOTES, bool NT>
__device__ __forceinline__ void tile_masks(TileMasks<GPL, COMMIT>& m, const uint16_t* voters , const uint32_t tile) {
  constexpr int kTile = kBlock * GPL;
  constexpr uint32_t kFullPair = ((1u << N) - 1u) * 0x10001u;
  const uint32_t tid = threadIdx.x;
  if (voters != nullptr) {
    const uint16_t* const base = voters + (uint64_t)tile * kTile;
    if constexpr (VOTES) {
      if (tid < kTile / 8) m.v = ldg<NT>(reinterpret_cast<const u32x4p*>(base + 8u * tid));
    }
    if constexpr (COMMIT) {
#pragma unroll
      for (int j = 0; j < GPL / 2; ++j) {
        const uint32_t g = (tid >> 6) * (64 * GPL) + (uint32_t)j * 128 + 2 * (tid & 63);
        m.c[j] = ldg<NT>(reinterpret_cast<const uint32_t*>(base + g));
      }
    }
  } else {
    m.v.x = m.v.y = m.v.z = m.v.w = kFullPair;
#pragma unroll
    for (int j = 0; j < (COMMIT ? GPL / 2 : 1); ++j) m.c[j] = kFullPair;
  }
}
template <int N, int GPL, bool COMMIT, bool GATED, bool VOTES, int POLICY>
static __global__ __launch_bounds__(kBlock) void sweep_set_voters_kernel(const VoterSweepArgs* __restrict__ tab, uint32_t want_bits) {
#define RAFTQ_VT_PROLOGUE                                 \
  VoterSweepArgs va = tab[blockIdx.y];                    \
  if (!want_bits) va.s.changed_bits = nullptr;            \
  const SweepArgs& a = va.s;                              \
  const uint32_t tid = threadIdx.x, tile = blockIdx.x;    \
  TileMasks<GPL, COMMIT> tm;                              \
  tile_masks<N, GPL, COMMIT, VOTES, NT>(tm, va.voters, tile);
#define RAFTQ_VT_VMASK(at) tm.v
#define RAFTQ_VT_CMASK(j, at) tm.c[j]
#include "raftq_sweep_voters_tile.inc"
#undef RAFTQ_VT_PROLOGUE
#undef RAFTQ_VT_VMASK
#undef RAFTQ_VT_CMASK
}

static __global__ __launch_bounds__(kBlock) void fill_voters_kernel(uint16_t* voters, uint64_t n_groups, uint16_t full) {
  const uint64_t g = (uint64_t)blockIdx.x * kBlock + threadIdx.x;
  if (g < n_groups) voters[g] = full;
}

struct VoterDeltaRec {
  uint64_t group;
  uint16_t voters, reset;
  uint32_t pad;
};
static __global__ __launch_bounds__(kBlock) void apply_voter_deltas_kernel(uint16_t* voters, uint64_t* match, uint64_t ld, uint8_t* votes,
                                                                           int wide, uint32_t n_peers, const VoterDeltaRec* __restrict__ d,
                                                                           uint64_t n, uint32_t* self_max, uint32_t* narrow) {
  const uint64_t i = (uint64_t)blockIdx.x * kBlock + threadIdx.x;
  bool resets = false;
  if (i < n) {
    const VoterDeltaRec r = d[i];
    voters[r.group] = r.voters;
    resets = r.reset != 0;
    if (resets) {
      const uint32_t fields = spread_even(r.reset) * 3u;
      for (uint32_t p = 0; p < n_peers; ++p)
        if ((r.reset >> p) & 1u) match[(uint64_t)p * ld + r.group] = 0ull;
      if (wide) reinterpret_cast<uint32_t*>(votes)[r.group] &= ~fields;
      else reinterpret_cast<uint16_t*>(votes)[r.group] &= (uint16_t)~fields;
    }
  }
  clear_self_max_if(resets, self_max);
  clear_narrow_if(resets, narrow);
}

struct TickArgs {
  const uint8_t* role;
  uint32_t* elapsed;
  uint8_t* action;
  uint64_t* hup_bits;
  uint64_t* beat_bits;
  uint4* partials;
  uint64_t n_groups;
  uint64_t seed, tick_no;
  uint32_t election_tick, heartbeat_tick;
  uint32_t et_magic;
};

__device__ __forceinline__ uint64_t tick_key(uint64_t seed, uint64_t tick_no) {
  uint64_t z = seed ^ (tick_no * 0xD1B54A32D192ED03ull);
  z += 0x9E3779B97F4A7C15ull;
  z = (z ^ (z >> 30)) * 0xBF58476D1CE4E5B9ull;
  z = (z ^ (z >> 27)) * 0x94D049BB133111EBull;
  return z ^ (z >> 31);
}
__device__ __forceinline__ uint32_t tick_rand(uint64_t key, uint32_t group ) {
  uint32_t x = group ^ (uint32_t)key;
  x ^= x >> 16;
  x *= 0x85EBCA6Bu;
  x ^= x >> 13;
  x *= 0xC2B2AE35u;
  x ^= x >> 16;
  return x ^ (uint32_t)(key >> 32);
}

__device__ __forceinline__ uint32_t tick_mod(uint32_t x, uint32_t d, uint32_t magic) {
  uint32_t r = x - __umulhi(x, magic) * d;
  r = r >= d ? r - d : r;
  return r >= d ? r - d : r;
}

template <int L>
__device__ __forceinline__ uint32_t write_lane(uint32_t v, uint32_t x ) {
  asm("v_writelane_b32 %0, %1, %2" : "+v"(v) : "s"(x), "n"(L));
  return v;
}

__device__ __forceinline__ void tick_chunk_out(const TickArgs& a, uint64_t chunk , uint32_t lane, const uint64_t (&hb)[4],
                                               const uint64_t (&bb)[4], uint32_t n_hup, uint32_t n_beat) {
  uint32_t v = 0;
  v = write_lane<0>(v, (uint32_t)hb[0]);  v = write_lane<1>(v, (uint32_t)(hb[0] >> 32));
  v = write_lane<2>(v, (uint32_t)hb[1]);  v = write_lane<3>(v, (uint32_t)(hb[1] >> 32));
  v = write_lane<4>(v, (uint32_t)hb[2]);  v = write_lane<5>(v, (uint32_t)(hb[2] >> 32));
  v = write_lane<6>(v, (uint32_t)hb[3]);  v = write_lane<7>(v, (uint32_t)(hb[3] >> 32));
  v = write_lane<8>(v, (uint32_t)bb[0]);  v = write_lane<9>(v, (uint32_t)(bb[0] >> 32));
  v = write_lane<10>(v, (uint32_t)bb[1]); v = write_lane<11>(v, (uint32_t)(bb[1] >> 32));
  v = write_lane<12>(v, (uint32_t)bb[2]); v = write_lane<13>(v, (uint32_t)(bb[2] >> 32));
  v = write_lane<14>(v, (uint32_t)bb[3]); v = write_lane<15>(v, (uint32_t)(bb[3] >> 32));
  v = write_lane<16>(v, n_hup);
  v = write_lane<17>(v, n_beat);
  const uint64_t at_hup = (uint64_t)(uintptr_t)a.hup_bits + chunk * 32 + 4ull * lane;
  const uint64_t at_beat = (uint64_t)(uintptr_t)a.beat_bits + chunk * 32 + 4ull * lane - 32;
  const uint64_t at_part = (uint64_t)(uintptr_t)a.partials + chunk * 16 + 4ull * lane - 64;
  const uint64_t at = lane < 8 ? at_hup : (lane < 16 ? at_beat : at_part);
  if (lane < 20) stg<false>(reinterpret_cast<uint32_t*>((uintptr_t)at), v);
}

template <int R, bool NT = false>
__device__ __forceinline__ void tick_tile(const TickArgs& a, uint64_t n_blocks) {
  const uint32_t tid = threadIdx.x, lane = tid & 63, wave = tid >> 6;
  const uint64_t key = tick_key(a.seed, a.tick_no);
  uint32_t roles[R];
  uint4 el[R];
#pragma unroll
  for (int r = 0; r < R; ++r) {
    const uint64_t blk = (uint64_t)blockIdx.x * R + r;
    if (blk < n_blocks) {
      const uint64_t g = (blk * kBlock + tid) * 4;
      roles[r] = ldg<NT>(reinterpret_cast<const uint32_t*>(a.role + g));
      const u32x4 v = ldg<NT>(reinterpret_cast<const u32x4*>(a.elapsed + g));
      el[r].x = v.x; el[r].y = v.y; el[r].z = v.z; el[r].w = v.w;
    }
  }
#pragma unroll
  for (int r = 0; r < R; ++r) {
    const uint64_t blk = (uint64_t)blockIdx.x * R + r;
// ... 292 lines not shown
    pos_b += mine[1][k];
  }
  const uint64_t wv = first_wave + wave;
  const uint64_t below = lane == 0 ? 0ull : (~0ull >> (64 - lane));
  uint64_t hb[4], bb[4];
#pragma unroll
  for (int k = 0; k < 4; ++k) {
    hb[k] = hup_bits[wv * 4 + k];
    bb[k] = beat_bits[wv * 4 + k];
  }
  uint64_t rh = pos_h + __popcll(hb[0] & below) + __popcll(hb[1] & below) + __popcll(hb[2] & below) + __popcll(hb[3] & below);
  uint64_t rb = pos_b + __popcll(bb[0] & below) + __popcll(bb[1] & below) + __popcll(bb[2] & below) + __popcll(bb[3] & below);
#pragma unroll
  for (int k = 0; k < 4; ++k) {
    const uint64_t g = wv * 256 + 4ull * lane + k;
    if ((hb[k] >> lane) & 1) {
      if (rh < hup_cap) hup_out[rh] = g;
      ++rh;
    }
    if ((bb[k] >> lane) & 1) {
      if (rb < beat_cap) beat_out[rb] = g;
      ++rb;
    }
  }
}

__device__ __forceinline__ void run_out(uint32_t* out, uint64_t cap, uint64_t pos, const uint32_t* ids , uint32_t n, uint32_t tid) {
  if (pos >= cap) return;
  if (pos + n > cap) n = (uint32_t)(cap - pos);
  const uint32_t head = (uint32_t)((4 - (pos & 3)) & 3) < n ? (uint32_t)((4 - (pos & 3)) & 3) : n;
  const uint32_t quads = (n - head) >> 2;
  if (tid < head) out[pos + tid] = ids[tid];
  for (uint32_t q = tid; q < quads; q += kBlock) {
    const uint32_t i = head + 4 * q;
    u32x4 v;
    v.x = ids[i]; v.y = ids[i + 1]; v.z = ids[i + 2]; v.w = ids[i + 3];
    *reinterpret_cast<u32x4*>(out + pos + i) = v;
  }
  const uint32_t done = head + 4 * quads;
  if (tid < n - done) out[pos + done + tid] = ids[done + tid];
}

#define RAFTQ_LISTS_KERNEL tick_lists32_kernel
#define RAFTQ_LISTS_N 2
#define RAFTQ_LISTS_PARAM
#define RAFTQ_LISTS_CHK(...)
#include "raftq_tick_lists32.inc"
#undef RAFTQ_LISTS_KERNEL
#undef RAFTQ_LISTS_N
#undef RAFTQ_LISTS_PARAM
#undef RAFTQ_LISTS_CHK
struct TickChecksArgs {
  const uint64_t* chk_bits;
  uint32_t* chk_out;
  uint64_t chk_cap;
  const uint64_t* wave_off_chk;
};
#define RAFTQ_LISTS_KERNEL tick_lists32_checks_kernel
#define RAFTQ_LISTS_N 3
#define RAFTQ_LISTS_PARAM , TickChecksArgs c
#define RAFTQ_LISTS_CHK(...) __VA_ARGS__
#include "raftq_tick_lists32.inc"
#undef RAFTQ_LISTS_KERNEL
#undef RAFTQ_LISTS_N
#undef RAFTQ_LISTS_PARAM
#undef RAFTQ_LISTS_CHK

constexpr int kTickSetRounds = 4;
static __global__ __launch_bounds__(kBlock) void tick_set_kernel(const TickArgs* __restrict__ tab, uint64_t ticks_since, uint64_t n_blocks) {
  TickArgs a = tab[blockIdx.y];
  a.tick_no += ticks_since;
  tick_tile<kTickSetRounds, true>(a, n_blocks);
}
constexpr int kTickWideBlocks = 1;
template <int R>
static __global__ __launch_bounds__(kBlock) void tick_set_wide_kernel(const TickArgs* __restrict__ tab, uint64_t ticks_since, uint64_t n_blocks) {
  TickArgs a = tab[blockIdx.y];
  a.tick_no += ticks_since;
  tick_tile_wide<R, true>(a, n_blocks);
}

static __global__ __launch_bounds__(kBlock) void campaign_kernel(uint8_t* role, uint32_t* elapsed, uint8_t* votes,
                                                          uint32_t n_peers, uint32_t self_peer,
                                                          const uint64_t* __restrict__ groups, uint64_t n) {
  const uint64_t i = (uint64_t)blockIdx.x * kBlock + threadIdx.x;
  if (i >= n) return;
  const uint64_t g = groups[i];
  role[g] = 1;
  elapsed[g] = 0;
  if (n_peers <= 8) reinterpret_cast<uint16_t*>(votes)[g] = (uint16_t)(1u << (2 * self_peer));
  else reinterpret_cast<uint32_t*>(votes)[g] = 1u << (2 * self_peer);
}

}
```

raftsql_amd/csrc/raftq_step_kernels.hpp:

```cpp
#pragma once
#include <hip/hip_runtime.h>
#include <stdint.h>

#include "raftq_kernels.hpp"

namespace raftqk {

struct MsgRec {
  uint64_t group, term, log_term, index, commit, reject_hint;
  uint32_t from;
  uint8_t type, reject, pad[2];
  uint64_t resv;
};
struct StepOutRec {
  uint64_t group, term, index, log_term, commit, last_index;
  uint32_t to, vote, lead;
  uint8_t type, reject, flags, role;
};
struct LogDeltaRec {
  uint64_t group, last_index, last_term, commit_to;
};
struct StepOutC {
  uint64_t term, index, commit, aux;
  uint8_t vote, lead, type, reject, flags, role, pad[2];
// ... 229 lines not shown
  for (uint32_t k = 0; k < (uint32_t)kMaxPeers; ++k)
    if (k == p && ack[k] < c) {
      ack[k] = c;
      raised = true;
    }
  if (raised) rec->acked[p] = c;
  const uint32_t after = read_confirmed(ack, members, q);
  if (op == kReadRequest) return (uint64_t)seq | ((uint64_t)(after >= seq ? 1u : 0u) << 32);
  return after > before ? after : 0;
}

template <bool MASKED, bool LEAD = false, bool CQ = false, bool RI = false>
struct NodeT {
  static_assert(CQ || !RI, "the read rules live in the CQ form");
  const NodeArrays& a;
  uint64_t g;
  uint64_t term, last_index, last_term, committed, first_idx;
  uint64_t mt[kMaxPeers];
  uint32_t mt_dirty = 0;
  uint32_t vote, lead;
  uint32_t vw = 0;
  uint32_t lst_head, lst_cnt, lst_min;
  uint8_t role;
  bool held = false;
  bool at_tail = false, host_owns = false;
  uint64_t committed0, first_idx0;
  uint8_t role0;
  bool vw_known = false, vw_dirty = false, elapsed_reset = false;
  uint32_t vmask = 0;
  uint64_t last_term_was = 0;
  uint32_t cqw = 0;
  bool cq_known = false, cq_dirty = false;
  ReadRec* reads = nullptr;
  bool rd_zeroed = false;

  __device__ NodeT(const NodeArrays& arr, uint64_t group, const uint16_t* voters = nullptr, ReadRec* read_recs = nullptr) : a(arr), g(group) {
    if constexpr (RI) reads = read_recs;
    if constexpr (MASKED) vmask = voters[g];
    const NodeRec r = a.rec[g];
    term = r.term; last_index = r.last_index; last_term = r.last_term;
    vote = r.vote; lead = r.lead;
    lst_head = r.lst_head; lst_cnt = r.lst_cnt; lst_min = r.lst_min;
    committed = committed0 = r.committed;
    first_idx = first_idx0 = r.first_idx;
    role = role0 = r.role;
#pragma unroll
    for (int p = 0; p < kMaxPeers; ++p) mt[p] = r.match[p];
    if (a.at_tail != nullptr) at_tail = ((a.at_tail[g >> 6] >> (g & 63)) & 1ull) != 0;
  }
  __device__ void store(bool list_reset = true) const {
    NodeRec r;
    r.term = term; r.last_index = last_index; r.last_term = last_term;
    r.vote = (uint8_t)vote; r.lead = (uint8_t)lead;
    r.role = role; r.pad = 0;
    r.lst_head = list_reset ? kNil : lst_head;
    r.lst_cnt = list_reset ? 0u : lst_cnt;
    r.lst_min = list_reset ? kNil : lst_min;
    r.committed = committed;
    r.first_idx = first_idx;
#pragma unroll
    for (int p = 0; p < kMaxPeers; ++p) r.match[p] = mt[p];
    a.rec[g] = r;
    if (committed != committed0) a.committed[g] = committed;
    if (role != role0) a.role[g] = role;
    if (first_idx != first_idx0) a.first_idx[g] = first_idx;
#pragma unroll
    for (int p = 0; p < kMaxPeers; ++p)
      if ((mt_dirty >> p) & 1u) a.match[(uint64_t)p * a.ld + g] = mt[p];
    if (mt_dirty != 0 && a.self_max != nullptr) {
      const uint32_t w = *a.self_max;
      if ((w & kSelfMaxValid) != 0) {
        const uint64_t own = match(w & 0xffu);
        bool broken = false;
#pragma unroll
        for (uint32_t p = 0; p < (uint32_t)kMaxPeers; ++p) broken |= p < a.n_peers && mt[p] > own;
        if (broken) *a.self_max = 0u;
      }
    }
    if (mt_dirty != 0 && a.self_max != nullptr && a.self_max[1] != 0u) a.self_max[1] = 0u;
    if (elapsed_reset) a.elapsed[g] = 0;
    if (vw_dirty) {
      if (a.n_peers <= 8) reinterpret_cast<uint16_t*>(a.votes)[g] = (uint16_t)vw;
      else reinterpret_cast<uint32_t*>(a.votes)[g] = vw;
    }
    if constexpr (CQ)
      if (cq_dirty) a.cq[g] = cqw;
  }
  __device__ void set_cq(uint32_t w) {
    cqw = w;
    cq_known = cq_dirty = true;
  }
  __device__ uint32_t get_cq() {
    if (!cq_known) {
      cqw = a.cq[g];
      cq_known = true;
    }
    return cqw;
  }
  __device__ bool in_lease() const {
    return role == kLeader || (lead != 0 && (elapsed_reset ? 0u : a.elapsed[g]) < a.election_tick);
  }
  __device__ void set_first_idx(uint64_t v) { first_idx = v; }
  __device__ uint64_t get_first_idx() const { return first_idx; }
  __device__ void set_votes(uint32_t w) {
    vw = w;
    vw_known = vw_dirty = true;
  }
  __device__ uint32_t get_votes() {
    if (!vw_known) {
      vw = a.n_peers <= 8 ? (uint32_t)reinterpret_cast<const uint16_t*>(a.votes)[g] : reinterpret_cast<const uint32_t*>(a.votes)[g];
      vw_known = true;
    }
    return vw;
  }
  __device__ uint64_t match(uint32_t p) const {
    uint64_t v = 0;
#pragma unroll
    for (uint32_t k = 0; k < (uint32_t)kMaxPeers; ++k) v = k == p ? mt[k] : v;
    return v;
  }
  __device__ void set_match(uint32_t p, uint64_t v) {
#pragma unroll
    for (uint32_t k = 0; k < (uint32_t)kMaxPeers; ++k) mt[k] = k == p ? v : mt[k];
    mt_dirty |= 1u << p;
  }
  __device__ __forceinline__ uint8_t ri() const {
    if constexpr (RI) return a.ri;
    else return 0;
  }
  __device__ __forceinline__ uint32_t read_members() const {
    if constexpr (MASKED) return vmask;
    else return (1u << a.n_peers) - 1u;
  }
  __device__ __forceinline__ uint64_t read_op(uint32_t op, uint32_t p = 0, uint32_t c = 0) {
    rd_zeroed = op == kReadClear;
    return read_rule(reads + g, op, p, c, read_members(), quorum());
  }
  __device__ uint32_t quorum() const {
    if constexpr (MASKED) return ((uint32_t)__popc(vmask) >> 1) + 1u;
    else return a.n_peers / 2 + 1;
  }
  __device__ bool counts(uint32_t p, uint32_t n) const {
    if constexpr (MASKED) return ((vmask >> p) & 1u) != 0;
    else return p < n;
  }

  __device__ void reset(uint64_t t) {
    if (term != t) { term = t; vote = 0; }
    lead = 0;
    elapsed_reset = true;
    set_votes(0);
    if constexpr (CQ) {
      set_cq(0);
      if (ri() == kReadSafe && !rd_zeroed) (void)read_op(kReadClear);
    }
#pragma unroll
    for (uint32_t p = 0; p < (uint32_t)kMaxPeers; ++p)
      if (p < a.n_peers) {
        const uint64_t v = p == a.self ? last_index : 0;
        if (mt[p] != v) mt_dirty |= 1u << p;
        mt[p] = v;
      }
  }
  __device__ void become_follower(uint64_t t, uint32_t new_lead) {
    reset(t);
    lead = new_lead;
// ... 571 lines not shown
```

raftsql_amd/engine.py:

```python
from __future__ import annotations

import ctypes as C
from dataclasses import dataclass
from typing import Optional

import numpy as np

from . import _lib
from ._lib import (SWEEP_CACHED, SWEEP_CHANGED, SWEEP_COMMIT, SWEEP_GATED, SWEEP_LDS, SWEEP_NO_ADOPT,
                   SWEEP_STREAM, SWEEP_VOTES, Advance, Counts, Delta, RaftqError, VoteDelta)

__all__ = ["QuorumEngine", "SweepSet", "sweep_many_async", "SweepCounts", "device_count", "RaftqError", "pinned_empty", "pinned_copy", "SWEEP_COMMIT", "SWEEP_GATED",
           "SWEEP_VOTES", "SWEEP_NO_ADOPT", "SWEEP_LDS", "SWEEP_CHANGED", "SWEEP_STREAM", "SWEEP_CACHED"]


@dataclass
class SweepCounts:
    n_changed: int
    n_won: int
    n_lost: int


def device_count() -> int:
    lib = _lib.load()
# ... 268 lines not shown
        nv = 0 if vote_deltas is None else len(vote_deltas)
        n = C.c_uint64(0)
        self._chk(self._lib.raftq_cycle(
            self._h, _ptr(deltas) if nd else None, nd, _ptr(vote_deltas) if nv else None, nv, flags,
            None, int(cap), C.byref(n), None))
        return int(n.value)

    def cycle(self, flags: int, deltas: Optional[np.ndarray] = None, vote_deltas: Optional[np.ndarray] = None,
              cap: Optional[int] = None, out: Optional[np.ndarray] = None, want_counts: bool = True):
        nd = 0 if deltas is None else len(deltas)
        nv = 0 if vote_deltas is None else len(vote_deltas)
        if nd:
            assert deltas.dtype == self._DELTA_DT and deltas.flags.c_contiguous
        if nv:
            assert vote_deltas.dtype == self._VDELTA_DT and vote_deltas.flags.c_contiguous
        cap = (self.n_groups if cap is None else int(cap))
        if out is None:
            out = np.empty(cap, dtype=self._ADV_DT)
        n = C.c_uint64(0)
        c = Counts()
        self._chk(self._lib.raftq_cycle(
            self._h, _ptr(deltas) if nd else None, nd, _ptr(vote_deltas) if nv else None, nv, flags,
            _ptr(out) if cap else None, cap, C.byref(n), C.byref(c) if want_counts else None))
        total = int(n.value)
        cnt = SweepCounts(int(c.n_changed), int(c.n_won), int(c.n_lost)) if want_counts else None
        return out[: min(total, cap)], total, cnt

    def step_async(self, flags: int) -> None:
        self._chk(self._lib.raftq_step_async(self._h, flags))

    def wait(self, want_counts: bool = False) -> Optional[SweepCounts]:
        if not want_counts:
            self._chk(self._lib.raftq_wait(self._h, None))
            return None
        c = Counts()
        self._chk(self._lib.raftq_wait(self._h, C.byref(c)))
        return SweepCounts(int(c.n_changed), int(c.n_won), int(c.n_lost))

    def sweep(self, flags: int) -> SweepCounts:
        self.step_async(flags)
        return self.wait(want_counts=True)

    def commit_advance(self, gated: bool = False):
        out = np.empty(self.n_groups, dtype=np.uint64)
        n = C.c_uint64(0)
        self._chk(self._lib.raftq_commit_advance(self._h, int(gated), _ptr(out), C.byref(n)))
        return out, int(n.value)

    def vote_tally(self):
        out = np.empty(self.n_groups, dtype=np.uint8)
        c = Counts()
        self._chk(self._lib.raftq_vote_tally(self._h, _ptr(out), C.byref(c)))
        return out, SweepCounts(int(c.n_changed), int(c.n_won), int(c.n_lost))

    def read_committed(self) -> np.ndarray:
        out = np.empty(self.n_groups, dtype=np.uint64)
        self._chk(self._lib.raftq_read_committed(self._h, _ptr(out)))
        return out

    def read_outcome(self) -> np.ndarray:
        out = np.empty(self.n_groups, dtype=np.uint8)
        self._chk(self._lib.raftq_read_outcome(self._h, _ptr(out)))
        return out

    def read_match(self) -> np.ndarray:
        out = np.empty((self.n_peers, self.n_groups), dtype=np.uint64)
        self._chk(self._lib.raftq_read_match(self._h, _ptr(out)))
        return out

    def self_max(self) -> int:
        s = C.c_int32(-1)
        self._chk(self._lib.raftq_self_max(self._h, C.byref(s)))
        return int(s.value)

    def narrow(self) -> bool:
        v = C.c_int32(0)
        self._chk(self._lib.raftq_narrow(self._h, C.byref(v)))
        return bool(v.value)

    def narrow_rebuild(self) -> bool:
        self._chk(self._lib.raftq_narrow_rebuild(self._h))
        return self.narrow()

    def read_votes(self) -> np.ndarray:
        out = np.empty((self.n_peers, self.n_groups), dtype=np.uint8)
        self._chk(self._lib.raftq_read_votes(self._h, _ptr(out)))
        return out

    def collect_changed(self, cap: Optional[int] = None):
        cap = self.n_groups if cap is None else int(cap)
        arr = (Advance * cap)()
        n = C.c_uint64(0)
        self._chk(self._lib.raftq_collect_changed(self._h, C.addressof(arr) if cap else None, cap, C.byref(n)))
        a = np.frombuffer(arr, dtype=np.dtype([("group", "<u8"), ("old_commit", "<u8"), ("new_commit", "<u8")]))
        return a[: min(int(n.value), cap)].copy(), int(n.value)

    def set_timers(self, election_tick: int = 10, heartbeat_tick: int = 1, seed: int = 0x1000) -> None:
        self._chk(self._lib.raftq_set_timers(self._h, election_tick, heartbeat_tick, seed))

    def load_roles(self, role: np.ndarray, elapsed: Optional[np.ndarray] = None) -> None:
        r = np.ascontiguousarray(role, dtype=np.uint8)
        if r.shape != (self.n_groups,):
            raise ValueError("role must be [G]")
        e = None if elapsed is None else np.ascontiguousarray(elapsed, dtype=np.uint32)
        self._chk(self._lib.raftq_load_roles(self._h, _ptr(r), _ptr(e) if e is not None else None))

    def tick(self, want_counts: bool = True):
        if not want_counts:
            self._chk(self._lib.raftq_tick(self._h, None))
            return None
        c = _lib.TickCounts()
        self._chk(self._lib.raftq_tick(self._h, C.byref(c)))
        return int(c.n_hup), int(c.n_beat)

    def read_tick(self):
        a = np.empty(self.n_groups, dtype=np.uint8)
        e = np.empty(self.n_groups, dtype=np.uint32)
        r = np.empty(self.n_groups, dtype=np.uint8)
        self._chk(self._lib.raftq_read_tick(self._h, _ptr(a), _ptr(e), _ptr(r)))
        return a, e, r

    def collect_hups(self, cap: Optional[int] = None):
        cap = self.n_groups if cap is None else int(cap)
        out = np.empty(cap, dtype=np.uint64)
        n = C.c_uint64(0)
        self._chk(self._lib.raftq_collect_hups(self._h, _ptr(out) if cap else None, cap, C.byref(n)))
        return out[: min(cap, int(n.value))], int(n.value)

    def collect_beats(self, cap: Optional[int] = None):
        cap = self.n_groups if cap is None else int(cap)
        out = np.empty(cap, dtype=np.uint64)
        n = C.c_uint64(0)
        self._chk(self._lib.raftq_collect_beats(self._h, _ptr(out) if cap else None, cap, C.byref(n)))
        return out[: min(cap, int(n.value))], int(n.value)

    def set_check_quorum(self, on=True) -> None:
        self._chk(self._lib.raftq_set_check_quorum(self._h, int(on)))

    def set_pre_vote(self, on=True) -> None:
        self._chk(self._lib.raftq_set_pre_vote(self._h, int(on)))

    def set_lead_transfer(self, on=True) -> None:
        self._chk(self._lib.raftq_set_lead_transfer(self._h, int(on)))

    def load_transfer(self, transferee: np.ndarray) -> None:
        t = np.ascontiguousarray(transferee, dtype=np.uint8)
        if t.shape != (self.n_groups,):
            raise ValueError("transferee must be [G]")
        self._chk(self._lib.raftq_load_transfer(self._h, _ptr(t)))

    def read_transfer(self) -> np.ndarray:
        t = np.empty(self.n_groups, dtype=np.uint8)
        self._chk(self._lib.raftq_read_transfer(self._h, _ptr(t)))
        return t

    def set_read_index(self, mode=_lib.READ_SAFE) -> None:
        self._chk(self._lib.raftq_set_read_index(self._h, int(mode)))

    def load_reads(self, seq: Optional[np.ndarray] = None, acked: Optional[np.ndarray] = None) -> None:
        s = None if seq is None else np.ascontiguousarray(seq, dtype=np.uint32)
        a = None if acked is None else np.ascontiguousarray(acked, dtype=np.uint32)
        if s is not None and s.shape != (self.n_groups,):
            raise ValueError("seq must be [G]")
        if a is not None and a.shape != (self.n_peers, self.n_groups):
            raise ValueError("acked must be [N][G]")
        self._chk(self._lib.raftq_load_reads(self._h, None if s is None else _ptr(s), None if a is None else _ptr(a)))
# ... 164 lines not shown
```

Measured before the change: 130.3 billion.

## Maintain per-group vote tally bytes so the vote sweep reads one byte per group

After: 133.4 billion, median of 6. +2.4%, better.

```diff
diff --git a/go/raftq/engine_more.go b/go/raftq/engine_more.go
--- a/go/raftq/engine_more.go
+++ b/go/raftq/engine_more.go
@@ -28,6 +28,22 @@
 }
 
 func (e *Engine) NarrowRebuild() error { return e.err(C.raftq_narrow_rebuild(e.h)) }
+
+func (e *Engine) Tally() (bool, error) {
+	var valid C.int32_t
+	if err := e.err(C.raftq_tally(e.h, &valid)); err != nil {
+		return false, err
+	}
+	return valid != 0, nil
+}
+
+func (e *Engine) TallyRebuild() (bool, error) {
+	var valid C.int32_t
+	if err := e.err(C.raftq_tally_rebuild(e.h, &valid)); err != nil {
+		return false, err
+	}
+	return valid != 0, nil
+}
 
 func (e *Engine) SetStream(stream unsafe.Pointer) error { return e.err(C.raftq_set_stream(e.h, stream)) }
 func (e *Engine) Stream() unsafe.Pointer                { return C.raftq_get_stream(e.h) }
diff --git a/include/raftq.h b/include/raftq.h
--- a/include/raftq.h
+++ b/include/raftq.h
@@ -122,6 +122,8 @@
 int raftq_self_max(raftq_t* h, int32_t* slot_out);
 int raftq_narrow(raftq_t* h, int32_t* valid_out);
 int raftq_narrow_rebuild(raftq_t* h);
+int raftq_tally(raftq_t* h, int32_t* valid_out);
+int raftq_tally_rebuild(raftq_t* h, int32_t* valid_out);
 int raftq_read_votes(raftq_t* h, uint8_t* votes_out );
 int raftq_collect_changed(raftq_t* h, raftq_advance_t* out, uint64_t cap, uint64_t* n);
 
diff --git a/raftsql_amd/_lib.py b/raftsql_amd/_lib.py
--- a/raftsql_amd/_lib.py
+++ b/raftsql_amd/_lib.py
@@ -81,6 +81,8 @@
     ("raftq_self_max", C.c_int, [_H, C.POINTER(C.c_int32)]),
     ("raftq_narrow", C.c_int, [_H, C.POINTER(C.c_int32)]),
     ("raftq_narrow_rebuild", C.c_int, [_H]),
+    ("raftq_tally", C.c_int, [_H, C.POINTER(C.c_int32)]),
+    ("raftq_tally_rebuild", C.c_int, [_H, C.POINTER(C.c_int32)]),
     ("raftq_read_votes", C.c_int, [_H, C.c_void_p]),
     ("raftq_collect_changed", C.c_int, [_H, C.c_void_p, C.c_uint64, C.POINTER(C.c_uint64)]),
     ("raftq_set_timers", C.c_int, [_H, C.c_uint32, C.c_uint32, C.c_uint64]),
diff --git a/raftsql_amd/csrc/raftq_capi.hip b/raftsql_amd/csrc/raftq_capi.hip
--- a/raftsql_amd/csrc/raftq_capi.hip
+++ b/raftsql_amd/csrc/raftq_capi.hip
@@ -253,6 +253,20 @@
   const uint64_t blocks = std::min<uint64_t>((h->G + kBlock - 1) / kBlock, 4096);
   hipLaunchKernelGGL(narrow_build_kernel, dim3((unsigned)std::max<uint64_t>(blocks, 1)), dim3(kBlock), 0, h->stream,
                      (const uint64_t*)h->match, h->ld, h->G, h->N, h->anchor, h->moff, h->narrow_word());
+  HIPCHK(h, hipGetLastError());
+  return RAFTQ_OK;
+}
+int raftq_detail::tally_build(raftq_t* h) {
+  if (int rc = use_device(h)) return rc;
+  if (!h->tally) return RAFTQ_OK;
+  if (h->step_collected != h->step_submitted) {
+    HIPCHK(h, hipMemsetAsync(h->tally_word(), 0, sizeof(uint32_t), h->stream));
+    return RAFTQ_OK;
+  }
+  HIPCHK(h, hipMemsetD32Async((hipDeviceptr_t)h->tally_word(), (int)kTallyValid, 1, h->stream));
+  const uint64_t blocks = std::min<uint64_t>((h->G + kBlock - 1) / kBlock, 4096);
+  hipLaunchKernelGGL(tally_build_kernel, dim3((unsigned)std::max<uint64_t>(blocks, 1)), dim3(kBlock), 0, h->stream,
+                     (const uint8_t*)h->votes, h->G, h->N, h->tally);
   HIPCHK(h, hipGetLastError());
   return RAFTQ_OK;
 }
@@ -372,6 +386,18 @@
     }
     e = hipMemsetD32Async((hipDeviceptr_t)h->self_max, (int)(kSelfMaxValid | 0u), 1, h->stream);
     if (e != hipSuccess) { rc = fail(h, RAFTQ_EHIP, std::string("hipMemsetD32Async: ") + hipGetErrorString(e)); break; }
+    {
+      const char* tl = std::getenv("RAFTQ_TALLY");
+      if (!(tl && std::strcmp(tl, "0") == 0)) {
+        e = raftq_buf::alloc_group({{(void**)&h->tally, (size_t)ld}}, h->stream);
+        if (e != hipSuccess) {
+          rc = fail(h, e == hipErrorOutOfMemory ? RAFTQ_ENOMEM : RAFTQ_EHIP, std::string("device arrays: ") + hipGetErrorString(e));
+          break;
+        }
+        e = hipMemsetD32Async((hipDeviceptr_t)h->tally_word(), (int)kTallyValid, 1, h->stream);
+        if (e != hipSuccess) { rc = fail(h, RAFTQ_EHIP, std::string("hipMemsetD32Async: ") + hipGetErrorString(e)); break; }
+      }
+    }
     e = raftq_buf::alloc_group({{(void**)&h->h_partials, h->max_partials * sizeof(uint4), raftq_buf::Kind::pinned},
                                 {(void**)&h->h_total, 64, raftq_buf::Kind::mapped_coherent, (void**)&h->d_total}},
                                h->stream);
@@ -416,7 +442,7 @@
   raftq_detail::free_node_state(h);
   raftq_detail::free_wire_state(h);
   raftq_buf::free_device(h->match, h->committed[0], h->committed[1], h->first_idx, h->votes, h->voters, h->outcome, h->changed_bits,
-                         h->partials, h->offsets, h->self_max, h->anchor, h->moff, h->claim, h->delta_bad, h->role, h->elapsed, h->action, h->hup_bits,
+                         h->partials, h->offsets, h->self_max, h->anchor, h->moff, h->tally, h->claim, h->delta_bad, h->role, h->elapsed, h->action, h->hup_bits,
                          h->beat_bits, h->tick_partials, h->tick_offsets2, h->tick_offsets3, h->cq, h->chk_bits, h->reads);
   raftq_buf::free_host(h->h_partials, h->h_total);
   if (h->ev0) (void)hipEventDestroy(h->ev0);
@@ -490,6 +516,7 @@
   if (wb == 2) pack_votes(votes, h->G, h->N, reinterpret_cast<uint16_t*>(packed.data()));
   else pack_votes(votes, h->G, h->N, reinterpret_cast<uint32_t*>(packed.data()));
   HIPCHK(h, hipMemcpyAsync(h->votes, packed.data(), packed.size(), hipMemcpyHostToDevice, h->stream));
+  if (int rc = raftq_detail::tally_build(h)) return rc;
   HIPCHK(h, hipStreamSynchronize(h->stream));
   return RAFTQ_OK;
 }
@@ -568,7 +595,7 @@
     hipLaunchKernelGGL(vote_claim_kernel, gv, dim3(kBlock), 0, h->stream, h->claim, h->ld, (const VoteDeltaRec*)dev_v, nv, bad,
                        em_gate, ev, h->G, h->N, trusted ? 1 : 0);
     hipLaunchKernelGGL(vote_apply_kernel, gv, dim3(kBlock), 0, h->stream, h->votes, h->N > 8 ? 1 : 0, h->claim, h->ld,
-                       (const VoteDeltaRec*)dev_v, nv, bad, em_gate, ev, h->G, h->N, trusted ? 1 : 0);
+                       (const VoteDeltaRec*)dev_v, nv, bad, em_gate, ev, h->G, h->N, trusted ? 1 : 0, h->tally_mirror());
   }
   HIPCHK(h, hipGetLastError());
   return RAFTQ_OK;
@@ -722,7 +749,8 @@
   }
   dense_changed(h);
   hipLaunchKernelGGL(apply_voter_deltas_kernel, dim3((unsigned)((m + kBlock - 1) / kBlock)), dim3(kBlock), 0, h->stream, h->voters, h->match,
-                     h->ld, h->votes, h->N > 8 ? 1 : 0, h->N, (const VoterDeltaRec*)h->stage.d, m, h->self_max, h->narrow_word());
+                     h->ld, h->votes, h->N > 8 ? 1 : 0, h->N, (const VoterDeltaRec*)h->stage.d, m, h->self_max, h->narrow_word(),
+                     h->tally_word());
   HIPCHK(h, hipGetLastError());
   HIPCHK(h, hipStreamSynchronize(h->stream));
   return RAFTQ_OK;
@@ -762,6 +790,8 @@
   a.narrow = h->anchor ? h->narrow_word() : nullptr;
   a.anchor = h->anchor;
   a.moff = h->moff;
+  a.tally_word = h->tally ? h->tally_word() : nullptr;
+  a.tally = h->tally;
   return a;
 }
 
@@ -917,6 +947,24 @@
 int raftq_narrow_rebuild(raftq_t* h) {
   if (int rc = use_device_idle(h, "raftq_narrow_rebuild")) return rc;
   if (int rc = raftq_detail::narrow_build(h)) return rc;
+  HIPCHK(h, hipStreamSynchronize(h->stream));
+  return RAFTQ_OK;
+}
+
+int raftq_tally(raftq_t* h, int32_t* valid) {
+  if (int rc = use_device_idle(h, "raftq_tally")) return rc;
+  if (!valid) return fail(h, RAFTQ_EINVAL, "raftq_tally: null argument");
+  uint32_t w = 0;
+  HIPCHK(h, hipMemcpyAsync(&w, h->tally_word(), sizeof w, hipMemcpyDeviceToHost, h->stream));
+  HIPCHK(h, hipStreamSynchronize(h->stream));
+  *valid = w == kTallyValid ? 1 : 0;
+  return RAFTQ_OK;
+}
+
+int raftq_tally_rebuild(raftq_t* h, int32_t* valid) {
+  if (int rc = use_device_idle(h, "raftq_tally_rebuild")) return rc;
+  if (int rc = raftq_detail::tally_build(h)) return rc;
+  if (valid) return raftq_tally(h, valid);
   HIPCHK(h, hipStreamSynchronize(h->stream));
   return RAFTQ_OK;
 }
@@ -1647,7 +1695,7 @@
   if (int rc = ensure_staging(h, (size_t)n * 8)) return rc;
   std::memcpy(h->stage.h, groups, n * 8);
   hipLaunchKernelGGL(campaign_kernel, dim3((unsigned)((n + kBlock - 1) / kBlock)), dim3(kBlock), 0, h->stream,
-                     h->role, h->elapsed, h->votes, h->N, self_peer, (const uint64_t*)h->stage.d, n);
+                     h->role, h->elapsed, h->votes, h->N, self_peer, (const uint64_t*)h->stage.d, n, h->tally);
   dense_changed(h);
   HIPCHK(h, hipGetLastError());
   HIPCHK(h, hipStreamSynchronize(h->stream));
@@ -2373,6 +2421,12 @@
   } else {
     HIPCHK(dst, hipMemsetAsync(dst->narrow_word(), 0, sizeof(uint32_t), dst->stream));
   }
+  if (src->tally && dst->tally) {
+    HIPCHK(dst, hipMemcpyAsync(dst->tally, src->tally, ld, hipMemcpyDeviceToDevice, dst->stream));
+    HIPCHK(dst, hipMemcpyAsync(dst->tally_word(), src->tally_word(), sizeof(uint32_t), hipMemcpyDeviceToDevice, dst->stream));
+  } else {
+    HIPCHK(dst, hipMemsetAsync(dst->tally_word(), 0, sizeof(uint32_t), dst->stream));
+  }
   if (src->voters) HIPCHK(dst, hipMemcpyAsync(dst->voters, src->voters, ld * sizeof(uint16_t), hipMemcpyDeviceToDevice, dst->stream));
   if (src->cq && dst->cq) HIPCHK(dst, hipMemcpyAsync(dst->cq, src->cq, ld * sizeof(uint32_t), hipMemcpyDeviceToDevice, dst->stream));
   if (src->reads && dst->reads) HIPCHK(dst, hipMemcpyAsync(dst->reads, src->reads, ld * sizeof(raftqk::ReadRec), hipMemcpyDeviceToDevice, dst->stream));
diff --git a/raftsql_amd/csrc/raftq_internal.hpp b/raftsql_amd/csrc/raftq_internal.hpp
--- a/raftsql_amd/csrc/raftq_internal.hpp
+++ b/raftsql_amd/csrc/raftq_internal.hpp
@@ -56,6 +56,9 @@
   bool narrow_off = false;
   uint32_t* narrow_word() const { return self_max + 1; }
   raftqk::NarrowMirror narrow_mirror() const { return raftqk::NarrowMirror{self_max + 1, anchor, moff}; }
+  uint8_t* tally = nullptr;
+  uint32_t* tally_word() const { return self_max + 2; }
+  raftqk::TallyMirror tally_mirror() const { return raftqk::TallyMirror{self_max + 2, tally}; }
   uint64_t compact_epoch = 0;
   uint64_t compact_epoch_armed = 0;
   uint32_t flag_misses[2] = {0, 0}, flag_rested[2] = {0, 0};
@@ -246,6 +249,7 @@
 inline bool tick_checks(const raftq_t* h) { return h->cq != nullptr && h->tick_chk_cap != 0; }
 int self_max_check(raftq_t* h);
 int narrow_build(raftq_t* h);
+int tally_build(raftq_t* h);
 int ensure_staging(raftq_t* h, size_t bytes);
 int ensure_ingest(raftq_t* h, size_t bytes);
 int ensure_tick_state(raftq_t* h);
diff --git a/raftsql_amd/csrc/raftq_kernels.hpp b/raftsql_amd/csrc/raftq_kernels.hpp
--- a/raftsql_amd/csrc/raftq_kernels.hpp
+++ b/raftsql_amd/csrc/raftq_kernels.hpp
@@ -34,11 +34,15 @@
   const uint32_t* narrow = nullptr;
   const uint64_t* anchor = nullptr;
   const uint32_t* moff = nullptr;
+  const uint32_t* tally_word = nullptr;
+  const uint8_t* tally = nullptr;
 };
 
 constexpr uint32_t kSelfMaxValid = 0x80000000u;
 
 constexpr uint32_t kNarrowValid = 1u;
+
+constexpr uint32_t kTallyValid = 1u;
 
 template <typename T>
 __device__ __forceinline__ void ce_desc(T& a, T& b) {
@@ -142,6 +146,18 @@
   return won | lost;
 }
 
+__device__ __forceinline__ uint32_t tally_of_word(uint32_t w, uint32_t n_peers) {
+  const uint32_t low = 0x55555555u & (n_peers >= 16 ? 0xffffffffu : ((1u << (2 * n_peers)) - 1u));
+  return __popc(w & ~(w >> 1) & low) | (__popc((w >> 1) & ~w & low) << 4);
+}
+template <int N>
+__device__ __forceinline__ uint32_t poll_tally(uint32_t b) {
+  constexpr uint32_t q = N / 2 + 1;
+  const uint32_t won = (b & 15u) >= q ? 1u : 0u;
+  const uint32_t lost = (won == 0u && (b >> 4) >= q) ? 2u : 0u;
+  return won | lost;
+}
+
 template <typename T>
 __device__ __forceinline__ T ld_stream(const T* p) {
   return __builtin_nontemporal_load(p);
@@ -188,33 +204,55 @@
   u64x2 f[COMMIT && GATED ? kRounds : 1];
   u32x4p vw[VOTES ? (N <= 8 ? 1 : 2) : 1];
   uint32_t skip = 0;
+  bool tally = false;
 };
 
 constexpr int kBodyAll = 0, kBodySkip = 1, kBodyNarrow = 2;
 constexpr uint32_t kSkipNarrow = 0x100u;
 
+struct HandleWords {
+  uint32_t self_max = 0, narrow = 0, tally = 0;
+};
+template <int N, bool COMMIT, bool VOTES>
+__device__ __forceinline__ HandleWords handle_words(const SweepArgs& a) {
+  HandleWords hw;
+  if constexpr ((COMMIT && N >= 2) || VOTES) {
+    if (a.self_max == nullptr) return hw;
+    const u32x4p w = ldg<false>(reinterpret_cast<const u32x4p*>(a.self_max));
+    hw.self_max = __builtin_amdgcn_readfirstlane(w.x);
+    if (a.narrow != nullptr) hw.narrow = __builtin_amdgcn_readfirstlane(w.y);
+    if (VOTES && a.tally_word != nullptr) hw.tally = __builtin_amdgcn_readfirstlane(w.z);
+  }
+  return hw;
+}
+
 template <int N, bool COMMIT>
-__device__ __forceinline__ uint32_t self_max_skip(const SweepArgs& a) {
+__device__ __forceinline__ uint32_t self_max_skip(const HandleWords& hw) {
   if constexpr (!COMMIT || N < 2) {
     return 0;
   } else {
-    if (a.self_max == nullptr) return 0;
-    const uint32_t w = __builtin_amdgcn_readfirstlane(ldg<false>(a.self_max));
-    return (w & kSelfMaxValid) != 0 ? (w & 0xffu) + 1 : 0;
-  }
-}
-
-template <int N, bool COMMIT>
+    return (hw.self_max & kSelfMaxValid) != 0 ? (hw.self_max & 0xffu) + 1 : 0;
+  }
+}
+
+constexpr uint32_t kBodyTally = 0x200u;
+template <int N, bool COMMIT, bool VOTES = false>
 __device__ __forceinline__ uint32_t tile_body(const SweepArgs& a) {
-  const uint32_t skip = self_max_skip<N, COMMIT>(a);
+  const HandleWords hw = handle_words<N, COMMIT, VOTES>(a);
+  const uint32_t tally = VOTES && hw.tally == kTallyValid ? kBodyTally : 0u;
+  const uint32_t skip = self_max_skip<N, COMMIT>(hw);
   if constexpr (!COMMIT || N < 3) {
-    return skip;
+    return skip | tally;
   } else {
-    if (N < 5 && skip != 0) return skip;
-    if (a.narrow == nullptr) return skip;
-    const uint32_t w = __builtin_amdgcn_readfirstlane(ldg<false>(a.narrow));
-    return w == kNarrowValid ? kSkipNarrow : skip;
-  }
+    if (N < 5 && skip != 0) return skip | tally;
+    return (hw.narrow == kNarrowValid ? kSkipNarrow : skip) | tally;
+  }
+}
+template <int N, bool COMMIT, bool VOTES, typename Regs>
+__device__ __forceinline__ void tile_words(Regs& r, const SweepArgs& a) {
+  const uint32_t body = tile_body<N, COMMIT, VOTES>(a);
+  r.skip = body & ~kBodyTally;
+  r.tally = (body & kBodyTally) != 0;
 }
 
 template <int N, int GPL, bool COMMIT, bool GATED, bool VOTES, int POLICY, int BLOCK = kBlock, int BODY = kBodyAll>
@@ -231,9 +269,15 @@
   constexpr int kVoteLanes = kTile / 8;
   if constexpr (VOTES) {
     if (tid < kVoteLanes) {
-      const uint8_t* src = a.votes + (tile0 + 8ull * tid) * vote_word_bytes(N);
-      r.vw[0] = ldg<NT>(reinterpret_cast<const u32x4p*>(src));
-      if constexpr (N > 8) r.vw[1] = ldg<NT>(reinterpret_cast<const u32x4p*>(src + 16));
+      if (r.tally) {
+        const uint64_t t = ldg<NT>(reinterpret_cast<const uint64_t*>(a.tally + tile0 + 8ull * tid));
+        r.vw[0].x = (uint32_t)t;
+        r.vw[0].y = (uint32_t)(t >> 32);
+      } else {
+        const uint8_t* src = a.votes + (tile0 + 8ull * tid) * vote_word_bytes(N);
+        r.vw[0] = ldg<NT>(reinterpret_cast<const u32x4p*>(src));
+        if constexpr (N > 8) r.vw[1] = ldg<NT>(reinterpret_cast<const u32x4p*>(src + 16));
+      }
     }
   }
   if constexpr (COMMIT) {
@@ -376,20 +420,31 @@
     if (vote_lane) {
       const uint64_t g = tile0 + 8ull * tid;
       uint32_t out = 0, n_won = 0, n_lost = 0;
-#pragma unroll
-      for (int k = 0; k < 8; ++k) {
-        uint32_t w;
-        if constexpr (N <= 8) {
-          const uint32_t pair = k < 2 ? r.vw[0].x : k < 4 ? r.vw[0].y : k < 6 ? r.vw[0].z : r.vw[0].w;
-          w = (k & 1) ? pair >> 16 : pair & 0xffffu;
-        } else {
-          w = k == 0 ? r.vw[0].x : k == 1 ? r.vw[0].y : k == 2 ? r.vw[0].z : k == 3 ? r.vw[0].w
-            : k == 4 ? r.vw[1].x : k == 5 ? r.vw[1].y : k == 6 ? r.vw[1].z : r.vw[1].w;
+      if (r.tally) {
+#pragma unroll
+        for (int k = 0; k < 8; ++k) {
+          const uint32_t b = ((k < 4 ? r.vw[0].x : r.vw[0].y) >> (8 * (k & 3))) & 0xffu;
+          const uint32_t oc = poll_tally<N>(b);
+          out |= oc << (2 * k);
+          n_won += oc & 1u;
+          n_lost += oc >> 1;
         }
-        const uint32_t oc = poll_word<N>(w);
-        out |= oc << (2 * k);
-        n_won += oc & 1u;
-        n_lost += oc >> 1;
+      } else {
+#pragma unroll
+        for (int k = 0; k < 8; ++k) {
+          uint32_t w;
+          if constexpr (N <= 8) {
+            const uint32_t pair = k < 2 ? r.vw[0].x : k < 4 ? r.vw[0].y : k < 6 ? r.vw[0].z : r.vw[0].w;
+            w = (k & 1) ? pair >> 16 : pair & 0xffffu;
+          } else {
+            w = k == 0 ? r.vw[0].x : k == 1 ? r.vw[0].y : k == 2 ? r.vw[0].z : k == 3 ? r.vw[0].w
+              : k == 4 ? r.vw[1].x : k == 5 ? r.vw[1].y : k == 6 ? r.vw[1].z : r.vw[1].w;
+          }
+          const uint32_t oc = poll_word<N>(w);
+          out |= oc << (2 * k);
+          n_won += oc & 1u;
+          n_lost += oc >> 1;
+        }
       }
       uint16_t* dst = reinterpret_cast<uint16_t*>(a.outcome + (g >> 2));
       if constexpr (NOSTORE) {
@@ -415,7 +470,7 @@
 template <int N, int GPL, bool COMMIT, bool GATED, bool VOTES, int POLICY, bool BITS, int BLOCK = kBlock>
 __device__ __forceinline__ void sweep_tile(const SweepArgs& a, const uint32_t tile) {
   TileRegs<N, GPL, COMMIT, GATED, VOTES> r;
-  r.skip = tile_body<N, COMMIT>(a);
+  tile_words<N, COMMIT, VOTES>(r, a);
   if constexpr (COMMIT && N >= 3) {
     if (r.skip == kSkipNarrow) {
       tile_load<N, GPL, COMMIT, GATED, VOTES, POLICY, BLOCK, kBodyNarrow>(r, a, tile);
@@ -459,7 +514,7 @@
     if (!want_bits) a.changed_bits = nullptr;
   };
   auto load = [&](Regs& r, const SweepArgs& a, uint32_t tile) {
-    r.skip = tile_body<N, COMMIT>(a);
+    tile_words<N, COMMIT, VOTES>(r, a);
     if constexpr (COMMIT && N >= 3) {
       if (r.skip == kSkipNarrow) {
         tile_load<N, GPL, COMMIT, GATED, VOTES, POLICY, kBlock, kBodyNarrow>(r, a, tile);
@@ -725,6 +780,19 @@
 }
 __device__ __forceinline__ void clear_narrow_if(bool broken, uint32_t* word) { clear_self_max_if(broken, word); }
 
+static __global__ __launch_bounds__(kBlock) void tally_build_kernel(const uint8_t* __restrict__ votes, uint64_t n_groups,
+                                                                    uint32_t n_peers, uint8_t* __restrict__ tally) {
+  for (uint64_t g = (uint64_t)blockIdx.x * kBlock + threadIdx.x; g < n_groups; g += (uint64_t)gridDim.x * kBlock) {
+    const uint32_t w = n_peers <= 8 ? (uint32_t)reinterpret_cast<const uint16_t*>(votes)[g] : reinterpret_cast<const uint32_t*>(votes)[g];
+    tally[g] = (uint8_t)tally_of_word(w, n_peers);
+  }
+}
+struct TallyMirror {
+  const uint32_t* word;
+  uint8_t* bytes;
+};
+__device__ __forceinline__ void clear_tally_if(bool broken, uint32_t* word) { clear_self_max_if(broken, word); }
+
 template <typename Rec>
 static __global__ __launch_bounds__(kBlock) void deltas_in_kernel(const Rec* __restrict__ src, Rec* __restrict__ dst,
                                                                   uint64_t n, uint64_t n_groups, uint32_t n_peers,
@@ -842,7 +910,7 @@
                                                             const VoteDeltaRec* __restrict__ d, uint64_t n,
                                                             const unsigned long long* bad, unsigned long long epoch_match,
                                                             unsigned long long epoch_votes, uint64_t n_groups,
-                                                            uint32_t n_peers, int each) {
+                                                            uint32_t n_peers, int each, TallyMirror tally) {
   if (!each && batch_is_bad(bad, epoch_match, epoch_votes)) return;
   const uint64_t i = (uint64_t)blockIdx.x * kBlock + threadIdx.x;
   if (i >= n) return;
@@ -850,6 +918,7 @@
   if (each && !vote_rec_ok(r, n_groups, n_peers)) return;
   const uint64_t slot = (uint64_t)r.peer * ld + r.group;
   if (claim[slot] != (uint32_t)i) return;
+  const bool follow = tally.bytes != nullptr && *tally.word == kTallyValid;
   unsigned int* word = reinterpret_cast<unsigned int*>(votes) + (wide ? r.group : r.group >> 1);
   const unsigned sh = (wide ? 0u : (unsigned)(r.group & 1ull) * 16u) + 2u * r.peer;
   const unsigned nv = (unsigned)r.vote << sh;
@@ -858,7 +927,12 @@
     const unsigned cur = (old >> sh) & 3u;
     if (cur == 1u || cur == 2u) break;
     const unsigned seen = atomicCAS(word, old, (old & ~(3u << sh)) | nv);
-    if (seen == old) break;
+    if (seen == old) {
+      if (follow)
+        atomicAdd(reinterpret_cast<unsigned int*>(tally.bytes) + (r.group >> 2),
+                  (r.vote == 1 ? 1u : 16u) << (8u * (unsigned)(r.group & 3ull)));
+      break;
+    }
     old = seen;
   }
   claim[slot] = 0xffffffffu;
@@ -997,7 +1071,7 @@
   __shared__ uint32_t wave_cnt[kWaves];
   const uint32_t tid = threadIdx.x, lane = tid & 63, wave = tid >> 6, tile = blockIdx.x;
   TileRegs<N, GPL, true, GATED, false> r;
-  r.skip = tile_body<N, true>(a);
+  tile_words<N, true, false>(r, a);
   const bool narrow = N >= 3 && r.skip == kSkipNarrow;
   if (narrow) {
     if constexpr (N >= 3) tile_load<N, GPL, true, GATED, false, POLICY, kBlock, kBodyNarrow>(r, a, tile);
@@ -1193,7 +1267,8 @@
 };
 static __global__ __launch_bounds__(kBlock) void apply_voter_deltas_kernel(uint16_t* voters, uint64_t* match, uint64_t ld, uint8_t* votes,
                                                                            int wide, uint32_t n_peers, const VoterDeltaRec* __restrict__ d,
-                                                                           uint64_t n, uint32_t* self_max, uint32_t* narrow) {
+                                                                           uint64_t n, uint32_t* self_max, uint32_t* narrow,
+                                                                           uint32_t* tally_word) {
   const uint64_t i = (uint64_t)blockIdx.x * kBlock + threadIdx.x;
   bool resets = false;
   if (i < n) {
@@ -1210,6 +1285,7 @@
   }
   clear_self_max_if(resets, self_max);
   clear_narrow_if(resets, narrow);
+  clear_tally_if(resets, tally_word);
 }
 
 struct TickArgs {
@@ -1668,7 +1744,7 @@
 
 static __global__ __launch_bounds__(kBlock) void campaign_kernel(uint8_t* role, uint32_t* elapsed, uint8_t* votes,
                                                           uint32_t n_peers, uint32_t self_peer,
-                                                          const uint64_t* __restrict__ groups, uint64_t n) {
+                                                          const uint64_t* __restrict__ groups, uint64_t n, uint8_t* tally) {
   const uint64_t i = (uint64_t)blockIdx.x * kBlock + threadIdx.x;
   if (i >= n) return;
   const uint64_t g = groups[i];
@@ -1676,6 +1752,7 @@
   elapsed[g] = 0;
   if (n_peers <= 8) reinterpret_cast<uint16_t*>(votes)[g] = (uint16_t)(1u << (2 * self_peer));
   else reinterpret_cast<uint32_t*>(votes)[g] = 1u << (2 * self_peer);
-}
-
-}
+  if (tally != nullptr) tally[g] = 1;
+}
+
+}
diff --git a/raftsql_amd/csrc/raftq_step_kernels.hpp b/raftsql_amd/csrc/raftq_step_kernels.hpp
--- a/raftsql_amd/csrc/raftq_step_kernels.hpp
+++ b/raftsql_amd/csrc/raftq_step_kernels.hpp
@@ -335,6 +335,7 @@
     if (vw_dirty) {
       if (a.n_peers <= 8) reinterpret_cast<uint16_t*>(a.votes)[g] = (uint16_t)vw;
       else reinterpret_cast<uint32_t*>(a.votes)[g] = vw;
+      if (a.self_max != nullptr && a.self_max[2] != 0u) a.self_max[2] = 0u;
     }
     if constexpr (CQ)
       if (cq_dirty) a.cq[g] = cqw;
diff --git a/raftsql_amd/engine.py b/raftsql_amd/engine.py
--- a/raftsql_amd/engine.py
+++ b/raftsql_amd/engine.py
@@ -374,6 +374,16 @@
         self._chk(self._lib.raftq_narrow_rebuild(self._h))
         return self.narrow()
 
+    def tally(self) -> bool:
+        v = C.c_int32(0)
+        self._chk(self._lib.raftq_tally(self._h, C.byref(v)))
+        return bool(v.value)
+
+    def tally_rebuild(self) -> bool:
+        v = C.c_int32(0)
+        self._chk(self._lib.raftq_tally_rebuild(self._h, C.byref(v)))
+        return bool(v.value)
+
     def read_votes(self) -> np.ndarray:
         out = np.empty((self.n_peers, self.n_groups), dtype=np.uint8)
         self._chk(self._lib.raftq_read_votes(self._h, _ptr(out)))
```
